# flashlight/wav2letter

Hardware: NVIDIA H100
Metric: frames_per_sec (higher is better)
Workload: dtype f32

## Files before the change

### include/w2l_b200.h

```cpp
#ifndef W2L_B200_H_
#define W2L_B200_H_

#include <stddef.h>
#include <stdint.h>

#ifdef __cplusplus
extern "C" {
#endif

#define W2L_API __attribute__((visibility("default")))

enum {
  W2L_OK = 0,
  W2L_ERR_INVALID_ARGUMENT = 1,
  W2L_ERR_WORKSPACE = 2,
  W2L_ERR_CUDA = 3,
  W2L_ERR_UNSUPPORTED = 4
};

enum {
  W2L_SCALE_NONE = 0,
  W2L_SCALE_INPUT_SZ = 1,
  W2L_SCALE_INPUT_SZ_SQRT = 2,
  W2L_SCALE_TARGET_SZ = 3,
  W2L_SCALE_TARGET_SZ_SQRT = 4
};

enum {
  W2L_TERM_FCC = 1,
  W2L_TERM_FAC = 2,
  W2L_TERM_ASG = 3
};

W2L_API int w2l_version(void);
W2L_API const char* w2l_last_error(void);
W2L_API long long w2l_launch_count(void);
W2L_API void w2l_reset_launch_count(void);
W2L_API void w2l_set_profile_events(void* start_event, void* stop_event);
W2L_API int w2l_set_profile_event_list(int kind, void** start_events, void** stop_events, int n);
W2L_API int w2l_profile_events_used(void);
W2L_API int w2l_trace_begin(void* stream, int capacity);
W2L_API long long w2l_trace_end(char* out, long long out_bytes);
W2L_API long long w2l_trace_list(char* out, long long out_bytes);

W2L_API size_t w2l_asg_workspace_size(int B, int T, int N, int L);
W2L_API int w2l_asg_forward_backward(void* stream, int terms, int B, int T, int N, int L, int scale_mode,
                                     const float* emis, const int32_t* target, const float* trans,
                                     const float* dloss, float* loss, float* d_emis, float* d_trans,
                                     void* workspace, size_t workspace_bytes);

W2L_API size_t w2l_fcc_viterbi_workspace_size(int B, int T, int N);
W2L_API int w2l_fcc_viterbi(void* stream, int B, int T, int N, const float* emis, const float* trans,
                            int32_t* path, void* workspace, size_t workspace_bytes);
W2L_API size_t w2l_fac_viterbi_workspace_size(int B, int T, int N, int L);
W2L_API int w2l_fac_viterbi(void* stream, int B, int T, int N, int L, const float* emis, const int32_t* target,
                            const float* trans, int32_t* path, int32_t* path_idx, void* workspace,
                            size_t workspace_bytes);

W2L_API size_t w2l_ctc_workspace_size(int B, int T, int N, int L);
W2L_API int w2l_ctc_forward_backward(void* stream, int B, int T, int N, int L, int scale_mode, const float* emis,
                                     const int32_t* target, const float* dloss, float* loss, float* d_emis,
                                     void* workspace, size_t workspace_bytes);
W2L_API int w2l_argmax_path(void* stream, int B, int T, int N, const float* emis, int32_t* path);

W2L_API size_t w2l_ctc_viterbi_workspace_size(int B, int T, int N, int L);
W2L_API int w2l_ctc_viterbi_target(void* stream, int B, int T, int N, int L, const float* emis, const int32_t* target,
                                   int32_t* path, int32_t* state, void* workspace, size_t workspace_bytes);

W2L_API int w2l_linseg_target(void* stream, int B, int T, int L, const int32_t* target, int32_t* out);

W2L_API int w2l_gemm_tf32_view(void* stream, int a_mn_major, int b_mn_major, int M, int N, int K, const float* A, int lda,
                               const float* B, int ldb, float* C, int ldc, const float* bias, int act, int accumulate);
enum { W2L_GEMM_TF32 = 0, W2L_GEMM_F32X3 = 1, W2L_GEMM_BF16 = 2 };
enum { W2L_PRECISION_TF32 = 0, W2L_PRECISION_F32 = 1, W2L_PRECISION_BF16 = 2 };
W2L_API int w2l_set_precision(int precision);
W2L_API int w2l_get_precision(void);
W2L_API int w2l_gemm(void* stream, int kind, int a_mn_major, int b_mn_major, int M, int N, int K, const void* A, int lda,
                     const void* B, int ldb, void* C, int ldc, int c_bf16, const float* bias, int act, int accumulate,
                     const void* aux, int ld_aux, int aux_bf16, int aux_mode, float aux_scale, float dropout_p,
                     unsigned long long seed, int allow_overlap);
W2L_API int w2l_cast_bf16(void* stream, long long n, const float* x, void* y);
W2L_API int w2l_cast_bf16_rows(void* stream, long long rows, int cols, int ld_in, int cols_padded, const float* x, void* y);
W2L_API int w2l_gemm_set_tile(int bn);
W2L_API int w2l_gemm_set_variant(int variant);
W2L_API int w2l_gemm_tf32(void* stream, int a_mn_major, int b_mn_major, int M, int N, int K, const float* A, int lda,
                          const float* B, int ldb, float* C, int ldc, const float* bias, int act);

W2L_API int w2l_gemm_tf32_ex(void* stream, int a_mn_major, int b_mn_major, int M, int N, int K, const float* A, int lda,
                             const float* B, int ldb, float* C, int ldc, const float* bias, int act, int accumulate,
                             const float* aux, int ld_aux, int aux_mode, float aux_scale, float dropout_p,
                             unsigned long long seed);

W2L_API size_t w2l_conv_time_workspace_size(int B, int Tout, int Cin, int Cout, int K);
W2L_API int w2l_conv_time_fwd(void* stream, int B, int T, int Tout, int W, int Cin, int Cout, int K, int stride,
                              int pad_left, const float* x, const float* wt, const float* bias, const float* add, float* y,
                              int act, float dropout_p, unsigned long long seed, void* ws, size_t ws_bytes);
W2L_API int w2l_conv_time_dgrad(void* stream, int B, int T, int Tout, int W, int Cin, int Cout, int K, int stride,
                                int pad_left, const float* dy, const float* wt, const float* add, float* dx, void* ws,
                                size_t ws_bytes);
W2L_API int w2l_conv_time_wgrad(void* stream, int B, int T, int Tout, int W, int Cin, int Cout, int K, int stride,
                                int pad_left, const float* x, const float* dy, float* dwt, float* dbias, void* ws,
                                size_t ws_bytes);

W2L_API int w2l_weightnorm_fwd(void* stream, int rows, int len, const float* v, const float* g, float* w, float* inv_norm);
W2L_API int w2l_weightnorm_bwd(void* stream, int rows, int len, const float* v, const float* g, const float* inv_norm,
                               const float* dw, float* dv, float* dg);
W2L_API int w2l_conv1d_arrange(void* stream, int cin, int cout, int kw, int cin_p, int cout_p, int glu_split, const float* w,
                               const float* bias, float* fwd, float* flip, float* bias_p);
W2L_API int w2l_conv1d_arrange_ex(void* stream, int cin, int cout, int kw, int cin_p, int cout_p, int glu_split, const float* w,
                                  const float* bias, void* fwd, void* flip, float* bias_p, int out_bf16);
W2L_API int w2l_conv1d_unarrange_grad(void* stream, int cin, int cout, int kw, int cin_p, int cout_p, int glu_split,
                                      const float* dfwd, float* dw, long long rows, const float* dy, float* dbias);
W2L_API int w2l_glu_fwd(void* stream, long long rows, int half, const float* x, float* y, float dropout_p,
                        unsigned long long seed);
W2L_API int w2l_glu_bwd(void* stream, long long rows, int half, const float* x, const float* dy, float* dx, float dropout_p,
                        unsigned long long seed);

#define W2L_LN_MAX_PARTS 80
#define W2L_LN_SCRATCH_DOUBLES(B) (2 * W2L_LN_MAX_PARTS * (size_t)(B))
W2L_API int w2l_layernorm_fwd(void* stream, int B, long long R, float eps, const float* a, const float* r,
                              const float* gain, const float* bias, float* y, float* mean_rstd, double* scratch);
W2L_API int w2l_layernorm_bwd(void* stream, int B, long long R, const float* a, const float* r, const float* dy,
                              const float* gain, const float* mean_rstd, float* d_branch, float* d_res, int branch_mode,
                              float branch_scale, float* dgain, float* dbias, double* scratch);

W2L_API int w2l_colsum_accumulate(void* stream, int M, int N, const float* X, int ld, float* out);
W2L_API int w2l_sq_norm_accumulate(void* stream, long long n, const float* g, double* out);
W2L_API int w2l_sgd_step(void* stream, long long n, float* params, const float* grads, float* velocity, float lr,
                         float momentum, float weight_decay, float grad_scale, float max_grad_norm, const double* sq_norm);
W2L_API int w2l_sgd_step_ex(void* stream, long long n, float* params, const float* grads, float* velocity, float lr, float momentum,
                            float weight_decay, float grad_scale, float max_grad_norm, const double* sq_norm, int nesterov,
                            const int* guard);
W2L_API int w2l_finite_guard(void* stream, int n_loss, const float* loss, const double* sq_norm, int* guard);
W2L_API int w2l_mask_bands(void* stream, int B, int T, int C, int W, const float* x, float* y, int n_f, const int* f0_host,
                           const int* f1_host, int n_t, const int* t0_host, const int* t1_host, float value);

W2L_API int w2l_transpose_input(void* stream, int B, int F, int T, const float* in, float* out);
W2L_API int w2l_axpy(void* stream, long long n, float a, const float* x, float* y);
W2L_API int w2l_fill(void* stream, long long n, float v, float* y);
W2L_API int w2l_delay(void* stream, int us);
W2L_API int w2l_act_fwd(void* stream, long long n, const float* x, int relu, float dropout_p, unsigned long long seed, float* y);
W2L_API int w2l_mask_mul(void* stream, long long n, const float* g, const float* ref, int mode, float scale, float* out);

W2L_API int w2l_mfsc_num_frames(int n_samples, int sample_rate, int frame_ms, int stride_ms);
W2L_API size_t w2l_mfsc_workspace_size(int B, int max_samples, int sample_rate, int frame_ms, int stride_ms, int n_filters);
W2L_API int w2l_mfsc(void* stream, int B, int max_samples, const float* audio, const int32_t* n_samples_host, int sample_rate,
                     int frame_ms, int stride_ms, int n_filters, int left_ctx, float* features, int T_out, void* ws,
                     size_t ws_bytes);

W2L_API void* w2l_trainer_create(void* stream, const char* arch_text, int n_feat, int n_label, const char* criterion,
                                 int scale_mode, float transdiag, float lr, float lrcrit, float momentum, float maxgradnorm);
W2L_API void w2l_trainer_destroy(void* trainer);
W2L_API int w2l_trainer_step(void* trainer, void* stream, int B, int T, const float* features, int L, const int32_t* target,
                             float* loss_out, int train, float total_batch);
W2L_API int w2l_trainer_forward(void* trainer, void* stream, int B, int T, const float* features, float* emissions_out,
                                long long capacity, int* t_out);
W2L_API int w2l_trainer_align(void* trainer, void* stream, int B, int T, const float* features, int L, const int32_t* target,
                              int32_t* path, int32_t* idx, long long capacity, int* t_out);
W2L_API int w2l_trainer_time_stride(void* trainer);
W2L_API int w2l_trainer_set_grad_stream(void* trainer, int on);
W2L_API int w2l_trainer_set_grad_stream_delay(void* trainer, int us);
W2L_API int w2l_trainer_set_precision(void* trainer, int precision);
W2L_API int w2l_trainer_status(void* trainer, void* stream, long long* skipped_steps);
W2L_API long long w2l_trainer_num_params(void* trainer, int which );
W2L_API int w2l_trainer_param_layout(void* trainer, int which, int max_params, long long* elements, long long* dims4);
W2L_API int w2l_trainer_get_flat(void* trainer, void* stream, int which, int what , float* out);
W2L_API int w2l_trainer_set_flat(void* trainer, void* stream, int which, const float* in);
W2L_API int w2l_trainer_sync_parameters(void* trainer, void* stream);
W2L_API const char* w2l_trainer_describe(void* trainer);
W2L_API int w2l_trainer_save(void* trainer, void* stream, const char* path);
W2L_API void* w2l_trainer_load(void* stream, const char* path);
W2L_API int w2l_trainer_export_streaming(void* trainer, void* stream, const char* outdir, const char* tokens_text);
W2L_API int w2l_nccl_unique_id(void* out128);
W2L_API int w2l_init_distributed(int rank, int world, const void* id128);

W2L_API void* w2l_text_create(const char* tokens_text, const char* lexicon_text, const char* criterion, int replabel,
                              const char* surround, int usewordpiece, const char* wordsep);
W2L_API void w2l_text_destroy(void* text);
W2L_API int w2l_text_num_classes(void* text);
W2L_API long long w2l_text_encode(void* text, const char* transcript, int32_t* out, long long cap);
W2L_API long long w2l_text_prediction2ltr(void* text, const int32_t* path, int n, char* out, long long cap);
W2L_API long long w2l_text_target2ltr(void* text, const int32_t* target, int len, char* out, long long cap);
W2L_API long long w2l_text_ltr2wrd(void* text, const char* letters, char* out, long long cap);
W2L_API long long w2l_text_align_words(void* text, const int32_t* target, int len, const int32_t* idx, int n_frames,
                                       double ms_per_frame, const char* utt_id, char* out, long long cap);
W2L_API int w2l_edit_distance(const char* hyp, const char* ref, long long* out4);

#ifdef __cplusplus
}
#endif
#endif
```

### wav2letter_b200/capi.py

```python
from __future__ import annotations

import ctypes
import os

import torch

_HERE = os.path.dirname(os.path.abspath(__file__))
LIB_PATH = os.path.join(_HERE, "libw2l_b200.so")

SCALE_MODES = {"none": 0, "input_sz": 1, "input_sz_sqrt": 2, "target_sz": 3, "target_sz_sqrt": 4}
TERM_FCC, TERM_FAC, TERM_ASG = 1, 2, 3

EXPORTS = [
    "w2l_version", "w2l_last_error", "w2l_launch_count", "w2l_reset_launch_count", "w2l_set_profile_events", "w2l_set_profile_event_list", "w2l_profile_events_used", "w2l_trace_begin", "w2l_trace_end", "w2l_trace_list",
    "w2l_asg_workspace_size", "w2l_asg_forward_backward",
    "w2l_fcc_viterbi_workspace_size", "w2l_fcc_viterbi",
    "w2l_fac_viterbi_workspace_size", "w2l_fac_viterbi",
    "w2l_ctc_workspace_size", "w2l_ctc_forward_backward", "w2l_argmax_path", "w2l_linseg_target",
    "w2l_ctc_viterbi_workspace_size", "w2l_ctc_viterbi_target",
    "w2l_set_precision", "w2l_get_precision", "w2l_gemm", "w2l_cast_bf16", "w2l_cast_bf16_rows", "w2l_sgd_step_ex", "w2l_finite_guard",
    "w2l_mask_bands", "w2l_trainer_set_precision", "w2l_trainer_set_grad_stream", "w2l_trainer_set_grad_stream_delay", "w2l_delay", "w2l_trainer_status", "w2l_trainer_save", "w2l_trainer_load", "w2l_trainer_export_streaming",
    "w2l_text_create", "w2l_text_destroy", "w2l_text_num_classes", "w2l_text_encode", "w2l_text_prediction2ltr", "w2l_text_target2ltr",
    "w2l_text_ltr2wrd", "w2l_text_align_words", "w2l_edit_distance",
    "w2l_gemm_set_variant", "w2l_gemm_set_tile", "w2l_gemm_tf32", "w2l_gemm_tf32_ex", "w2l_gemm_tf32_view", "w2l_conv_time_workspace_size", "w2l_conv_time_fwd", "w2l_conv_time_dgrad",
    "w2l_conv_time_wgrad", "w2l_layernorm_fwd", "w2l_layernorm_bwd", "w2l_colsum_accumulate", "w2l_sq_norm_accumulate",
    "w2l_sgd_step", "w2l_weightnorm_fwd", "w2l_weightnorm_bwd", "w2l_conv1d_arrange", "w2l_conv1d_arrange_ex", "w2l_conv1d_unarrange_grad",
    "w2l_glu_fwd", "w2l_glu_bwd", "w2l_transpose_input", "w2l_axpy", "w2l_fill", "w2l_act_fwd", "w2l_mask_mul",
    "w2l_trainer_create", "w2l_trainer_destroy", "w2l_trainer_step", "w2l_trainer_forward", "w2l_trainer_num_params",
    "w2l_trainer_param_layout", "w2l_trainer_get_flat", "w2l_trainer_set_flat", "w2l_trainer_sync_parameters",
    "w2l_trainer_describe", "w2l_nccl_unique_id", "w2l_init_distributed", "w2l_trainer_align", "w2l_trainer_time_stride",
    "w2l_mfsc_num_frames", "w2l_mfsc_workspace_size", "w2l_mfsc",
]


class W2LError(RuntimeError):
    def __init__(self, code: int, msg: str):
        super().__init__(f"w2l error {code}: {msg}")
        self.code = code


def _load() -> ctypes.CDLL:
    if not os.path.exists(LIB_PATH):
        raise ImportError(
            f"{LIB_PATH} is missing: build it with `python -c 'import __graft_entry__ as g; g.build()'` "
            "(there is no CPU / PyTorch fallback for the hot path)")
    lib = ctypes.CDLL(LIB_PATH)
    vp, i, sz = ctypes.c_void_p, ctypes.c_int, ctypes.c_size_t
    lib.w2l_last_error.restype = ctypes.c_char_p
    lib.w2l_launch_count.restype = ctypes.c_longlong
    lib.w2l_set_profile_events.argtypes = [vp, vp]
    lib.w2l_set_profile_event_list.argtypes = [i, vp, vp, i]
    lib.w2l_trace_begin.argtypes = [vp, i]
    lib.w2l_trace_end.restype = ctypes.c_longlong
    lib.w2l_trace_end.argtypes = [ctypes.c_char_p, ctypes.c_longlong]
    lib.w2l_trace_list.restype = ctypes.c_longlong
    lib.w2l_trace_list.argtypes = [ctypes.c_char_p, ctypes.c_longlong]
    lib.w2l_asg_workspace_size.restype = sz
    lib.w2l_asg_workspace_size.argtypes = [i, i, i, i]
    lib.w2l_asg_forward_backward.argtypes = [vp, i, i, i, i, i, i, vp, vp, vp, vp, vp, vp, vp, vp, sz]
    lib.w2l_fcc_viterbi_workspace_size.restype = sz
    lib.w2l_fcc_viterbi_workspace_size.argtypes = [i, i, i]
    lib.w2l_fcc_viterbi.argtypes = [vp, i, i, i, vp, vp, vp, vp, sz]
    lib.w2l_fac_viterbi_workspace_size.restype = sz
    lib.w2l_fac_viterbi_workspace_size.argtypes = [i, i, i, i]
    lib.w2l_fac_viterbi.argtypes = [vp, i, i, i, i, vp, vp, vp, vp, vp, vp, sz]
    lib.w2l_ctc_workspace_size.restype = sz
    lib.w2l_ctc_workspace_size.argtypes = [i, i, i, i]
    lib.w2l_ctc_forward_backward.argtypes = [vp, i, i, i, i, i, vp, vp, vp, vp, vp, vp, sz]
    lib.w2l_argmax_path.argtypes = [vp, i, i, i, vp, vp]
    lib.w2l_linseg_target.argtypes = [vp, i, i, i, vp, vp]
    lib.w2l_ctc_viterbi_workspace_size.restype = sz
    lib.w2l_ctc_viterbi_workspace_size.argtypes = [i, i, i, i]
    lib.w2l_ctc_viterbi_target.argtypes = [vp, i, i, i, i, vp, vp, vp, vp, vp, sz]
    lib.w2l_gemm_tf32.argtypes = [vp, i, i, i, i, i, vp, i, vp, i, vp, i, vp, i]
    f32, u64, ll = ctypes.c_float, ctypes.c_ulonglong, ctypes.c_longlong
    ll = ctypes.c_longlong
    lib.w2l_weightnorm_fwd.argtypes = [vp, i, i, vp, vp, vp, vp]
    lib.w2l_weightnorm_bwd.argtypes = [vp, i, i, vp, vp, vp, vp, vp, vp]
    lib.w2l_conv1d_arrange.argtypes = [vp, i, i, i, i, i, i, vp, vp, vp, vp, vp]
    lib.w2l_conv1d_unarrange_grad.argtypes = [vp, i, i, i, i, i, i, vp, vp, ll, vp, vp]
    lib.w2l_glu_fwd.argtypes = [vp, ll, i, vp, vp, f32, u64]
    lib.w2l_glu_bwd.argtypes = [vp, ll, i, vp, vp, vp, f32, u64]
    lib.w2l_act_fwd.argtypes = [vp, ll, vp, i, f32, u64, vp]
    lib.w2l_mask_mul.argtypes = [vp, ll, vp, vp, i, f32, vp]
    lib.w2l_gemm_tf32_view.argtypes = [vp, i, i, i, i, i, vp, i, vp, i, vp, i, vp, i, i]
    lib.w2l_gemm_tf32_ex.argtypes = [vp, i, i, i, i, i, vp, i, vp, i, vp, i, vp, i, i, vp, i, i, f32, f32, u64]
    lib.w2l_conv_time_workspace_size.restype = sz
    lib.w2l_conv_time_workspace_size.argtypes = [i, i, i, i, i]
    lib.w2l_conv_time_fwd.argtypes = [vp, i, i, i, i, i, i, i, i, i, vp, vp, vp, vp, vp, i, f32, u64, vp, sz]
    lib.w2l_conv_time_dgrad.argtypes = [vp, i, i, i, i, i, i, i, i, i, vp, vp, vp, vp, vp, sz]
    lib.w2l_conv_time_wgrad.argtypes = [vp, i, i, i, i, i, i, i, i, i, vp, vp, vp, vp, vp, sz]
    lib.w2l_layernorm_fwd.argtypes = [vp, i, ll, f32, vp, vp, vp, vp, vp, vp, vp]
    lib.w2l_layernorm_bwd.argtypes = [vp, i, ll, vp, vp, vp, vp, vp, vp, vp, i, f32, vp, vp, vp]
    lib.w2l_colsum_accumulate.argtypes = [vp, i, i, vp, i, vp]
    lib.w2l_sq_norm_accumulate.argtypes = [vp, ll, vp, vp]
    lib.w2l_sgd_step.argtypes = [vp, ll, vp, vp, vp, f32, f32, f32, f32, f32, vp]
    lib.w2l_set_precision.argtypes = [i]
    lib.w2l_gemm.argtypes = [vp, i, i, i, i, i, i, vp, i, vp, i, vp, i, i, vp, i, i, vp, i, i, i, f32, f32, u64, i]
    lib.w2l_cast_bf16.argtypes = [vp, ll, vp, vp]
    lib.w2l_cast_bf16_rows.argtypes = [vp, ll, i, i, i, vp, vp]
    lib.w2l_sgd_step_ex.argtypes = [vp, ll, vp, vp, vp, f32, f32, f32, f32, f32, vp, i, vp]
    lib.w2l_finite_guard.argtypes = [vp, i, vp, vp, vp]
    lib.w2l_mask_bands.argtypes = [vp, i, i, i, i, vp, vp, i, vp, vp, i, vp, vp, f32]
    lib.w2l_trainer_set_precision.argtypes = [vp, i]
    lib.w2l_trainer_set_grad_stream.argtypes = [vp, i]
    lib.w2l_trainer_set_grad_stream_delay.argtypes = [vp, i]
    lib.w2l_delay.argtypes = [vp, i]
    lib.w2l_trainer_status.argtypes = [vp, vp, vp]
    cp = ctypes.c_char_p
    lib.w2l_trainer_save.argtypes = [vp, vp, cp]
    lib.w2l_trainer_load.restype = vp
    lib.w2l_trainer_load.argtypes = [vp, cp]
    lib.w2l_trainer_export_streaming.argtypes = [vp, vp, cp, cp]
    lib.w2l_text_create.restype = vp
    lib.w2l_text_create.argtypes = [cp, cp, cp, i, cp, i, cp]
    lib.w2l_text_destroy.argtypes = [vp]
    lib.w2l_text_destroy.restype = None
    lib.w2l_text_num_classes.argtypes = [vp]
    for fn in (lib.w2l_text_encode, lib.w2l_text_prediction2ltr, lib.w2l_text_target2ltr, lib.w2l_text_ltr2wrd):
        fn.restype = ll
    lib.w2l_text_encode.argtypes = [vp, cp, vp, ll]
    lib.w2l_text_prediction2ltr.argtypes = [vp, vp, i, vp, ll]
    lib.w2l_text_target2ltr.argtypes = [vp, vp, i, vp, ll]
    lib.w2l_text_ltr2wrd.argtypes = [vp, cp, vp, ll]
    lib.w2l_text_align_words.restype = ll
    lib.w2l_text_align_words.argtypes = [vp, vp, i, vp, i, ctypes.c_double, cp, vp, ll]
    lib.w2l_edit_distance.argtypes = [cp, cp, vp]
    lib.w2l_trainer_create.restype = vp
    lib.w2l_trainer_create.argtypes = [vp, ctypes.c_char_p, i, i, ctypes.c_char_p, i, f32, f32, f32, f32, f32]
    lib.w2l_trainer_destroy.argtypes = [vp]
    lib.w2l_trainer_destroy.restype = None
    lib.w2l_trainer_step.argtypes = [vp, vp, i, i, vp, i, vp, vp, i, f32]
    lib.w2l_trainer_forward.argtypes = [vp, vp, i, i, vp, vp, ll, vp]
    lib.w2l_trainer_align.argtypes = [vp, vp, i, i, vp, i, vp, vp, vp, ll, vp]
    lib.w2l_trainer_time_stride.argtypes = [vp]
    lib.w2l_trainer_num_params.restype = ll
    lib.w2l_trainer_num_params.argtypes = [vp, i]
    lib.w2l_trainer_param_layout.argtypes = [vp, i, i, vp, vp]
    lib.w2l_trainer_get_flat.argtypes = [vp, vp, i, i, vp]
    lib.w2l_trainer_set_flat.argtypes = [vp, vp, i, vp]
    lib.w2l_trainer_sync_parameters.argtypes = [vp, vp]
    lib.w2l_trainer_describe.restype = ctypes.c_char_p
    lib.w2l_trainer_describe.argtypes = [vp]
    lib.w2l_nccl_unique_id.argtypes = [vp]
    lib.w2l_init_distributed.argtypes = [i, i, vp]
    lib.w2l_mfsc_num_frames.argtypes = [i, i, i, i]
    lib.w2l_mfsc_workspace_size.restype = sz
    lib.w2l_mfsc_workspace_size.argtypes = [i, i, i, i, i, i]
    lib.w2l_mfsc.argtypes = [vp, i, i, vp, vp, i, i, i, i, i, vp, i, vp, sz]
    return lib


lib = _load()


def _check(rc: int) -> None:
    if rc != 0:
        raise W2LError(rc, lib.w2l_last_error().decode())


def _stream() -> int:
    return torch.cuda.current_stream().cuda_stream


def _ptr(t):
    return None if t is None else ctypes.c_void_p(t.data_ptr())


def _req(t, dtype, name):
    if t is None:
        return None
    if not t.is_cuda or t.dtype != dtype or not t.is_contiguous():
        raise TypeError(f"{name}: expected a contiguous CUDA tensor of {dtype}")
    return t


_ws_cache: dict = {}


def workspace(nbytes: int, device) -> torch.Tensor:
    key = (str(device), "ws")
    t = _ws_cache.get(key)
    if t is None or t.numel() < nbytes:
        t = torch.empty(max(nbytes, 256), dtype=torch.uint8, device=device)
        _ws_cache[key] = t
    return t


def _mode(m) -> int:
    return SCALE_MODES[m] if isinstance(m, str) else int(m)


def launch_count() -> int:
    return int(lib.w2l_launch_count())


def reset_launch_count() -> None:
    lib.w2l_reset_launch_count()


def set_profile_events(start=None, stop=None) -> None:
    if start is None:
        lib.w2l_set_profile_events(None, None)
    else:
        start.record()
        stop.record()
        lib.w2l_set_profile_events(ctypes.c_void_p(start.cuda_event), ctypes.c_void_p(stop.cuda_event))


def asg_forward_backward(emis, target, trans, scale_mode="none", dloss=None, terms=TERM_ASG, need_grad=True,
                         out=None, ws=None):
    emis = _req(emis, torch.float32, "emis")
    trans = _req(trans, torch.float32, "trans")
    target = _req(target, torch.int32, "target")
    dloss = _req(dloss, torch.float32, "dloss")
    B, T, N = emis.shape
    L = 0 if target is None else target.shape[1]
    if out is None:
        loss = torch.empty(B, dtype=torch.float32, device=emis.device)
        d_emis = torch.empty_like(emis) if need_grad else None
        d_trans = torch.empty_like(trans) if need_grad else None
    else:
        loss, d_emis, d_trans = out
    need = lib.w2l_asg_workspace_size(B, T, N, L)
    if ws is None:
        ws = workspace(need, emis.device)
    _check(lib.w2l_asg_forward_backward(_stream(), terms, B, T, N, L, _mode(scale_mode), _ptr(emis), _ptr(target),
                                        _ptr(trans), _ptr(dloss), _ptr(loss), _ptr(d_emis), _ptr(d_trans),
                                        _ptr(ws), ws.numel()))
    return loss, d_emis, d_trans


def fcc_viterbi(emis, trans):
    emis = _req(emis, torch.float32, "emis")
    trans = _req(trans, torch.float32, "trans")
    B, T, N = emis.shape
    path = torch.empty((B, T), dtype=torch.int32, device=emis.device)
    ws = workspace(lib.w2l_fcc_viterbi_workspace_size(B, T, N), emis.device)
    _check(lib.w2l_fcc_viterbi(_stream(), B, T, N, _ptr(emis), _ptr(trans), _ptr(path), _ptr(ws), ws.numel()))
    return path


def fac_viterbi(emis, target, trans, return_index=False):
    emis = _req(emis, torch.float32, "emis")
    trans = _req(trans, torch.float32, "trans")
    target = _req(target, torch.int32, "target")
    B, T, N = emis.shape
    L = target.shape[1]
    path = torch.empty((B, T), dtype=torch.int32, device=emis.device)
    idx = torch.empty((B, T), dtype=torch.int32, device=emis.device) if return_index else None
    ws = workspace(lib.w2l_fac_viterbi_workspace_size(B, T, N, L), emis.device)
    _check(lib.w2l_fac_viterbi(_stream(), B, T, N, L, _ptr(emis), _ptr(target), _ptr(trans), _ptr(path), _ptr(idx),
                               _ptr(ws), ws.numel()))
    return (path, idx) if return_index else path


def ctc_forward_backward(emis, target, scale_mode="none", dloss=None, need_grad=True, out=None, ws=None):
    emis = _req(emis, torch.float32, "emis")
    target = _req(target, torch.int32, "target")
    dloss = _req(dloss, torch.float32, "dloss")
    B, T, N = emis.shape
    L = 0 if target is None else target.shape[1]
    if out is None:
        loss = torch.empty(B, dtype=torch.float32, device=emis.device)
        d_emis = torch.empty_like(emis) if need_grad else None
    else:
        loss, d_emis = out
    need = lib.w2l_ctc_workspace_size(B, T, N, L)
    if ws is None:
        ws = workspace(need, emis.device)
    _check(lib.w2l_ctc_forward_backward(_stream(), B, T, N, L, _mode(scale_mode), _ptr(emis), _ptr(target),
                                        _ptr(dloss), _ptr(loss), _ptr(d_emis), _ptr(ws), ws.numel()))
    return loss, d_emis


def argmax_path(emis):
    emis = _req(emis, torch.float32, "emis")
    B, T, N = emis.shape
    path = torch.empty((B, T), dtype=torch.int32, device=emis.device)
    _check(lib.w2l_argmax_path(_stream(), B, T, N, _ptr(emis), _ptr(path)))
    return path


def ctc_viterbi_target(emis, target, return_state=False):
    emis = _req(emis, torch.float32, "emis")
    target = _req(target, torch.int32, "target")
    B, T, N = emis.shape
    L = target.shape[1]
    path = torch.empty((B, T), dtype=torch.int32, device=emis.device)
    state = torch.empty((B, T), dtype=torch.int32, device=emis.device) if return_state else None
    ws = workspace(lib.w2l_ctc_viterbi_workspace_size(B, T, N, L), emis.device)
    _check(lib.w2l_ctc_viterbi_target(_stream(), B, T, N, L, _ptr(emis), _ptr(target), _ptr(path), _ptr(state), _ptr(ws),
                                      ws.numel()))
    return (path, state) if return_state else path


def linseg_target(target, T: int):
    target = _req(target, torch.int32, "target")
    B, L = target.shape
    out = torch.empty((B, int(T)), dtype=torch.int32, device=target.device)
    _check(lib.w2l_linseg_target(_stream(), B, int(T), L, _ptr(target), _ptr(out)))
    return out


class ProfileList:

    def __init__(self, kind: int, n: int):
        self.starts = [torch.cuda.Event(enable_timing=True) for _ in range(n)]
        self.stops = [torch.cuda.Event(enable_timing=True) for _ in range(n)]
        for e in self.starts + self.stops:
            e.record()
        self._a = (ctypes.c_void_p * n)(*[e.cuda_event for e in self.starts])
        self._b = (ctypes.c_void_p * n)(*[e.cuda_event for e in self.stops])
        self.kind, self.n = kind, n

    def arm(self):
        lib.w2l_set_profile_event_list(self.kind, self._a, self._b, self.n)

    def disarm(self) -> int:
        used = int(lib.w2l_profile_events_used())
        lib.w2l_set_profile_event_list(0, None, None, 0)
        return used

    def times_ms(self, used: int):
        return [self.starts[k].elapsed_time(self.stops[k]) for k in range(used)]


def trace_list() -> list:
    buf = ctypes.create_string_buffer(1 << 18)
    lib.w2l_trace_list(buf, len(buf))
    return [(ln.split("\t")[0], float(ln.split("\t")[1])) for ln in buf.value.decode().splitlines()]


PRECISIONS = {"tf32": 0, "f32": 1, "fp32": 1, "bf16": 2}
GEMM_KINDS = {"tf32": 0, "f32x3": 1, "bf16": 2}


def set_precision(p) -> None:
    _check(lib.w2l_set_precision(PRECISIONS[p] if isinstance(p, str) else int(p)))


def get_precision() -> int:
    return int(lib.w2l_get_precision())


def gemm(A, B, kind="tf32", a_mn=False, b_mn=False, bias=None, act=0, out=None, out_bf16=False, accumulate=False, aux=None,
         aux_mode=0, aux_scale=1.0, dropout_p=0.0, seed=0, M=None, N=None, K=None, lda=None, ldb=None, allow_overlap=False):
    if M is None:
        M, K = (A.shape[1], A.shape[0]) if a_mn else A.shape
        N = B.shape[1] if b_mn else B.shape[0]
    lda = A.stride(0) if lda is None else lda
    ldb = B.stride(0) if ldb is None else ldb
    if out is None:
        out = torch.empty((M, N), dtype=torch.bfloat16 if out_bf16 else torch.float32, device=A.device)
    _check(lib.w2l_gemm(_stream(), GEMM_KINDS[kind], int(a_mn), int(b_mn), M, N, K, _ptr(A), lda, _ptr(B), ldb, _ptr(out),
                        out.stride(0), int(out.dtype == torch.bfloat16), _ptr(bias), int(act), int(accumulate), _ptr(aux),
                        0 if aux is None else aux.stride(0), int(aux is not None and aux.dtype == torch.bfloat16),
                        int(aux_mode), float(aux_scale), float(dropout_p), int(seed), int(allow_overlap)))
    return out


def cast_bf16(x):
    x = _req(x, torch.float32, "x")
    y = torch.empty(x.shape, dtype=torch.bfloat16, device=x.device)
    _check(lib.w2l_cast_bf16(_stream(), x.numel(), _ptr(x), _ptr(y)))
    return y


def gemm_set_variant(v: int = 1):
    _check(lib.w2l_gemm_set_variant(int(v)))


def gemm_set_tile(bn: int = 0):
    _check(lib.w2l_gemm_set_tile(int(bn)))


def trace(fn, capacity: int = 4096) -> dict:
    _check(lib.w2l_trace_begin(_stream(), capacity))
    try:
        fn()
    finally:
        buf = ctypes.create_string_buffer(1 << 16)
        lib.w2l_trace_end(buf, len(buf))
    out = {}
    for line in buf.value.decode().splitlines():
        name, n, ms = line.split("\t")
        out[name] = (int(n), float(ms))
    return out


def gemm_tf32(A, B, bias=None, act=0, a_mn=False, b_mn=False, out=None):
    A = _req(A, torch.float32, "A")
    B = _req(B, torch.float32, "B")
    bias = _req(bias, torch.float32, "bias")
    M, K = (A.shape[1], A.shape[0]) if a_mn else A.shape
    N = B.shape[1] if b_mn else B.shape[0]
    if out is None:
        out = torch.empty((M, N), dtype=torch.float32, device=A.device)
    _check(lib.w2l_gemm_tf32(_stream(), int(a_mn), int(b_mn), M, N, K, _ptr(A), A.stride(0), _ptr(B), B.stride(0),
                             _ptr(out), out.stride(0), _ptr(bias), int(act)))
    return out


def gemm_tf32_ex(A, B, out, bias=None, act=0, a_mn=False, b_mn=False, accumulate=False, aux=None, aux_mode=0,
                 aux_scale=1.0, dropout_p=0.0, seed=0):
    M, K = (A.shape[1], A.shape[0]) if a_mn else A.shape
    N = B.shape[1] if b_mn else B.shape[0]
    _check(lib.w2l_gemm_tf32_ex(_stream(), int(a_mn), int(b_mn), M, N, K, _ptr(A), A.stride(0), _ptr(B), B.stride(0),
                                _ptr(out), out.stride(0), _ptr(bias), int(act), int(accumulate), _ptr(aux),
                                0 if aux is None else aux.stride(0), int(aux_mode), float(aux_scale), float(dropout_p),
                                int(seed)))
    return out


def gemm_tf32_view(A, lda, B, ldb, out, M, N, K, a_mn=False, b_mn=False, bias=None, act=0, accumulate=False):
    _check(lib.w2l_gemm_tf32_view(_stream(), int(a_mn), int(b_mn), M, N, K, _ptr(A), lda, _ptr(B), ldb, _ptr(out), out.stride(0),
                                  _ptr(bias), int(act), int(accumulate)))
    return out


def conv_time_ws(B, Tout, Cin, Cout, K, device):
    return workspace(lib.w2l_conv_time_workspace_size(B, Tout, Cin, Cout, K), device)


def conv_time_fwd(x, wt, bias, Tout, stride, pad_left, act=0, dropout_p=0.0, seed=0, add=None):
    B, T, Cin, W = x.shape
    Cout, _, K = wt.shape
    y = torch.empty((B, Tout, Cout, W), dtype=torch.float32, device=x.device)
    ws = conv_time_ws(B, Tout, Cin, Cout, K, x.device)
    _check(lib.w2l_conv_time_fwd(_stream(), B, T, Tout, W, Cin, Cout, K, stride, pad_left, _ptr(x), _ptr(wt), _ptr(bias),
                                 _ptr(add), _ptr(y), act, float(dropout_p), int(seed), _ptr(ws), ws.numel()))
    return y


def conv_time_dgrad(dy, wt, T, stride, pad_left, add=None, out=None):
    B, Tout, Cout, W = dy.shape
    _, Cin, K = wt.shape
    dx = out if out is not None else torch.empty((B, T, Cin, W), dtype=torch.float32, device=dy.device)
    ws = conv_time_ws(B, Tout, Cin, Cout, K, dy.device)
    _check(lib.w2l_conv_time_dgrad(_stream(), B, T, Tout, W, Cin, Cout, K, stride, pad_left, _ptr(dy), _ptr(wt), _ptr(add),
                                   _ptr(dx), _ptr(ws), ws.numel()))
    return dx


def conv_time_wgrad(x, dy, K, stride, pad_left, dwt=None, dbias=None):
    B, T, Cin, W = x.shape
    _, Tout, Cout, _ = dy.shape
    if dwt is None:
        dwt = torch.zeros((Cout, Cin, K), dtype=torch.float32, device=x.device)
        dbias = torch.zeros(Cout, dtype=torch.float32, device=x.device)
    ws = conv_time_ws(B, Tout, Cin, Cout, K, x.device)
    _check(lib.w2l_conv_time_wgrad(_stream(), B, T, Tout, W, Cin, Cout, K, stride, pad_left, _ptr(x), _ptr(dy), _ptr(dwt),
                                   _ptr(dbias), _ptr(ws), ws.numel()))
    return dwt, dbias


def layernorm_fwd(a, r, gain, bias, eps=1e-5):
    B = a.shape[0]
    R = a[0].numel()
    y = torch.empty_like(a)
    mr = torch.empty((B, 2), dtype=torch.float32, device=a.device)
    scratch = torch.empty(160 * B, dtype=torch.float64, device=a.device)
    _check(lib.w2l_layernorm_fwd(_stream(), B, R, float(eps), _ptr(a), _ptr(r), _ptr(gain), _ptr(bias), _ptr(y), _ptr(mr),
                                 _ptr(scratch)))
    return y, mr


def layernorm_bwd(a, r, dy, gain, mr, branch_mode=0, branch_scale=1.0):
    B = a.shape[0]
    R = a[0].numel()
    d_branch = torch.empty_like(a)
    d_res = torch.empty_like(a)
    dgain = torch.zeros(1, dtype=torch.float32, device=a.device)
    dbias = torch.zeros(1, dtype=torch.float32, device=a.device)
    scratch = torch.empty(160 * B, dtype=torch.float64, device=a.device)
    _check(lib.w2l_layernorm_bwd(_stream(), B, R, _ptr(a), _ptr(r), _ptr(dy), _ptr(gain), _ptr(mr), _ptr(d_branch),
                                 _ptr(d_res), int(branch_mode), float(branch_scale), _ptr(dgain), _ptr(dbias),
                                 _ptr(scratch)))
    return d_branch, d_res, dgain, dbias
```

### wav2letter_b200/csrc/gemm_wgmma.cu

```cuda
#include <cuda.h>
#include <cuda_bf16.h>
#include <cuda_runtime.h>

#include <algorithm>
#include <cmath>
#include <cstdlib>
#include <mutex>

#include "common.cuh"
#include "tma_ptx.cuh"
#include "wgmma_ptx.cuh"

namespace w2l {
namespace {
using namespace tma;

constexpr int BM = 128;
constexpr int kRowBytes = 128;
constexpr int kTileBytes = BM * kRowBytes;
constexpr int kGemmThreads = 384;
constexpr int kConvThreads = 96;
constexpr int kConsumerThreads = 256;
enum { kTf32 = W2L_GEMM_TF32, kF32x3 = W2L_GEMM_F32X3, kBf16 = W2L_GEMM_BF16 };

__host__ __device__ constexpr bool converts(int mode, bool a_mn, bool b_mn) { return mode == kF32x3 || (mode == kTf32 && (a_mn || b_mn)); }
__host__ __device__ constexpr size_t raw_bytes(int bn) { return (size_t)kTileBytes + (size_t)bn * kRowBytes; }
__host__ __device__ constexpr size_t cvt_bytes(int mode, int bn) { return (size_t)bn * kRowBytes * (mode == kF32x3 ? 2 : 1); }
constexpr size_t kSmemTail = 1024 + 256;
constexpr size_t kSmemBudget = 227 * 1024 - kSmemTail;
constexpr int kConvRawStages = 4;
constexpr int kIdSlots = 4;
__host__ __device__ constexpr int raw_stages(int mode, bool a_mn, bool b_mn, int bn) {
  return converts(mode, a_mn, b_mn) ? kConvRawStages : (kSmemBudget / raw_bytes(bn) > 6 ? 6 : (int)(kSmemBudget / raw_bytes(bn)));
}
__host__ __device__ constexpr int cvt_stages(int mode, bool a_mn, bool b_mn, int bn) {
  return !converts(mode, a_mn, b_mn) ? 0
         : (kSmemBudget - kConvRawStages * raw_bytes(bn)) / cvt_bytes(mode, bn) > 4 ? 4
                                                                                     : (int)((kSmemBudget - kConvRawStages * raw_bytes(bn)) / cvt_bytes(mode, bn));
}
__host__ __device__ constexpr size_t smem_for(int mode, bool a_mn, bool b_mn, int bn) {
  return raw_stages(mode, a_mn, b_mn, bn) * raw_bytes(bn) + cvt_stages(mode, a_mn, b_mn, bn) * cvt_bytes(mode, bn) + kSmemTail;
}

struct GemmParams {
  int M, N, K, ldc, act;
  void* C;
  const float* bias;
  int accumulate, aux_mode, ld_aux;
  const void* aux;
  float aux_scale, drop_p;
  unsigned long long seed;
  int k_splits;
  int c_bf16, aux_bf16;
  float* ws;
};

__device__ __forceinline__ uint32_t rn_tf32(uint32_t x) { return (x + 0x1000u) & 0xffffe000u; }

template <bool kMn, bool kLo, int ROWS>
__device__ __forceinline__ void convert_tile(const unsigned char* raw, unsigned char* hi, unsigned char* lo, int ct) {
#pragma unroll 4
  for (int i = ct; i < ROWS * 8; i += kConvThreads) {
    const int r = i % ROWS, c = i / ROWS;
    const uint32_t off = (uint32_t)r * 128u + ((uint32_t)(c ^ (r & 7)) << 4);
    uint4 v;
    if (kMn) {
      const uint32_t* src = reinterpret_cast<const uint32_t*>(raw) + 4 * c * ROWS + r;
      v = make_uint4(src[0], src[ROWS], src[2 * ROWS], src[3 * ROWS]);
    } else {
      v = *reinterpret_cast<const uint4*>(raw + off);
    }
    const uint4 h = make_uint4(rn_tf32(v.x), rn_tf32(v.y), rn_tf32(v.z), rn_tf32(v.w));
    *reinterpret_cast<uint4*>(hi + off) = h;
    if (kLo) {
      const uint4 l = make_uint4(rn_tf32(__float_as_uint(__uint_as_float(v.x) - __uint_as_float(h.x))),
                                 rn_tf32(__float_as_uint(__uint_as_float(v.y) - __uint_as_float(h.y))),
                                 rn_tf32(__float_as_uint(__uint_as_float(v.z) - __uint_as_float(h.z))),
                                 rn_tf32(__float_as_uint(__uint_as_float(v.w) - __uint_as_float(h.w))));
      *reinterpret_cast<uint4*>(lo + off) = l;
    }
  }
}

__device__ __forceinline__ void epilogue_pair(const GemmParams& p, int z, int row, int col, float x0, float x1, float b0, float b1, bool vec_c) {
  const bool two = col + 1 < p.N;
  x0 += b0;
  x1 += b1;
  if (p.act == 1) {
    x0 = fmaxf(x0, 0.f);
    x1 = fmaxf(x1, 0.f);
  }
  if (p.drop_p > 0.f) {
    const uint32_t thresh = (uint32_t)(p.drop_p * 65536.0f);
    const float inv_keep = 1.0f / (1.0f - p.drop_p);
    const unsigned long long idx = ((unsigned long long)row * (unsigned long long)p.N + (unsigned long long)col) >> 1;
    uint32_t h = ((uint32_t)idx ^ (uint32_t)p.seed) * 0x9E3779B1u + ((uint32_t)(idx >> 32) ^ (uint32_t)(p.seed >> 32));
    h ^= h >> 15;
    h *= 0x85EBCA77u;
    h ^= h >> 13;
    h *= 0xC2B2AE3Du;
    h ^= h >> 16;
    x0 *= (h & 0xffffu) >= thresh ? inv_keep : 0.f;
    x1 *= (h >> 16) >= thresh ? inv_keep : 0.f;
  }
  if (p.aux_mode != 0) {
    float m0, m1 = 0.f;
    const size_t ai = (size_t)row * p.ld_aux + col;
    if (p.aux_bf16) {
      const __nv_bfloat16* a = static_cast<const __nv_bfloat16*>(p.aux) + ai;
      m0 = __bfloat162float(a[0]);
      if (two) m1 = __bfloat162float(a[1]);
    } else {
      const float* a = static_cast<const float*>(p.aux) + ai;
      m0 = a[0];
      if (two) m1 = a[1];
    }
    if (p.aux_mode == 1) {
      x0 *= m0 > 0.f ? p.aux_scale : 0.f;
      x1 *= m1 > 0.f ? p.aux_scale : 0.f;
    } else {
      x0 *= m0 != 0.f ? p.aux_scale : 0.f;
      x1 *= m1 != 0.f ? p.aux_scale : 0.f;
    }
  }
  const size_t ci = (size_t)row * p.ldc + col;
  if (p.c_bf16) {
    __nv_bfloat16* dst = static_cast<__nv_bfloat16*>(p.C) + ci;
    if (two && vec_c) {
      *reinterpret_cast<__nv_bfloat162*>(dst) = __floats2bfloat162_rn(x0, x1);
    } else {
      dst[0] = __float2bfloat16_rn(x0);
      if (two) dst[1] = __float2bfloat16_rn(x1);
    }
    return;
  }
  if (p.k_splits > 1) {
    float* part = p.ws + ((size_t)z * p.M + row) * p.N + col;
    part[0] = x0;
    if (two) part[1] = x1;
    return;
  }
  float* dst = static_cast<float*>(p.C) + ci;
  if (two && vec_c) {
    if (p.accumulate) {
      const float2 c = *reinterpret_cast<const float2*>(dst);
      x0 += c.x;
      x1 += c.y;
    }
    *reinterpret_cast<float2*>(dst) = make_float2(x0, x1);
  } else {
    if (p.accumulate) x0 += dst[0];
    dst[0] = x0;
    if (two) {
      if (p.accumulate) x1 += dst[1];
      dst[1] = x1;
    }
  }
}

template <int kMode, bool kAMn, bool kBMn, int BN>
__global__ void __launch_bounds__(kGemmThreads, 1)
gemm_wgmma_kernel(const __grid_constant__ CUtensorMap map_a, const __grid_constant__ CUtensorMap map_b, GemmParams p, int tiles_m, int tiles_n,
                  unsigned int* sched) {
  extern __shared__ __align__(1024) unsigned char smem_raw[];
  unsigned char* smem = reinterpret_cast<unsigned char*>((reinterpret_cast<uintptr_t>(smem_raw) + 1023) & ~(uintptr_t)1023);
  constexpr bool kIsBf16 = kMode == kBf16, kSplit = kMode == kF32x3, kConv = converts(kMode, kAMn, kBMn);
  constexpr int BKE = kRowBytes / (kIsBf16 ? 2 : 4);
  constexpr int kStages = raw_stages(kMode, kAMn, kBMn, BN), kCvtStages = cvt_stages(kMode, kAMn, kBMn, BN);
  constexpr size_t kRaw = raw_bytes(BN), kCvt = cvt_bytes(kMode, BN);
  constexpr uint32_t kOperandBytes = (uint32_t)kRaw;
  static_assert(kStages >= 2 && (!kConv || kCvtStages >= 2), "gemm: at least two stages per ring");
  static_assert(!kConv || BN == 128, "gemm: the converted kinds take A from registers at BN = 128");
  static_assert(!kIsBf16 || !kBMn || BN % 64 == 0, "gemm: MN-major bf16 B is staged in boxes of 64 columns");
  unsigned char* cvt_ring = smem + kStages * kRaw;
  uint64_t* bars = reinterpret_cast<uint64_t*>(cvt_ring + kCvtStages * kCvt);
  uint64_t* full = bars;
  uint64_t* empty = bars + kStages;
  uint64_t* ready = bars + 2 * kStages;
  uint64_t* cvt_empty = ready + kCvtStages;
  uint64_t* id_full = cvt_empty + kCvtStages;
  uint64_t* id_empty = id_full + kIdSlots;
  int* id_ring = reinterpret_cast<int*>(id_empty + kIdSlots);
  static_assert((2 * (kStages + kCvtStages + kIdSlots)) * 8 + kIdSlots * 4 <= kSmemTail - 1024, "gemm: barrier space");
  constexpr uint32_t kIdReaders = kConsumerThreads + (kConv ? kConvThreads : 0);

  const int tid = threadIdx.x, warp = tid >> 5, lane = tid & 31, wg = warp >> 2;
  const int total_kb = (p.K + BKE - 1) / BKE;
  const int kb_per = (total_kb + p.k_splits - 1) / p.k_splits;
  const int tiles_mn = tiles_m * tiles_n, total_tiles = tiles_mn * p.k_splits;

  if (tid == 0) {
    for (int s = 0; s < kStages; ++s) {
      mbar_init(&full[s], 1);
      mbar_init(&empty[s], kConsumerThreads + (kConv ? kConvThreads : 0));
    }
    for (int s = 0; s < kCvtStages; ++s) {
      mbar_init(&ready[s], kConvThreads);
      mbar_init(&cvt_empty[s], kConsumerThreads);
    }
    for (int s = 0; s < kIdSlots; ++s) {
      mbar_init(&id_full[s], 1);
      mbar_init(&id_empty[s], kIdReaders);
    }
    asm volatile("fence.mbarrier_init.release.cluster;" ::: "memory");
  }
  __syncthreads();

  uint32_t id_it = 0;
  auto next_item = [&]() {
    const int s = id_it % kIdSlots;
    mbar_wait(&id_full[s], (id_it / kIdSlots) & 1);
    const int t = id_ring[s];
    mbar_arrive(&id_empty[s]);
    ++id_it;
    return t;
  };
  auto tile_coords = [&](int t, int& m0, int& n0, int& kb_begin, int& num_kb) {
    const int z = t / tiles_mn, r = t - z * tiles_mn;
    m0 = (r / tiles_n) * BM;
    n0 = (r % tiles_n) * BN;
    kb_begin = z * kb_per;
    num_kb = max(0, min(total_kb, kb_begin + kb_per) - kb_begin);
  };

  if (wg == 0) {
    if (warp == 0) {
      if (lane == 0) {
        asm volatile("prefetch.tensormap [%0];" ::"l"(&map_a) : "memory");
        asm volatile("prefetch.tensormap [%0];" ::"l"(&map_b) : "memory");
        uint32_t it = 0;
        for (int t = blockIdx.x; t < total_tiles;) {
          int m0, n0, kb_begin, num_kb;
          tile_coords(t, m0, n0, kb_begin, num_kb);
          for (int kb = 0; kb < num_kb; ++kb, ++it) {
            const int s = it % kStages;
            mbar_wait(&empty[s], ((it / kStages) & 1) ^ 1);
            mbar_expect_tx(&full[s], kOperandBytes);
            unsigned char* sa = smem + s * kRaw;
            unsigned char* sb = sa + kTileBytes;
            const int k0 = (kb_begin + kb) * BKE;
            if (!kAMn) {
              tma_load_2d(&map_a, &full[s], sa, k0, m0);
            } else if (kIsBf16) {
#pragma unroll
              for (int j = 0; j < BM / 64; ++j) tma_load_2d(&map_a, &full[s], sa + j * 8192, m0 + 64 * j, k0);
            } else {
#pragma unroll
              for (int j = 0; j < BM / 8; ++j) tma_load_2d(&map_a, &full[s], sa + j * 1024, m0 + 8 * j, k0);
            }
            if (!kBMn) {
              tma_load_2d(&map_b, &full[s], sb, k0, n0);
            } else if (kIsBf16) {
#pragma unroll
              for (int j = 0; j < BN / 64; ++j) tma_load_2d(&map_b, &full[s], sb + j * 8192, n0 + 64 * j, k0);
            } else {
              tma_load_2d(&map_b, &full[s], sb, n0, k0);
            }
          }
          t = sched ? (int)gridDim.x + (int)atomicAdd(sched, 1u) : t + (int)gridDim.x;
          const int s = id_it % kIdSlots;
          mbar_wait(&id_empty[s], ((id_it / kIdSlots) & 1) ^ 1);
          id_ring[s] = t;
          mbar_arrive(&id_full[s]);
          ++id_it;
        }
        if (sched) {
          __threadfence();
          if (atomicAdd(sched + 1, 1u) == gridDim.x - 1) {
            atomicExch(sched, 0u);
            atomicExch(sched + 1, 0u);
          }
        }
      }
    } else if constexpr (kConv) {
      const int ct = tid - 32;
      uint32_t it = 0;
      for (int t = blockIdx.x; t < total_tiles; t = next_item()) {
        int m0, n0, kb_begin, num_kb;
        tile_coords(t, m0, n0, kb_begin, num_kb);
        for (int kb = 0; kb < num_kb; ++kb, ++it) {
          const int s = it % kStages, c = it % kCvtStages;
          mbar_wait(&cvt_empty[c], ((it / kCvtStages) & 1) ^ 1);
          mbar_wait(&full[s], (it / kStages) & 1);
          unsigned char* dst = cvt_ring + c * kCvt;
          convert_tile<kBMn, kSplit, BN>(smem + s * kRaw + kTileBytes, dst, dst + BN * kRowBytes, ct);
          mbar_arrive(&empty[s]);
          asm volatile("fence.proxy.async.shared::cta;" ::: "memory");
          mbar_arrive(&ready[c]);
        }
      }
    }
  } else {
    const int cw = wg - 1;
    const bool vec_c = (p.ldc % 2) == 0 && (reinterpret_cast<uintptr_t>(p.C) & (p.c_bf16 ? 3 : 7)) == 0;
    const int fr = 64 * cw + 16 * (warp & 3) + (lane >> 2), fq = lane & 3;
    uint32_t it = 0;
    for (int t = blockIdx.x; t < total_tiles; t = next_item()) {
      int m0, n0, kb_begin, num_kb;
      tile_coords(t, m0, n0, kb_begin, num_kb);
      float acc[BN / 2];
#pragma unroll
      for (int i = 0; i < BN / 2; ++i) acc[i] = 0.f;
      if constexpr (kConv) {
        struct AFrag {
          uint32_t hi[4][4], lo[4][4];
        };
        auto fence_frag = [&](AFrag& f) {
          wg::fence_operands(f.hi);
          if constexpr (kSplit) wg::fence_operands(f.lo);
        };
        auto step = [&](AFrag& cur, AFrag& prev, int kb) {
          const int s = it % kStages, c = it % kCvtStages;
          mbar_wait(&full[s], (it / kStages) & 1);
          const uint32_t sa = smem_u32(smem + s * kRaw);
#pragma unroll
          for (int kk = 0; kk < 4; ++kk) {
#pragma unroll
            for (int i = 0; i < 4; ++i) {
              const int r = fr + 8 * (i & 1), k = 8 * kk + 4 * (i >> 1) + fq;
              const int off = kAMn ? (r >> 3) * 1024 + k * 32 + (r & 7) * 4 : r * 128 + (((k >> 2) ^ (r & 7)) << 4) + (k & 3) * 4;
              uint32_t x;
              asm volatile("ld.shared.b32 %0, [%1];" : "=r"(x) : "r"(sa + off) : "memory");
              cur.hi[kk][i] = rn_tf32(x);
              if constexpr (kSplit) cur.lo[kk][i] = rn_tf32(__float_as_uint(__uint_as_float(x) - __uint_as_float(cur.hi[kk][i])));
            }
          }
          mbar_arrive(&empty[s]);
          mbar_wait(&ready[c], (it / kCvtStages) & 1);
          const uint32_t b_base = smem_u32(cvt_ring + c * kCvt);
          fence_frag(cur);
          wg::fence_operands(acc);
          wg::fence();
#pragma unroll
          for (int kk = 0; kk < 4; ++kk) {
            const int sc = (kb | kk) != 0;
            const uint64_t db = make_desc_sw128(b_base + kk * 32, 16, 1024);
            if constexpr (kSplit) {
              wg::mma_tf32_rs<BN>(acc, cur.lo[kk], db, sc);
              wg::mma_tf32_rs<BN>(acc, cur.hi[kk], make_desc_sw128(b_base + BN * kRowBytes + kk * 32, 16, 1024), 1);
              wg::mma_tf32_rs<BN>(acc, cur.hi[kk], db, 1);
            } else {
              wg::mma_tf32_rs<BN>(acc, cur.hi[kk], db, sc);
            }
          }
          wg::commit();
          wg::fence_operands(acc);
          if constexpr (kSplit) wg::wait<1>(); else wg::wait<0>();
          fence_frag(prev);
          if (kb > 0) mbar_arrive(&cvt_empty[(it - 1) % kCvtStages]);
          ++it;
        };
        AFrag fa, fb;
        for (int kb = 0; kb < num_kb; kb += 2) {
          step(fa, fb, kb);
          if (kb + 1 < num_kb) step(fb, fa, kb + 1);
        }
        wg::wait<0>();
        wg::fence_operands(acc);
        fence_frag(fa);
        fence_frag(fb);
        if (num_kb > 0) mbar_arrive(&cvt_empty[(it - 1) % kCvtStages]);
      } else {
        for (int kb = 0; kb < num_kb; ++kb, ++it) {
          const int s = it % kStages;
          mbar_wait(&full[s], (it / kStages) & 1);
          const uint32_t a_base = smem_u32(smem + s * kRaw) + (uint32_t)(cw * 8192), b_base = smem_u32(smem + s * kRaw) + kTileBytes;
          wg::fence_operands(acc);
          wg::fence();
#pragma unroll
          for (int k = 0; k < 4; ++k) {
            const int sc = (kb | k) != 0;
            if constexpr (kIsBf16) {
              const uint64_t da = kAMn ? make_desc_sw128(a_base + k * 2048, 8192, 1024) : make_desc_sw128(a_base + k * 32, 16, 1024);
              const uint64_t db = kBMn ? make_desc_sw128(b_base + k * 2048, 8192, 1024) : make_desc_sw128(b_base + k * 32, 16, 1024);
              wg::mma_bf16<BN, kAMn ? 1 : 0, kBMn ? 1 : 0>(acc, da, db, sc);
            } else {
              wg::mma_tf32<BN>(acc, make_desc_sw128(a_base + k * 32, 16, 1024), make_desc_sw128(b_base + k * 32, 16, 1024), sc);
            }
          }
          wg::commit();
          wg::fence_operands(acc);
          wg::wait<1>();
          if (kb > 0) mbar_arrive(&empty[(it - 1) % kStages]);
        }
        wg::wait<0>();
        wg::fence_operands(acc);
        if (num_kb > 0) mbar_arrive(&empty[(it - 1) % kStages]);
      }
      const int z = t / tiles_mn;
      const int row0 = m0 + 64 * cw + 16 * (warp & 3) + (lane >> 2);
      const int col0 = n0 + 2 * (lane & 3);
#pragma unroll
      for (int j = 0; j < BN / 8; ++j) {
        const int col = col0 + 8 * j;
        if (col < p.N) {
          const float b0 = p.bias != nullptr ? __ldg(p.bias + col) : 0.f;
          const float b1 = (p.bias != nullptr && col + 1 < p.N) ? __ldg(p.bias + col + 1) : 0.f;
          if (row0 < p.M) epilogue_pair(p, z, row0, col, acc[4 * j], acc[4 * j + 1], b0, b1, vec_c);
          if (row0 + 8 < p.M) epilogue_pair(p, z, row0 + 8, col, acc[4 * j + 2], acc[4 * j + 3], b0, b1, vec_c);
        }
      }
    }
  }
}

__global__ void __launch_bounds__(256) splitk_reduce_kernel(int M, int N, int splits, const float* __restrict__ ws, float* __restrict__ C, int ldc,
                                                            int accumulate) {
  const long long mn = (long long)M * N;
  for (long long i = (long long)blockIdx.x * blockDim.x + threadIdx.x; i < mn; i += (long long)gridDim.x * blockDim.x) {
    const long long r = i / N, c = i - r * N;
    float* dst = C + r * ldc + c;
    float s = accumulate ? *dst : 0.f;
    for (int z = 0; z < splits; ++z) s += ws[z * mn + i];
    *dst = s;
  }
}

int make_map(CUtensorMap* map, int mode, bool conv, const void* ptr, long long rows, long long cols, long long ld, int box_cols, int box_rows,
             bool swizzle) {
  EncodeTiledFn fn = encode_fn();
  if (!fn) return fail(W2L_ERR_CUDA, "gemm: cuTensorMapEncodeTiled entry point not found");
  const int es = mode == kBf16 ? 2 : 4;
  cuuint64_t dims[2] = {(cuuint64_t)cols, (cuuint64_t)rows};
  cuuint64_t strides[1] = {(cuuint64_t)ld * es};
  cuuint32_t box[2] = {(cuuint32_t)box_cols, (cuuint32_t)box_rows};
  cuuint32_t estr[2] = {1, 1};
  const CUtensorMapDataType dt = mode == kBf16 ? CU_TENSOR_MAP_DATA_TYPE_BFLOAT16 : (conv ? CU_TENSOR_MAP_DATA_TYPE_FLOAT32 : CU_TENSOR_MAP_DATA_TYPE_TFLOAT32);
  CUresult r = fn(map, dt, 2, const_cast<void*>(ptr), dims, strides, box, estr, CU_TENSOR_MAP_INTERLEAVE_NONE,
                  swizzle ? CU_TENSOR_MAP_SWIZZLE_128B : CU_TENSOR_MAP_SWIZZLE_NONE, CU_TENSOR_MAP_L2_PROMOTION_L2_256B,
                  CU_TENSOR_MAP_FLOAT_OOB_FILL_NONE);
  if (r != CUDA_SUCCESS) return fail(W2L_ERR_CUDA, "gemm: cuTensorMapEncodeTiled failed with code " + std::to_string((int)r));
  return W2L_OK;
}

const char* kernel_name(int mode) { return mode == kBf16 ? "gemm_wgmma_kernel<bf16>" : (mode == kF32x3 ? "gemm_wgmma_kernel<f32x3>" : "gemm_wgmma_kernel<tf32>"); }

thread_local int g_variant = 1;

constexpr int kSchedSlots = 64;
__device__ unsigned int g_sched[kSchedSlots][2];
unsigned int* sched_slot(cudaStream_t stream) {
  static std::mutex mu;
  static cudaStream_t owner[kSchedSlots];
  static int used = 0;
  int slot = -1;
  {
    std::lock_guard<std::mutex> lock(mu);
    for (int i = 0; i < used && slot < 0; ++i)
      if (owner[i] == stream) slot = i;
    if (slot < 0 && used < kSchedSlots) {
      owner[used] = stream;
      slot = used++;
    }
  }
  void* base = nullptr;
  if (slot < 0 || cudaGetSymbolAddress(&base, g_sched) != cudaSuccess) return nullptr;
  return static_cast<unsigned int*>(base) + 2 * slot;
}

template <int kMode, bool kAMn, bool kBMn, int BN>
int launch_bn(cudaStream_t stream, const CUtensorMap& ma, const CUtensorMap& mb, const GemmParams& p) {
  constexpr size_t smem = smem_for(kMode, kAMn, kBMn, BN);
  static_assert(smem <= 227 * 1024, "gemm: shared-memory budget");
  static bool configured = false;
  if (!configured) {
    W2L_CUDA_CHECK(cudaFuncSetAttribute(gemm_wgmma_kernel<kMode, kAMn, kBMn, BN>, cudaFuncAttributeMaxDynamicSharedMemorySize, (int)smem));
    configured = true;
  }
  const int tiles_m = (p.M + BM - 1) / BM, tiles_n = (p.N + BN - 1) / BN;
  const int total = tiles_m * tiles_n * p.k_splits;
  const int grid = g_variant == 1 ? std::min(total, sm_count()) : total;
  unsigned int* sched = g_variant == 1 && grid < total ? sched_slot(stream) : nullptr;
  profile_kind(1);
  profile_start(stream);
  gemm_wgmma_kernel<kMode, kAMn, kBMn, BN><<<grid, kGemmThreads, smem, stream>>>(ma, mb, p, tiles_m, tiles_n, sched);
  profile_stop(stream);
  W2L_LAUNCH_CHECK(kernel_name(kMode));
  return W2L_OK;
}
template <int kMode, bool kAMn, bool kBMn>
int launch_mode(cudaStream_t stream, int bn, const CUtensorMap& ma, const CUtensorMap& mb, const GemmParams& p) {
  if constexpr (converts(kMode, kAMn, kBMn)) {
    return launch_bn<kMode, kAMn, kBMn, 128>(stream, ma, mb, p);
  } else if constexpr (kMode == kBf16) {
    return bn <= 128 ? launch_bn<kMode, kAMn, kBMn, 128>(stream, ma, mb, p) : launch_bn<kMode, kAMn, kBMn, 256>(stream, ma, mb, p);
  } else {
    switch (bn) {
      case 128: return launch_bn<kMode, kAMn, kBMn, 128>(stream, ma, mb, p);
      case 160: return launch_bn<kMode, kAMn, kBMn, 160>(stream, ma, mb, p);
      case 224: return launch_bn<kMode, kAMn, kBMn, 224>(stream, ma, mb, p);
      default: return launch_bn<kMode, kAMn, kBMn, 256>(stream, ma, mb, p);
    }
  }
}
template <int kMode>
int launch(cudaStream_t stream, bool a_mn, bool b_mn, int bn, const CUtensorMap& ma, const CUtensorMap& mb, const GemmParams& p) {
  if (!a_mn && !b_mn) return launch_mode<kMode, false, false>(stream, bn, ma, mb, p);
  if (!a_mn && b_mn) return launch_mode<kMode, false, true>(stream, bn, ma, mb, p);
  if (a_mn && b_mn) return launch_mode<kMode, true, true>(stream, bn, ma, mb, p);
  return launch_mode<kMode, true, false>(stream, bn, ma, mb, p);
}

int splits_for(int tiles, int total_kb, bool plain) {
  const int sms = sm_count();
  if (!plain || tiles >= sms || total_kb < 16) return 1;
  return std::max(1, std::min(std::min(sms / tiles, total_kb / 4), 32));
}
thread_local int g_force_bn = 0;
int choose_bn(int mode, bool a_mn, bool b_mn, int M, int N, int total_kb, bool plain, int* splits_out) {
  auto allowed = [&](int bn) {
    if (converts(mode, a_mn, b_mn)) return bn == 128;
    if (mode == kBf16) return bn == 128 || bn == 256;
    return true;
  };
  if (g_force_bn && allowed(g_force_bn)) {
    const int tiles = ((N + g_force_bn - 1) / g_force_bn) * ((M + BM - 1) / BM);
    *splits_out = splits_for(tiles, total_kb, plain);
    return g_force_bn;
  }
  const int cands[4] = {128, 160, 224, 256};
  const double sms = sm_count();
  double best = 1e300;
  int best_bn = 128;
  *splits_out = 1;
  for (int bn : cands) {
    if (!allowed(bn)) continue;
    const int tiles = ((N + bn - 1) / bn) * ((M + BM - 1) / BM);
    const int splits = splits_for(tiles, total_kb, plain);
    const int kb_local = (total_kb + splits - 1) / splits;
    const double waves = std::ceil((double)tiles * splits / sms);
    const double cost = waves * ((double)(128 + bn) * kb_local + 2.0 * bn);
    if (cost < best - 1e-9) {
      best = cost;
      best_bn = bn;
      *splits_out = splits;
    }
  }
  return best_bn;
}

int gemm_impl(void* stream_, int mode, int a_mn_major, int b_mn_major, int M, int N, int K, const void* A, int lda, const void* B, int ldb,
              void* C, int ldc, int c_bf16, const float* bias, int act, int accumulate, const void* aux, int ld_aux, int aux_bf16,
              int aux_mode, float aux_scale, float dropout_p, unsigned long long seed, bool allow_overlap) {
  cudaStream_t stream = static_cast<cudaStream_t>(stream_);
  if (mode != kTf32 && mode != kF32x3 && mode != kBf16) return fail(W2L_ERR_INVALID_ARGUMENT, "gemm: unknown operand kind");
  if (M <= 0 || N <= 0 || K <= 0) return fail(W2L_ERR_INVALID_ARGUMENT, "gemm: M, N, K must be positive");
  if (!A || !B || !C) return fail(W2L_ERR_INVALID_ARGUMENT, "gemm: null pointer");
  if (act < 0 || act > 1) return fail(W2L_ERR_INVALID_ARGUMENT, "gemm: act must be 0 (none) or 1 (relu)");
  if (aux_mode < 0 || aux_mode > 2 || (aux_mode != 0 && (!aux || ld_aux < N)))
    return fail(W2L_ERR_INVALID_ARGUMENT, "gemm: bad aux mask arguments");
  if (dropout_p < 0.f || dropout_p >= 1.f) return fail(W2L_ERR_INVALID_ARGUMENT, "gemm: dropout_p must be in [0, 1)");
  if (dropout_p > 0.f && N % 4 != 0) return fail(W2L_ERR_INVALID_ARGUMENT, "gemm: dropout needs N % 4 == 0");
  const int row_align = mode == kBf16 ? 8 : 4;
  if ((lda % row_align) || (ldb % row_align) || (reinterpret_cast<uintptr_t>(A) & 15) || (reinterpret_cast<uintptr_t>(B) & 15))
    return fail(W2L_ERR_INVALID_ARGUMENT, "gemm: operand rows must be 16-byte aligned (ld % 4 == 0 for fp32, ld % 8 == 0 for bf16)");
  if (ldc < N || (!allow_overlap && (lda < (a_mn_major ? M : K) || ldb < (b_mn_major ? N : K))))
    return fail(W2L_ERR_INVALID_ARGUMENT, "gemm: leading dimension smaller than the row length");
  if (lda <= 0 || ldb <= 0) return fail(W2L_ERR_INVALID_ARGUMENT, "gemm: non-positive leading dimension");
  if (c_bf16 && accumulate) return fail(W2L_ERR_INVALID_ARGUMENT, "gemm: accumulation needs an fp32 C");
  const int bke = kRowBytes / (mode == kBf16 ? 2 : 4);
  const int total_kb = (K + bke - 1) / bke;
  const bool plain = act == 0 && aux_mode == 0 && dropout_p == 0.f && bias == nullptr && !c_bf16;
  int splits = 1;
  const int BN = choose_bn(mode, a_mn_major != 0, b_mn_major != 0, M, N, total_kb, plain, &splits);
  const bool conv = converts(mode, a_mn_major != 0, b_mn_major != 0);
  const bool bf16 = mode == kBf16;
  CUtensorMap ma, mb;
  int rc;
  if (!a_mn_major)
    rc = make_map(&ma, mode, conv, A, M, K, lda, bke, BM, true);
  else
    rc = make_map(&ma, mode, conv, A, K, M, lda, bf16 ? 64 : 8, bke, bf16);
  if (rc) return rc;
  if (!b_mn_major)
    rc = make_map(&mb, mode, conv, B, N, K, ldb, bke, BN, true);
  else
    rc = make_map(&mb, mode, conv, B, K, N, ldb, bf16 ? 64 : BN, bke, bf16);
  if (rc) return rc;
  GemmParams p{M, N, K, ldc, act, C, bias, accumulate, aux_mode, ld_aux, aux, aux_scale, dropout_p, seed, splits, c_bf16, aux_bf16, nullptr};
  if (splits > 1) W2L_CUDA_CHECK(cudaMallocAsync(reinterpret_cast<void**>(&p.ws), sizeof(float) * (size_t)splits * M * N, stream));
  rc = mode == kBf16 ? launch<kBf16>(stream, a_mn_major, b_mn_major, BN, ma, mb, p)
                     : (mode == kF32x3 ? launch<kF32x3>(stream, a_mn_major, b_mn_major, BN, ma, mb, p) : launch<kTf32>(stream, a_mn_major, b_mn_major, BN, ma, mb, p));
  if (splits > 1) {
    if (rc == W2L_OK) {
      const long long mn = (long long)M * N;
      splitk_reduce_kernel<<<(unsigned)std::min<long long>((mn + 255) / 256, (long long)sm_count() * 8), 256, 0, stream>>>(M, N, splits, p.ws,
                                                                                                                        static_cast<float*>(C), ldc, accumulate);
      cudaError_t e = cudaGetLastError();
      if (e != cudaSuccess) rc = fail(W2L_ERR_CUDA, std::string("launch splitk_reduce_kernel: ") + cudaGetErrorString(e));
      else {
        count_launch();
        trace_launch("splitk_reduce_kernel");
      }
    }
    cudaFreeAsync(p.ws, stream);
  }
  return rc;
}

int f32_kind() { return current_precision() == W2L_PRECISION_F32 ? kF32x3 : kTf32; }

__global__ void __launch_bounds__(256) cast_bf16_kernel(long long n4, const float4* __restrict__ x, uint2* __restrict__ y, long long n,
                                                        const float* __restrict__ xs, __nv_bfloat16* __restrict__ ys) {
  const long long i = (long long)blockIdx.x * blockDim.x + threadIdx.x;
  if (i < n4) {
    const float4 v = x[i];
    const __nv_bfloat162 a = __floats2bfloat162_rn(v.x, v.y), b = __floats2bfloat162_rn(v.z, v.w);
    y[i] = make_uint2(*reinterpret_cast<const uint32_t*>(&a), *reinterpret_cast<const uint32_t*>(&b));
  }
  if (i < n - 4 * n4) ys[4 * n4 + i] = __float2bfloat16_rn(xs[4 * n4 + i]);
}
__global__ void __launch_bounds__(256) cast_bf16_rows_kernel(long long rows, int cols, int ld_in, int cols_p, const float* __restrict__ x,
                                                             __nv_bfloat16* __restrict__ y) {
  const long long total = rows * cols_p;
  for (long long i = (long long)blockIdx.x * blockDim.x + threadIdx.x; i < total; i += (long long)gridDim.x * blockDim.x) {
    const long long r = i / cols_p;
    const int c = (int)(i % cols_p);
    y[i] = c < cols ? __float2bfloat16_rn(x[r * ld_in + c]) : __float2bfloat16_rn(0.f);
  }
}

}
}

using namespace w2l;

extern "C" int w2l_gemm_set_variant(int variant) {
  if (variant < 0 || variant > 1) return fail(W2L_ERR_INVALID_ARGUMENT, "gemm: variant must be 0 (one tile per CTA) or 1 (one CTA per SM)");
  g_variant = variant;
  return W2L_OK;
}

extern "C" int w2l_gemm_set_tile(int bn) {
  if (bn != 0 && bn != 128 && bn != 160 && bn != 224 && bn != 256) return fail(W2L_ERR_INVALID_ARGUMENT, "gemm: tile width must be 0 (auto), 128, 160, 224 or 256");
  g_force_bn = bn;
  return W2L_OK;
}

extern "C" int w2l_gemm(void* stream, int kind, int a_mn_major, int b_mn_major, int M, int N, int K, const void* A, int lda, const void* B,
                        int ldb, void* C, int ldc, int c_bf16, const float* bias, int act, int accumulate, const void* aux, int ld_aux,
                        int aux_bf16, int aux_mode, float aux_scale, float dropout_p, unsigned long long seed, int allow_overlap) {
  return gemm_impl(stream, kind, a_mn_major, b_mn_major, M, N, K, A, lda, B, ldb, C, ldc, c_bf16, bias, act, accumulate, aux, ld_aux, aux_bf16,
                   aux_mode, aux_scale, dropout_p, seed, allow_overlap != 0);
}

extern "C" int w2l_gemm_tf32_ex(void* stream_, int a_mn_major, int b_mn_major, int M, int N, int K, const float* A, int lda,
                                const float* B, int ldb, float* C, int ldc, const float* bias, int act, int accumulate,
                                const float* aux, int ld_aux, int aux_mode, float aux_scale, float dropout_p,
                                unsigned long long seed) {
  return gemm_impl(stream_, f32_kind(), a_mn_major, b_mn_major, M, N, K, A, lda, B, ldb, C, ldc, 0, bias, act, accumulate, aux, ld_aux, 0, aux_mode,
                   aux_scale, dropout_p, seed, false);
}

extern "C" int w2l_gemm_tf32(void* stream_, int a_mn_major, int b_mn_major, int M, int N, int K, const float* A, int lda,
                             const float* B, int ldb, float* C, int ldc, const float* bias, int act) {
  return w2l_gemm_tf32_ex(stream_, a_mn_major, b_mn_major, M, N, K, A, lda, B, ldb, C, ldc, bias, act, 0, nullptr, 0, 0, 1.f, 0.f, 0ull);
}

extern "C" int w2l_gemm_tf32_view(void* stream_, int a_mn_major, int b_mn_major, int M, int N, int K, const float* A, int lda,
                                  const float* B, int ldb, float* C, int ldc, const float* bias, int act, int accumulate) {
  return gemm_impl(stream_, f32_kind(), a_mn_major, b_mn_major, M, N, K, A, lda, B, ldb, C, ldc, 0, bias, act, accumulate, nullptr, 0, 0, 0, 1.f, 0.f,
                   0ull, true);
}

extern "C" int w2l_cast_bf16(void* stream_, long long n, const float* x, void* y) {
  if (n <= 0) return W2L_OK;
  if (!x || !y) return fail(W2L_ERR_INVALID_ARGUMENT, "cast_bf16: null pointer");
  cudaStream_t stream = static_cast<cudaStream_t>(stream_);
  const bool vec = ((reinterpret_cast<uintptr_t>(x) & 15) == 0) && ((reinterpret_cast<uintptr_t>(y) & 7) == 0);
  const long long n4 = vec ? n / 4 : 0;
  const long long threads = std::max<long long>(n4, n - 4 * n4);
  cast_bf16_kernel<<<(unsigned)((threads + 255) / 256), 256, 0, stream>>>(n4, reinterpret_cast<const float4*>(x), static_cast<uint2*>(y), n, x,
                                                                         static_cast<__nv_bfloat16*>(y));
  W2L_LAUNCH_CHECK("cast_bf16_kernel");
  return W2L_OK;
}
extern "C" int w2l_cast_bf16_rows(void* stream_, long long rows, int cols, int ld_in, int cols_padded, const float* x, void* y) {
  if (rows <= 0 || cols <= 0) return W2L_OK;
  if (!x || !y || cols_padded < cols || ld_in < cols) return fail(W2L_ERR_INVALID_ARGUMENT, "cast_bf16_rows: bad arguments");
  cudaStream_t stream = static_cast<cudaStream_t>(stream_);
  const long long total = rows * cols_padded;
  const unsigned grid = (unsigned)std::min<long long>((total + 255) / 256, (long long)sm_count() * 16);
  cast_bf16_rows_kernel<<<grid, 256, 0, stream>>>(rows, cols, ld_in, cols_padded, x, static_cast<__nv_bfloat16*>(y));
  W2L_LAUNCH_CHECK("cast_bf16_rows_kernel");
  return W2L_OK;
}
```

### wav2letter_b200/csrc/tma_ptx.cuh

```cuda
#pragma once
#include <cuda.h>
#include <cuda_runtime.h>
#include <stdint.h>

namespace w2l {
namespace tma {

__device__ __forceinline__ uint32_t smem_u32(const void* p) { return (uint32_t)__cvta_generic_to_shared(p); }

__device__ __forceinline__ void mbar_init(uint64_t* bar, uint32_t count) {
  asm volatile("mbarrier.init.shared::cta.b64 [%0], %1;" ::"r"(smem_u32(bar)), "r"(count));
}
__device__ __forceinline__ void mbar_expect_tx(uint64_t* bar, uint32_t bytes) {
  asm volatile("mbarrier.arrive.expect_tx.shared::cta.b64 _, [%0], %1;" ::"r"(smem_u32(bar)), "r"(bytes) : "memory");
}
__device__ __forceinline__ void mbar_arrive(uint64_t* bar) {
  asm volatile("mbarrier.arrive.shared::cta.b64 _, [%0];" ::"r"(smem_u32(bar)) : "memory");
}
__device__ __forceinline__ void mbar_wait(uint64_t* bar, uint32_t parity) {
  asm volatile(
      "{\n"
      ".reg .pred P1;\n"
      "WAIT_LOOP:\n"
      "mbarrier.try_wait.parity.shared::cta.b64 P1, [%0], %1;\n"
      "@P1 bra DONE;\n"
      "bra WAIT_LOOP;\n"
      "DONE:\n"
      "}\n" ::"r"(smem_u32(bar)),
      "r"(parity)
      : "memory");
}
__device__ __forceinline__ void tma_load_2d(const CUtensorMap* map, uint64_t* bar, void* smem_dst, int c0, int c1) {
  asm volatile(
      "cp.async.bulk.tensor.2d.shared::cluster.global.mbarrier::complete_tx::bytes [%0], [%1, {%3, %4}], [%2];" ::"r"(
          smem_u32(smem_dst)),
      "l"(map), "r"(smem_u32(bar)), "r"(c0), "r"(c1)
      : "memory");
}
__device__ __forceinline__ uint64_t make_desc_sw128(uint32_t saddr, uint32_t lbo_bytes, uint32_t sbo_bytes) {
  uint64_t d = 0;
  d |= (uint64_t)((saddr >> 4) & 0x3FFF);
  d |= (uint64_t)((lbo_bytes >> 4) & 0x3FFF) << 16;
  d |= (uint64_t)((sbo_bytes >> 4) & 0x3FFF) << 32;
  d |= (uint64_t)1 << 62;
  return d;
}

typedef CUresult (*EncodeTiledFn)(CUtensorMap*, CUtensorMapDataType, cuuint32_t, void*, const cuuint64_t*, const cuuint64_t*,
                                  const cuuint32_t*, const cuuint32_t*, CUtensorMapInterleave, CUtensorMapSwizzle,
                                  CUtensorMapL2promotion, CUtensorMapFloatOOBfill);
inline EncodeTiledFn encode_fn() {
  static EncodeTiledFn fn = nullptr;
  if (fn == nullptr) {
    void* ptr = nullptr;
    cudaDriverEntryPointQueryResult qres;
    if (cudaGetDriverEntryPoint("cuTensorMapEncodeTiled", &ptr, cudaEnableDefault, &qres) != cudaSuccess ||
        qres != cudaDriverEntryPointSuccess)
      return nullptr;
    fn = reinterpret_cast<EncodeTiledFn>(ptr);
  }
  return fn;
}

}
}
```

### wav2letter_b200/host/fl_compat.cpp

```cpp
#include "fl_compat/fl_compat.h"

#include <dlfcn.h>

#include <cuda_runtime.h>
#include <nccl.h>

#include <algorithm>
#include <atomic>
#include <chrono>
#include <cstdio>
#include <thread>
#include <cmath>
#include <cstring>
#include <fstream>
#include <random>
#include <sstream>
#include <stdexcept>
#include <unordered_set>

#include "w2l_b200.h"

namespace w2l {

namespace {
thread_local cudaStream_t g_stream = nullptr;
void cudaCheck(cudaError_t e, const char* what) {
  if (e != cudaSuccess) throw std::runtime_error(std::string(what) + ": " + cudaGetErrorString(e));
}
}

void check(int rc) {
  if (rc == W2L_OK) return;
  const std::string msg = w2l_last_error();
  if (rc == W2L_ERR_CUDA) throw std::runtime_error(msg);
  throw std::invalid_argument(msg);
}

void* currentStream() { return g_stream; }
void copyRows(void* dst, size_t dstPitch, const void* src, size_t srcPitch, size_t width, size_t height) {
  cudaCheck(cudaMemcpy2DAsync(dst, dstPitch, src, srcPitch, width, height, cudaMemcpyDeviceToDevice, g_stream), "copyRows");
}
void setCurrentStream(void* s) { g_stream = static_cast<cudaStream_t>(s); }
void sync() { cudaCheck(cudaStreamSynchronize(g_stream), "af::sync"); }

namespace {
thread_local cudaStream_t g_grad_stream = nullptr;
thread_local int g_grad_delay_us = 0;
cudaError_t handOver(cudaStream_t from, cudaStream_t to) {
  static thread_local cudaEvent_t ev = nullptr;
  cudaError_t e = ev ? cudaSuccess : cudaEventCreateWithFlags(&ev, cudaEventDisableTiming);
  if (e == cudaSuccess) e = cudaEventRecord(ev, from);
  if (e == cudaSuccess) e = cudaStreamWaitEvent(to, ev, 0);
  return e;
}
}
void setGradStream(void* s, int delayUs) {
  g_grad_stream = static_cast<cudaStream_t>(s);
  g_grad_delay_us = s ? delayUs : 0;
}
void* gradStream() { return g_grad_stream; }
void forkGradStream() {
  cudaCheck(handOver(g_stream, g_grad_stream), "gradient stream fork");
  if (g_grad_delay_us) check(w2l_delay(g_grad_stream, g_grad_delay_us));
}
void joinGradStream() { cudaCheck(handOver(g_grad_stream, g_stream), "gradient stream join"); }

size_t dtypeSize(DType t) {
  switch (t) {
    case DType::f32:
    case DType::i32:
      return 4;
    case DType::f64:
      return 8;
    case DType::bf16:
      return 2;
    default:
      return 1;
  }
}

std::string Dims::str() const {
  std::ostringstream o;
  o << "[" << d[0] << " " << d[1] << " " << d[2] << " " << d[3] << "]";
  return o.str();
}

struct Storage {
  void* ptr = nullptr;
  size_t bytes = 0;
  cudaStream_t stream = nullptr;
  bool owner = true;
  bool gradRead = false;
  ~Storage() {
    if (!ptr || !owner) return;
    cudaStream_t s = g_stream ? g_stream : stream;
    if (gradRead && g_grad_stream && g_grad_stream != s) {
      handOver(s, g_grad_stream);
      s = g_grad_stream;
    }
    cudaFreeAsync(ptr, s);
  }
};
void readOnGradStream(const Tensor& t) {
  if (!t.isEmpty()) t.st_->gradRead = true;
}

namespace {
void configurePoolOnce() {
  static bool done = false;
  if (done) return;
  int dev = 0;
  cudaGetDevice(&dev);
  cudaMemPool_t pool;
  if (cudaDeviceGetDefaultMemPool(&pool, dev) == cudaSuccess) {
    unsigned long long threshold = ~0ull;
    cudaMemPoolSetAttribute(pool, cudaMemPoolAttrReleaseThreshold, &threshold);
  }
  done = true;
}
}

Tensor Tensor::empty(const Dims& dims, DType t) {
  configurePoolOnce();
  Tensor r;
  r.dims_ = dims;
  r.type_ = t;
  r.st_ = std::make_shared<Storage>();
  r.st_->bytes = std::max<size_t>(r.bytes(), 16);
  r.st_->stream = g_stream;
  cudaCheck(cudaMallocAsync(&r.st_->ptr, r.st_->bytes, g_stream), "cudaMallocAsync");
  return r;
}
Tensor Tensor::zeros(const Dims& dims, DType t) {
  Tensor r = empty(dims, t);
  r.zero();
  return r;
}
Tensor Tensor::fromHost(const void* host, const Dims& dims, DType t) {
  Tensor r = empty(dims, t);
  cudaCheck(cudaMemcpyAsync(r.ptr(), host, r.bytes(), cudaMemcpyHostToDevice, g_stream), "cudaMemcpyAsync H2D");
  return r;
}
Tensor Tensor::view(const Tensor& base, size_t byte_offset, const Dims& dims, DType t) {
  Tensor r;
  r.st_ = base.st_;
  r.off_ = base.off_ + byte_offset;
  r.dims_ = dims;
  r.type_ = t;
  if (r.off_ + r.bytes() > base.st_->bytes) throw std::invalid_argument("Tensor::view: window outside the storage");
  return r;
}
Tensor Tensor::wrap(void* device_ptr, const Dims& dims, DType t) {
  Tensor r;
  r.dims_ = dims;
  r.type_ = t;
  r.st_ = std::make_shared<Storage>();
  r.st_->ptr = device_ptr;
  r.st_->bytes = r.bytes();
  r.st_->owner = false;
  return r;
}
void* Tensor::ptr() const { return st_ ? static_cast<char*>(st_->ptr) + off_ : nullptr; }
Tensor Tensor::reshaped(const Dims& dims) const {
  if (dims.elements() != elements()) throw std::invalid_argument("moddims: element count mismatch " + dims_.str() + " -> " + dims.str());
  Tensor r = *this;
  r.dims_ = dims;
  return r;
}
void Tensor::copyToHost(void* host) const {
  cudaCheck(cudaMemcpyAsync(host, ptr(), bytes(), cudaMemcpyDeviceToHost, g_stream), "cudaMemcpyAsync D2H");
  sync();
}
void Tensor::zero() const { cudaCheck(cudaMemsetAsync(ptr(), 0, bytes(), g_stream), "cudaMemsetAsync"); }
void Tensor::fill(float v) const {
  if (type_ != DType::f32) throw std::invalid_argument("fill: f32 only");
  check(w2l_fill(g_stream, elements(), v, f32()));
}
void Tensor::copyFrom(const Tensor& src) const {
  if (src.bytes() != bytes()) throw std::invalid_argument("copyFrom: size mismatch");
  cudaCheck(cudaMemcpyAsync(ptr(), src.ptr(), bytes(), cudaMemcpyDeviceToDevice, g_stream), "cudaMemcpyAsync D2D");
}

}

namespace fl {

using w2l::check;
using w2l::currentStream;
using w2l::DType;
using w2l::forkGradStream;
using w2l::gradStream;
using w2l::readOnGradStream;

thread_local OverlappedArenaReducer* g_active_reducer = nullptr;

struct Variable::Impl {
  af::array data;
  bool calcGrad = false;
  std::vector<Variable> inputs;
  GradFunc gradFunc;
  std::shared_ptr<Variable> grad;
  af::array boundGrad;
  bool gradLive = false;
  bool onesSeed = false;
  bool gradOwned = false;
  long long validFrames = -1;
};

Variable::Variable(const af::array& data, bool calcGrad) : impl_(std::make_shared<Impl>()) {
  impl_->data = data;
  impl_->calcGrad = calcGrad;
}
Variable::Variable(const af::array& data, std::vector<Variable> inputs, GradFunc gradFunc) : impl_(std::make_shared<Impl>()) {
  impl_->data = data;
  bool any = false;
  for (auto& in : inputs) any = any || in.isCalcGrad();
  impl_->calcGrad = any;
  if (any) {
    impl_->inputs = std::move(inputs);
    impl_->gradFunc = std::move(gradFunc);
  }
}
af::array& Variable::array() const {
  if (!impl_) throw std::logic_error("Variable: empty");
  return impl_->data;
}
bool Variable::isCalcGrad() const { return impl_ && impl_->calcGrad; }
bool Variable::isGradAvailable() const { return impl_ && impl_->calcGrad && (impl_->grad != nullptr); }
Variable& Variable::grad() const {
  if (!isGradAvailable()) throw std::logic_error("Variable::grad: gradient not available");
  return *impl_->grad;
}
bool Variable::isOnesSeed() const { return impl_ && impl_->onesSeed; }
void Variable::setGradStorage(const af::array& buf) {
  if (buf.elements() != array().elements()) throw std::invalid_argument("setGradStorage: size mismatch");
  impl_->boundGrad = buf.reshaped(array().dims());
  impl_->gradLive = false;
  impl_->grad.reset();
}
af::array Variable::gradStorage() const { return impl_ ? impl_->boundGrad : af::array(); }
long long Variable::validFrames() const { return impl_ ? impl_->validFrames : -1; }
void Variable::setValidFrames(long long n) {
  if (impl_) impl_->validFrames = n;
}
af::array Variable::accumulableGrad() const {
  if (impl_ && impl_->calcGrad && impl_->boundGrad.isEmpty() && impl_->grad && impl_->gradOwned) return impl_->grad->array();
  return af::array();
}
void Variable::addGrad(const Variable& g, bool fresh) {
  if (!impl_ || !impl_->calcGrad) return;
  if (g.elements() != elements()) throw std::invalid_argument("addGrad: size mismatch");
  if (!impl_->boundGrad.isEmpty()) {
    if (g.array().ptr() != impl_->boundGrad.ptr())
      check(w2l_axpy(currentStream(), elements(), 1.0f, g.array().f32(), impl_->boundGrad.f32()));
    if (!impl_->grad) impl_->grad = std::make_shared<Variable>(impl_->boundGrad, false);
    if (g_active_reducer) g_active_reducer->onGradReady(impl_.get());
    return;
  }
  if (!impl_->grad) {
    impl_->grad = std::make_shared<Variable>(g.array(), false);
    impl_->grad->impl_->onesSeed = g.isOnesSeed();
    impl_->gradOwned = fresh;
  } else if (impl_->gradOwned) {
    if (g.array().ptr() != impl_->grad->array().ptr())
      check(w2l_axpy(currentStream(), elements(), 1.0f, g.array().f32(), impl_->grad->array().f32()));
  } else {
    af::array sum = af::array::empty(array().dims());
    sum.copyFrom(impl_->grad->array());
    check(w2l_axpy(currentStream(), elements(), 1.0f, g.array().f32(), sum.f32()));
    impl_->grad = std::make_shared<Variable>(sum, false);
    impl_->gradOwned = true;
  }
}
void Variable::zeroGrad(bool zeroStorage) {
  if (!impl_) return;
  impl_->grad.reset();
  impl_->gradLive = false;
  impl_->gradOwned = false;
  if (zeroStorage && !impl_->boundGrad.isEmpty()) impl_->boundGrad.zero();
}
void Variable::backward(bool retainGraph) {
  af::array ones = af::array::empty(array().dims());
  ones.fill(1.0f);
  Variable seed(ones, false);
  seed.impl_->onesSeed = true;
  backward(seed, retainGraph);
}
void Variable::backward(const Variable& g, bool retainGraph) {
  addGrad(g);
  std::vector<Variable> order;
  std::unordered_set<const void*> seen;
  std::function<void(const Variable&)> dfs = [&](const Variable& v) {
    if (!v.impl_ || seen.count(v.id())) return;
    seen.insert(v.id());
    for (auto& in : v.impl_->inputs) dfs(in);
    order.push_back(v);
  };
  dfs(*this);
  if (g_active_reducer)
    for (const Variable& v : order)
      if (v.impl_->gradFunc)
        for (const Variable& in : v.impl_->inputs)
          if (in.impl_ && !in.impl_->boundGrad.isEmpty()) g_active_reducer->expectContribution(in.impl_.get());
  for (auto it = order.rbegin(); it != order.rend(); ++it) {
    Variable& v = *it;
    if (v.impl_->gradFunc && v.isGradAvailable()) v.impl_->gradFunc(v.impl_->inputs, v.grad());
    if (!retainGraph && v.impl_->gradFunc) {
      v.impl_->gradFunc = nullptr;
      v.impl_->inputs.clear();
      v.impl_->grad.reset();
    }
  }
}
Variable constant(double v, const af::dim4& dims, DType t, bool calcGrad) {
  af::array a = af::array::empty(dims, t);
  if (t == DType::f32)
    a.fill((float)v);
  else
    a.zero();
  return Variable(a, calcGrad);
}

Variable Module::param(int i) const {
  auto p = params();
  if (i < 0 || i >= (int)p.size()) throw std::out_of_range("Module::param: index out of range");
  return p[i];
}
void Module::setParams(const Variable& v, int i) {
  if (i < 0 || i >= (int)params_.size()) throw std::out_of_range("Module::setParams: index out of range");
  params_[i] = v;
}
void Module::zeroGrad() {
  for (auto& p : params()) p.zeroGrad();
}
std::vector<Variable> UnaryModule::forward(const std::vector<Variable>& inputs) {
  if (inputs.empty()) throw std::invalid_argument("UnaryModule: expects at least one input");
  return {forward(inputs[0])};
}
void Sequential::add(std::shared_ptr<Module> m) { modules_.push_back(std::move(m)); }
std::vector<Variable> Sequential::forward(const std::vector<Variable>& inputs) {
  std::vector<Variable> cur = inputs;
  for (auto& m : modules_) cur = m->forward(cur);
  return cur;
}
std::vector<Variable> Sequential::params() const {
  std::vector<Variable> all;
  for (auto& m : modules_) {
    auto p = m->params();
    all.insert(all.end(), p.begin(), p.end());
  }
  return all;
}
void Sequential::setParams(const Variable& v, int i) {
  for (auto& m : modules_) {
    const int n = (int)m->params().size();
    if (i < n) {
      m->setParams(v, i);
      return;
    }
    i -= n;
  }
  throw std::out_of_range("Sequential::setParams: index out of range");
}
void Sequential::train() {
  train_ = true;
  for (auto& m : modules_) m->train();
}
void Sequential::eval() {
  train_ = false;
  for (auto& m : modules_) m->eval();
}
std::string Sequential::prettyString() const {
  std::ostringstream o;
  o << "Sequential [input";
  for (size_t i = 0; i < modules_.size(); ++i) o << " -> (" << i << ")";
  o << " -> output]";
  for (size_t i = 0; i < modules_.size(); ++i) o << "\n\t(" << i << "): " << modules_[i]->prettyString();
  return o.str();
}

namespace {
std::atomic<unsigned long long> g_seed_counter{0x5eed0000ull};
unsigned long long nextSeed() { return g_seed_counter.fetch_add(0x9E3779B97F4A7C15ull); }

af::array uniformInit(const af::dim4& dims, double bound, unsigned long long seed) {
  std::mt19937_64 gen(seed);
  std::uniform_real_distribution<float> dist((float)-bound, (float)bound);
  std::vector<float> h((size_t)dims.elements());
  for (auto& v : h) v = dist(gen);
  return af::array::fromHost(h.data(), dims);
}

void requireInternal(const Variable& v, const char* who) {
  if (v.type() != DType::f32) throw std::invalid_argument(std::string(who) + ": expects f32 activations");
}
af::array workspaceFor(af::array& cache, size_t bytes) {
  if (cache.isEmpty() || cache.bytes() < bytes) cache = af::array::empty(af::dim4((long long)std::max<size_t>(bytes, 256)), DType::u8);
  return cache;
}
thread_local af::array g_conv_ws;
thread_local af::array g_conv_grad_ws;

bool bf16Mode() { return w2l_get_precision() == W2L_PRECISION_BF16; }
int gemmKind() { return bf16Mode() ? W2L_GEMM_BF16 : (w2l_get_precision() == W2L_PRECISION_F32 ? W2L_GEMM_F32X3 : W2L_GEMM_TF32); }
int chanPad() { return bf16Mode() ? 8 : 4; }
long long padUp(long long n, long long a) { return (n + a - 1) / a * a; }
af::array padRowsF32(const float* x, long long rows, int cols, int ld, int colsP) {
  af::array out = af::array::zeros(af::dim4(colsP, rows));
  w2l::copyRows(out.f32(), sizeof(float) * (size_t)colsP, x, sizeof(float) * (size_t)ld, sizeof(float) * (size_t)cols, (size_t)rows);
  return out;
}
af::array castRowsBf16(const float* x, long long rows, int cols, int ld, int colsP) {
  af::array out = af::array::empty(af::dim4(colsP, rows), DType::bf16);
  if (cols == colsP && ld == cols)
    check(w2l_cast_bf16(currentStream(), rows * cols, x, out.ptr()));
  else
    check(w2l_cast_bf16_rows(currentStream(), rows, cols, ld, colsP, x, out.ptr()));
  return out;
}
struct GemmOperand {
  af::array a;
  int ld = 0;
};
GemmOperand gemmOperand(const af::array& x, long long rows, int cols, int ld) {
  GemmOperand op;
  if (bf16Mode()) {
    op.ld = (int)padUp(cols, 8);
    op.a = castRowsBf16(x.f32(), rows, cols, ld, op.ld);
  } else if (ld % 4 == 0 && (reinterpret_cast<uintptr_t>(x.ptr()) & 15) == 0) {
    op.a = x;
    op.ld = ld;
  } else {
    op.ld = (int)padUp(cols, 4);
    op.a = padRowsF32(x.f32(), rows, cols, ld, op.ld);
  }
  return op;
}
int gemmP(int a_mn, int b_mn, int M, int N, int K, const GemmOperand& A, const GemmOperand& B, float* C, int ldc, const float* bias, int act,
          int accumulate, const float* aux = nullptr, int ld_aux = 0, int aux_mode = 0, float aux_scale = 1.f, float dropP = 0.f,
          unsigned long long seed = 0, int allowOverlap = 0) {
  return w2l_gemm(currentStream(), gemmKind(), a_mn, b_mn, M, N, K, A.a.ptr(), A.ld, B.a.ptr(), B.ld, C, ldc, 0, bias, act, accumulate, aux, ld_aux, 0,
                  aux_mode, aux_scale, dropP, seed, allowOverlap);
}
}

Variable View::forward(const Variable& in) {
  if (dims_[2] == 1 && dims_[0] == -1 && in.dims(2) == 1 && in.dims(1) == dims_[1]) {
    const long long T = in.dims(0), F = in.dims(1), B = in.dims(3);
    af::array out = af::array::empty(af::dim4(F, 1, T, B));
    check(w2l_transpose_input(currentStream(), (int)B, (int)F, (int)T, in.array().f32(), out.f32()));
    return Variable(out, in.isCalcGrad());
  }
  if (dims_[1] == 1 && dims_[0] == -1 && dims_[2] > 1 && in.dims(2) == 1 && in.dims(1) == dims_[2]) {
    const long long T = in.dims(0), F = in.dims(1), B = in.dims(3);
    if (F % chanPad()) throw std::invalid_argument("View: the channel-major head needs a feature count that is a multiple of 4 (8 in bf16 mode)");
    af::array out = af::array::empty(af::dim4(1, F, T, B));
    check(w2l_transpose_input(currentStream(), (int)B, (int)F, (int)T, in.array().f32(), out.f32()));
    return Variable(out, in.isCalcGrad());
  }
  if (dims_[2] > 1 && dims_[1] > 0 && (dims_[0] == 0 || dims_[0] == -1 || dims_[0] == in.dims(2)) && (dims_[3] == 0 || dims_[3] == in.dims(3)) &&
      dims_[1] * dims_[2] == in.dims(0) * in.dims(1) && (dims_[1] != in.dims(0) || dims_[2] != in.dims(1))) {
    af::array y = in.array().reshaped(af::dim4(dims_[1], dims_[2], in.dims(2), in.dims(3)));
    Variable out(y, {in}, [](std::vector<Variable>& ins, const Variable& g) { ins[0].addGrad(Variable(g.array().reshaped(ins[0].dims()), false)); });
    out.setValidFrames(in.validFrames());
    return out;
  }
  return in;
}
std::string View::prettyString() const { return "View (" + dims_.str() + ")"; }
std::string Reorder::prettyString() const {
  std::ostringstream o;
  o << "Reorder (" << perm_[0] << "," << perm_[1] << "," << perm_[2] << "," << perm_[3] << ")";
  return o.str();
}

Conv2D::Conv2D(int nIn_, int nOut_, int wx, int wy, int sx, int sy, int px, int py, int dx, int dy, bool bias, int groups)
    : nIn(nIn_), nOut(nOut_), kw(wx), stride(sx), pad(px), hasBias_(bias) {
  if (wy != 1 || sy != 1 || dx != 1 || dy != 1 || groups != 1 || (py != 0 && py != -1))
    throw std::invalid_argument("Conv2D: only kw x 1 kernels over time (wy = sy = 1, no dilation/groups) are covered");
  if (nIn <= 0 || nOut <= 0 || kw <= 0 || sx <= 0) throw std::invalid_argument("Conv2D: non-positive size");
  const double bound = std::sqrt(3.0 / (double)(nIn * kw));
  params_.push_back(Variable(uniformInit(af::dim4(kw, 1, nIn, nOut), bound, nextSeed()), true));
  if (bias) params_.push_back(Variable(uniformInit(af::dim4(1, 1, nOut, 1), bound, nextSeed()), true));
}
std::string Conv2D::prettyString() const {
  std::ostringstream o;
  o << "Conv2D (" << nIn << "->" << nOut << ", " << kw << "x1, " << stride << ",1, " << (pad == -1 ? std::string("SAME") : std::to_string(pad))
    << ",0, 1, 1)" << (hasBias_ ? " (with bias)" : " (without bias)") << (relu_ ? " +ReLU" : "") << (dropP_ > 0 ? " +Dropout" : "");
  return o.str();
}
Variable Conv2D::forwardMasked(const Variable& in, bool maskByConsumer) {
  return forwardWith(in, params_[0], hasBias_ ? params_[1] : Variable(), maskByConsumer);
}
Variable Conv2D::forwardWith(const Variable& in, const Variable& weight, const Variable& biasVar, bool maskByConsumer) {
  requireInternal(in, "Conv2D");
  const int W = (int)in.dims(0), Cin = (int)in.dims(1), T = (int)in.dims(2), B = (int)in.dims(3);
  if (W == 1 && (Cin == padUp(nIn, 4) || Cin == padUp(nIn, 8))) return forwardGemm(in, weight, biasVar);
  if (Cin != nIn) throw std::invalid_argument("Conv2D: input has " + std::to_string(Cin) + " channels, expected " + std::to_string(nIn));
  int pl, pr;
  if (explicitPad_) {
    pl = padL_;
    pr = padR_;
  } else if (pad == (int)PaddingMode::SAME) {
    const int rem = T % stride;
    int tot = (kw - 1) - (rem == 0 ? stride : rem) + 1;
    pl = pr = std::max((tot + 1) / 2, 0);
  } else {
    pl = pr = pad;
  }
  const int Tout = (T + pl + pr - kw) / stride + 1;
  if (Tout <= 0) throw std::invalid_argument("Conv2D: input shorter than the kernel");
  af::array y = af::array::empty(af::dim4(W, nOut, Tout, B));
  const size_t wsb = w2l_conv_time_workspace_size(B, Tout, nIn, nOut, kw);
  af::array ws = workspaceFor(g_conv_ws, wsb);
  const float dp = (train_ && dropP_ > 0) ? dropP_ : 0.f;
  const unsigned long long seed = nextSeed();
  Variable wv = weight;
  Variable bv = hasBias_ ? biasVar : Variable();
  check(w2l_conv_time_fwd(currentStream(), B, T, Tout, W, nIn, nOut, kw, stride, pl, in.array().f32(), wv.array().f32(),
                          hasBias_ ? bv.array().f32() : nullptr, nullptr, y.f32(), relu_ ? 1 : 0, dp, seed, ws.ptr(), ws.bytes()));
  const bool relu = relu_;
  const int k = kw, s = stride, cin = nIn, cout = nOut;
  const bool hasBias = hasBias_;
  std::vector<Variable> inputs{in, wv};
  if (hasBias) inputs.push_back(bv);
  return Variable(y, inputs, [=](std::vector<Variable>& ins, const Variable& gout) {
    af::array dy = gout.array();
    if (!maskByConsumer && (relu || dp > 0.f)) {
      af::array m = af::array::empty(y.dims());
      check(w2l_mask_mul(currentStream(), y.elements(), dy.f32(), y.f32(), relu ? 1 : 2, dp > 0.f ? 1.0f / (1.0f - dp) : 1.0f, m.f32()));
      dy = m;
    }
    const size_t wsb2 = w2l_conv_time_workspace_size(B, Tout, cin, cout, k);
    af::array ws2 = workspaceFor(g_conv_ws, wsb2);
    if (ins[0].isCalcGrad()) {
      af::array acc = ins[0].accumulableGrad();
      af::array dx = acc.isEmpty() ? af::array::empty(ins[0].dims()) : acc;
      check(w2l_conv_time_dgrad(currentStream(), B, T, Tout, W, cin, cout, k, s, pl, dy.f32(), ins[1].array().f32(),
                                acc.isEmpty() ? nullptr : acc.f32(), dx.f32(), ws2.ptr(), ws2.bytes()));
      if (acc.isEmpty()) ins[0].addGrad(Variable(dx, false), true);
    }
    if (ins[1].isCalcGrad()) {
      af::array dw = ins[1].gradStorage();
      af::array db = hasBias ? ins[2].gradStorage() : af::array();
      void* wstream = currentStream();
      af::array wws = ws2;
      if (gradStream() && !dw.isEmpty() && (!hasBias || !db.isEmpty())) {
        wstream = gradStream();
        wws = workspaceFor(g_conv_grad_ws, wsb2);
        readOnGradStream(wws);
        readOnGradStream(dy);
        readOnGradStream(ins[0].array());
        forkGradStream();
      }
      if (dw.isEmpty()) dw = af::array::zeros(ins[1].dims());
      if (hasBias && db.isEmpty()) db = af::array::zeros(ins[2].dims());
      check(w2l_conv_time_wgrad(wstream, B, T, Tout, W, cin, cout, k, s, pl, ins[0].array().f32(), dy.f32(), dw.f32(),
                                hasBias ? db.f32() : nullptr, wws.ptr(), wws.bytes()));
      ins[1].addGrad(Variable(dw, false));
      if (hasBias) ins[2].addGrad(Variable(db, false));
    }
  });
}

namespace {
void copyFrames(const af::array& src, long long srcFrames, long long srcOff, af::array& dst, long long dstFrames, long long dstOff,
                long long frames, long long C, long long B) {
  w2l::copyRows(dst.f32() + dstOff * C, sizeof(float) * dstFrames * C, src.f32() + srcOff * C, sizeof(float) * srcFrames * C,
                sizeof(float) * frames * C, (size_t)B);
}
}
Variable Conv2D::forwardGemm(const Variable& in, const Variable& weight, const Variable& biasVar) {
  if (stride != 1) throw std::invalid_argument("Conv2D: the large-channel path covers stride 1 only");
  const int Cp = (int)in.dims(1), TsIn = (int)in.dims(2), B = (int)in.dims(3);
  const int align = chanPad();
  if (Cp % align) throw std::invalid_argument("Conv2D: the activation's channel padding does not match the precision mode (bf16 rows are multiples of 8 channels)");
  const int TvIn = in.validFrames() >= 0 ? (int)in.validFrames() : TsIn;
  int pl, pr;
  if (explicitPad_) {
    pl = padL_;
    pr = padR_;
  } else if (pad == (int)PaddingMode::SAME) {
    pl = pr = kw / 2;
  } else {
    pl = pr = pad;
  }
  const bool padded = pl || pr;
  const int Ts = padded ? TvIn + pl + pr : TsIn;
  const int Tv = padded ? Ts : TvIn;
  const int Tout = Tv - kw + 1;
  if (Tout <= 0) throw std::invalid_argument("Conv2D: input shorter than the kernel");
  const bool glu = gluSplit_;
  if (glu && (nOut % 2)) throw std::invalid_argument("Conv2D: a GLU needs an even channel count");
  const int CoutP = glu ? 2 * (int)padUp(nOut / 2, align) : (int)padUp(nOut, align);
  const int cin = nIn, cout = nOut, k = kw;
  const bool hasBias = hasBias_, relu = relu_;
  const DType wtype = bf16Mode() ? DType::bf16 : DType::f32;
  GemmOperand fwdOp, flipOp;
  fwdOp.a = af::array::empty(af::dim4((long long)k * Cp, CoutP), wtype);
  fwdOp.ld = k * Cp;
  flipOp.a = af::array::empty(af::dim4((long long)k * CoutP, Cp), wtype);
  flipOp.ld = k * CoutP;
  af::array biasP = af::array::empty(af::dim4(CoutP));
  check(w2l_conv1d_arrange_ex(currentStream(), cin, cout, k, Cp, CoutP, glu ? 1 : 0, weight.array().f32(),
                              hasBias ? biasVar.array().f32() : nullptr, fwdOp.a.ptr(), flipOp.a.ptr(), biasP.f32(), bf16Mode() ? 1 : 0));
  af::array xp = in.array();
  if (padded) {
    xp = af::array::zeros(af::dim4(1, Cp, Ts, B));
    copyFrames(in.array(), TsIn, 0, xp, Ts, pl, TvIn, Cp, B);
  }
  const long long rowsAll = (long long)B * Ts, M = rowsAll - k + 1;
  if (rowsAll > 0x7fffffffLL / 2) throw std::invalid_argument("Conv2D: batch too long for one GEMM");
  const GemmOperand xop = gemmOperand(xp, rowsAll, Cp, Cp);
  af::array y = af::array::empty(af::dim4(1, CoutP, Ts, B));
  cudaMemsetAsync(y.f32() + (size_t)M * CoutP, 0, sizeof(float) * (size_t)(k - 1) * CoutP, static_cast<cudaStream_t>(currentStream()));
  check(gemmP(0, 0, (int)M, CoutP, k * Cp, xop, fwdOp, y.f32(), CoutP, biasP.f32(), relu ? 1 : 0, 0, nullptr, 0, 0, 1.f, 0.f, 0ull, 1));
  std::vector<Variable> inputs{in, weight};
  if (hasBias) inputs.push_back(biasVar);
  Variable out(y, inputs, [=](std::vector<Variable>& ins, const Variable& gout) {
    af::array dy = gout.array();
    if (relu) {
      af::array m = af::array::empty(y.dims());
      check(w2l_mask_mul(currentStream(), y.elements(), dy.f32(), y.f32(), 1, 1.0f, m.f32()));
      dy = m;
    }
    if (ins[1].isCalcGrad()) {
      af::array dWarr = af::array::empty(af::dim4((long long)k * Cp, CoutP));
      const GemmOperand dyop = gemmOperand(dy, rowsAll, CoutP, CoutP);
      check(gemmP(1, 1, CoutP, k * Cp, (int)M, dyop, xop, dWarr.f32(), k * Cp, nullptr, 0, 0, nullptr, 0, 0, 1.f, 0.f, 0ull, 1));
      af::array dw = ins[1].gradStorage();
      if (dw.isEmpty()) dw = af::array::zeros(ins[1].dims());
      af::array db;
      if (hasBias) {
        db = ins[2].gradStorage();
        if (db.isEmpty()) db = af::array::zeros(ins[2].dims());
      }
      check(w2l_conv1d_unarrange_grad(currentStream(), cin, cout, k, Cp, CoutP, glu ? 1 : 0, dWarr.f32(), dw.f32(), rowsAll, dy.f32(),
                                      hasBias ? db.f32() : nullptr));
      ins[1].addGrad(Variable(dw, false));
      if (hasBias) ins[2].addGrad(Variable(db, false));
    }
    if (ins[0].isCalcGrad()) {
      GemmOperand dypOp;
      dypOp.ld = CoutP;
      if (bf16Mode()) {
        dypOp.a = af::array::empty(af::dim4(CoutP, rowsAll + k - 1), DType::bf16);
        cudaMemsetAsync(dypOp.a.ptr(), 0, 2 * (size_t)(k - 1) * CoutP, static_cast<cudaStream_t>(currentStream()));
        check(w2l_cast_bf16(currentStream(), rowsAll * CoutP, dy.f32(), static_cast<char*>(dypOp.a.ptr()) + 2 * (size_t)(k - 1) * CoutP));
      } else {
        dypOp.a = af::array::empty(af::dim4(CoutP, rowsAll + k - 1));
        cudaMemsetAsync(dypOp.a.ptr(), 0, sizeof(float) * (size_t)(k - 1) * CoutP, static_cast<cudaStream_t>(currentStream()));
        w2l::copyRows(dypOp.a.f32() + (size_t)(k - 1) * CoutP, sizeof(float) * (size_t)rowsAll * CoutP, dy.f32(), sizeof(float) * (size_t)rowsAll * CoutP,
                      sizeof(float) * (size_t)rowsAll * CoutP, 1);
      }
      af::array dxp = af::array::empty(af::dim4(1, Cp, Ts, B));
      check(gemmP(0, 0, (int)rowsAll, Cp, k * CoutP, dypOp, flipOp, dxp.f32(), Cp, nullptr, 0, 0, nullptr, 0, 0, 1.f, 0.f, 0ull, 1));
      if (Tv < Ts)
        cudaMemset2DAsync(dxp.f32() + (size_t)Tv * Cp, sizeof(float) * (size_t)Ts * Cp, 0, sizeof(float) * (size_t)(Ts - Tv) * Cp, (size_t)B,
                          static_cast<cudaStream_t>(currentStream()));
      af::array dx = dxp;
      if (padded) {
        dx = af::array::zeros(af::dim4(1, Cp, TsIn, B));
        copyFrames(dxp, Ts, pl, dx, TsIn, 0, TvIn, Cp, B);
      }
      ins[0].addGrad(Variable(dx, false), true);
    }
  });
  out.setValidFrames(Tout);
  return out;
}

Variable Reorder::forward(const Variable& in) {
  const long long Tv = in.validFrames(), Ts = in.dims(2);
  if (Tv < 0 || Tv == Ts) return in;
  const long long C = in.dims(0) * in.dims(1), B = in.dims(3);
  af::array y = af::array::empty(af::dim4(in.dims(0), in.dims(1), Tv, B));
  w2l::copyRows(y.f32(), sizeof(float) * Tv * C, in.array().f32(), sizeof(float) * Ts * C, sizeof(float) * Tv * C, (size_t)B);
  return Variable(y, {in}, [=](std::vector<Variable>& ins, const Variable& g) {
    af::array dx = af::array::zeros(ins[0].dims());
    w2l::copyRows(dx.f32(), sizeof(float) * Ts * C, g.array().f32(), sizeof(float) * Tv * C, sizeof(float) * Tv * C, (size_t)B);
    ins[0].addGrad(Variable(dx, false), true);
  });
}

std::string GatedLinearUnit::prettyString() const {
  return "GatedLinearUnit (" + std::to_string(dim_) + ")" + (dropP_ > 0 ? " +Dropout" : "");
}
Variable GatedLinearUnit::forward(const Variable& in) {
  requireInternal(in, "GatedLinearUnit");
  const bool lead = in.dims(0) > 1;
  const long long C = lead ? in.dims(0) : in.dims(1);
  if (C % 2) throw std::invalid_argument("GatedLinearUnit: odd channel count " + std::to_string(C));
  const long long rows = in.elements() / C, H = C / 2;
  af::dim4 od = in.dims();
  od[lead ? 0 : 1] = H;
  af::array y = af::array::empty(od);
  const float dp = (train_ && dropP_ > 0) ? dropP_ : 0.f;
  const unsigned long long seed = nextSeed();
  check(w2l_glu_fwd(currentStream(), rows, (int)H, in.array().f32(), y.f32(), dp, seed));
  Variable out(y, {in}, [=](std::vector<Variable>& ins, const Variable& g) {
    af::array dx = af::array::empty(ins[0].dims());
    check(w2l_glu_bwd(currentStream(), rows, (int)H, ins[0].array().f32(), g.array().f32(), dx.f32(), dp, seed));
    ins[0].addGrad(Variable(dx, false), true);
  });
  out.setValidFrames(in.validFrames());
  return out;
}

WeightNorm::WeightNorm(std::shared_ptr<Module> module, int dim) : module_(std::move(module)), dim_(dim) {
  Variable v, b;
  bool hasBias = false;
  if (auto conv = std::dynamic_pointer_cast<Conv2D>(module_)) {
    if (dim != 3) throw std::invalid_argument("WeightNorm: a Conv2D is normalised along dim 3 (output channels)");
    rows_ = conv->nOut;
    len_ = conv->nIn * conv->kw;
    hasBias = conv->hasBias();
  } else if (auto lin = std::dynamic_pointer_cast<Linear>(module_)) {
    if (dim != 0) throw std::invalid_argument("WeightNorm: a Linear is normalised along dim 0 (output units)");
    rows_ = lin->nOut;
    len_ = lin->nIn;
    hasBias = lin->hasBias();
  } else {
    throw std::invalid_argument("WeightNorm: only Conv2D and Linear are covered");
  }
  v = module_->param(0);
  af::array g = af::array::empty(af::dim4(rows_));
  af::array tmpw = af::array::empty(v.dims()), ones = af::array::empty(af::dim4(rows_));
  ones.fill(1.0f);
  check(w2l_weightnorm_fwd(currentStream(), rows_, len_, v.array().f32(), ones.f32(), tmpw.f32(), g.f32()));
  std::vector<float> h = g.host<float>();
  for (auto& x : h) x = 1.0f / x;
  g = af::array::fromHost(h.data(), af::dim4(rows_));
  params_.push_back(v);
  params_.push_back(Variable(g, true));
  if (hasBias) params_.push_back(module_->param(1));
}
void WeightNorm::train() {
  train_ = true;
  module_->train();
}
void WeightNorm::eval() {
  train_ = false;
  module_->eval();
}
std::string WeightNorm::prettyString() const { return "WeightNorm (" + std::to_string(dim_) + ") of " + module_->prettyString(); }
Variable WeightNorm::forward(const Variable& in) {
  Variable v = params_[0], g = params_[1];
  Variable b = params_.size() > 2 ? params_[2] : Variable();
  af::array w = af::array::empty(v.dims());
  af::array inv = af::array::empty(af::dim4(rows_));
  const int rows = rows_, len = len_;
  check(w2l_weightnorm_fwd(currentStream(), rows, len, v.array().f32(), g.array().f32(), w.f32(), inv.f32()));
  Variable wv(w, {v, g}, [=](std::vector<Variable>& ins, const Variable& gw) {
    af::array dv = ins[0].gradStorage(), dg = ins[1].gradStorage();
    if (dv.isEmpty()) dv = af::array::zeros(ins[0].dims());
    if (dg.isEmpty()) dg = af::array::zeros(ins[1].dims());
    check(w2l_weightnorm_bwd(currentStream(), rows, len, ins[0].array().f32(), ins[1].array().f32(), inv.f32(), gw.array().f32(), dv.f32(),
                             dg.f32()));
    ins[0].addGrad(Variable(dv, false));
    ins[1].addGrad(Variable(dg, false));
  });
  if (auto conv = std::dynamic_pointer_cast<Conv2D>(module_)) return conv->forwardWith(in, wv, b, false);
  return std::static_pointer_cast<Linear>(module_)->forwardWith(in, wv, b);
}

Variable ReLU::forward(const Variable& in) {
  af::array y = af::array::empty(in.dims());
  check(w2l_act_fwd(currentStream(), in.elements(), in.array().f32(), 1, 0.f, 0ull, y.f32()));
  return Variable(y, {in}, [y](std::vector<Variable>& ins, const Variable& g) {
    af::array d = af::array::empty(y.dims());
    check(w2l_mask_mul(currentStream(), y.elements(), g.array().f32(), y.f32(), 1, 1.0f, d.f32()));
    ins[0].addGrad(Variable(d, false));
  });
}
Variable Dropout::forward(const Variable& in) {
  if (!train_ || p_ <= 0) return in;
  af::array y = af::array::empty(in.dims());
  const float p = (float)p_;
  check(w2l_act_fwd(currentStream(), in.elements(), in.array().f32(), 0, p, nextSeed(), y.f32()));
  return Variable(y, {in}, [y, p](std::vector<Variable>& ins, const Variable& g) {
    af::array d = af::array::empty(y.dims());
    check(w2l_mask_mul(currentStream(), y.elements(), g.array().f32(), y.f32(), 2, 1.0f / (1.0f - p), d.f32()));
    ins[0].addGrad(Variable(d, false));
  });
}
std::string Dropout::prettyString() const { return "Dropout (" + std::to_string(p_) + ")"; }

SpecAugment::SpecAugment(int tWarpW, int fMaskF, int nFMask, int tMaskT, double tMaskP, int nTMask)
    : tWarpW_(tWarpW), fMaskF_(fMaskF), nFMask_(nFMask), tMaskT_(tMaskT), nTMask_(nTMask), tMaskP_(tMaskP), rng_(nextSeed()) {
  if (nFMask > 0 && fMaskF <= 0) throw std::invalid_argument("invalid arguments for frequency masking.");
  if (nTMask > 0 && tMaskT <= 0) throw std::invalid_argument("invalid arguments for time masking.");
  if (nTMask > 0 && (tMaskP <= 0 || tMaskP > 1.0)) throw std::invalid_argument("invalid arguments for time masking.");
  if (nFMask > 8 || nTMask > 8) throw std::invalid_argument("SpecAugment: at most 8 masks per axis are covered");
}
std::string SpecAugment::prettyString() const {
  std::ostringstream o;
  o << "SpecAugment ( W: " << tWarpW_ << ", F: " << fMaskF_ << ", mF: " << nFMask_ << ", T: " << tMaskT_ << ", p: " << tMaskP_ << ", mT: " << nTMask_ << " )";
  return o.str();
}
Variable SpecAugment::forward(const Variable& in) {
  if (!train_) return in;
  requireInternal(in, "SpecAugment");
  const int W = (int)in.dims(0), C = (int)in.dims(1), T = (int)in.dims(2), B = (int)in.dims(3);
  if (W < fMaskF_) throw std::runtime_error("Invalid input frequency channels");
  auto randInt = [&](int low, int high) {
    return high - 1 <= low ? low : std::uniform_int_distribution<int>(low, high - 1)(rng_);
  };
  int f0[8], f1[8], t0[8], t1[8], nt = 0;
  for (int i = 0; i < nFMask_; ++i) {
    const int f = randInt(0, fMaskF_);
    f0[i] = randInt(0, W - f);
    f1[i] = std::min(W, f0[i] + f + 1);
  }
  const int Tm = std::min(tMaskT_, (int)(T * tMaskP_));
  if (Tm > 0)
    for (; nt < nTMask_; ++nt) {
      const int t = randInt(0, Tm);
      t0[nt] = randInt(0, T - t);
      t1[nt] = std::min(T, t0[nt] + t + 1);
    }
  af::array y = af::array::empty(in.dims());
  check(w2l_mask_bands(currentStream(), B, T, C, W, in.array().f32(), y.f32(), nFMask_, f0, f1, nt, t0, t1, 0.0f));
  return Variable(y, false);
}

LayerNorm::LayerNorm(const std::vector<int>& axes, double eps, bool affine) : axes_(axes), eps_(eps) {
  std::vector<int> s = axes;
  std::sort(s.begin(), s.end());
  const bool whole = (s == std::vector<int>{0, 1, 2}) || (s == std::vector<int>{3});
  perFrame_ = (s == std::vector<int>{1, 2});
  if (!whole && !perFrame_) throw std::invalid_argument("LayerNorm: axes must be {0,1,2} (whole sample) or {1,2} (per frame)");
  if (affine) {
    params_.push_back(Variable(af::array::zeros(af::dim4(1)), true));
    params_[0].array().fill(1.0f);
    params_.push_back(Variable(af::array::zeros(af::dim4(1)), true));
  }
}
std::string LayerNorm::prettyString() const {
  return perFrame_ ? "LayerNorm ( axis : { 1 2 } , size : -1)" : "LayerNorm ( axis : { 0 1 2 } , size : -1)";
}
Variable LayerNorm::forward(const Variable& in) { return forwardResidual(in, Variable(), 0, 1.0f); }
Variable LayerNorm::forwardResidual(const Variable& a, const Variable& r, int branchMode, float keepScale) {
  requireInternal(a, "LayerNorm");
  const long long groups = perFrame_ ? a.dims(2) * a.dims(3) : a.dims(3);
  if (groups > 0x7fffffffLL) throw std::invalid_argument("LayerNorm: too many groups");
  const int B = (int)groups;
  const long long R = a.elements() / B;
  const bool hasRes = !r.isEmpty();
  if (hasRes && r.elements() != a.elements()) throw std::invalid_argument("LayerNorm: residual size mismatch");
  af::array y = af::array::empty(a.dims());
  af::array mr = af::array::empty(af::dim4(2, B));
  af::array scratch = af::array::empty(af::dim4((long long)W2L_LN_SCRATCH_DOUBLES(B)), DType::f64);
  const bool affine = !params_.empty();
  check(w2l_layernorm_fwd(currentStream(), B, R, (float)eps_, a.array().f32(), hasRes ? r.array().f32() : nullptr,
                          affine ? params_[0].array().f32() : nullptr, affine ? params_[1].array().f32() : nullptr, y.f32(), mr.f32(),
                          scratch.f64()));
  std::vector<Variable> inputs{a};
  if (hasRes) inputs.push_back(r);
  if (affine) {
    inputs.push_back(params_[0]);
    inputs.push_back(params_[1]);
  }
  return Variable(y, inputs, [=](std::vector<Variable>& ins, const Variable& g) {
    const int gi = hasRes ? 2 : 1;
    af::array d_branch = af::array::empty(ins[0].dims());
    af::array d_res = hasRes ? af::array::empty(ins[0].dims()) : af::array();
    af::array dg, db;
    if (affine) {
      dg = ins[gi].gradStorage();
      if (dg.isEmpty()) dg = af::array::zeros(af::dim4(1));
      db = ins[gi + 1].gradStorage();
      if (db.isEmpty()) db = af::array::zeros(af::dim4(1));
    }
    af::array sc = af::array::empty(af::dim4((long long)W2L_LN_SCRATCH_DOUBLES(B)), DType::f64);
    check(w2l_layernorm_bwd(currentStream(), B, R, ins[0].array().f32(), hasRes ? ins[1].array().f32() : nullptr, g.array().f32(),
                            affine ? ins[gi].array().f32() : nullptr, mr.f32(), d_branch.f32(), hasRes ? d_res.f32() : nullptr,
                            branchMode, keepScale, affine ? dg.f32() : nullptr, affine ? db.f32() : nullptr, sc.f64()));
    ins[0].addGrad(Variable(d_branch, false), true);
    if (hasRes) ins[1].addGrad(Variable(d_res, false), true);
    if (affine) {
      ins[gi].addGrad(Variable(dg, false));
      ins[gi + 1].addGrad(Variable(db, false));
    }
  });
}

Linear::Linear(int nIn_, int nOut_, bool bias) : nIn(nIn_), nOut(nOut_), hasBias_(bias) {
  if (nIn <= 0 || nOut <= 0) throw std::invalid_argument("Linear: non-positive size");
  const double bound = std::sqrt(1.0 / (double)nIn);
  params_.push_back(Variable(uniformInit(af::dim4(nIn, nOut), bound, nextSeed()), true));
  if (bias) params_.push_back(Variable(uniformInit(af::dim4(nOut), bound, nextSeed()), true));
}
std::string Linear::prettyString() const {
  return "Linear (" + std::to_string(nIn) + "->" + std::to_string(nOut) + ")" + (hasBias_ ? " (with bias)" : " (without bias)");
}
Variable Linear::forward(const Variable& in) { return forwardFused(in, false, 0.f); }
Variable Linear::forwardFused(const Variable& in, bool relu, float dropP, bool maskByConsumer, int inMaskMode, float inMaskScale) {
  return forwardWith(in, params_[0], hasBias_ ? params_[1] : Variable(), relu, dropP, maskByConsumer, inMaskMode, inMaskScale);
}
Variable Linear::forwardWith(const Variable& in, const Variable& weight, const Variable& bias, bool relu, float dropP, bool maskByConsumer,
                             int inMaskMode, float inMaskScale) {
  requireInternal(in, "Linear");
  if (in.validFrames() >= 0 && in.validFrames() != in.dims(2))
    throw std::invalid_argument("Linear: the input carries slack frames (large-channel convolutions); a Reorder must come first");
  auto isPadded = [&](long long c) { return c == nIn || (c > nIn && (c == padUp(nIn, 4) || c == padUp(nIn, 8))); };
  long long T, B;
  int inCols;
  if (in.dims(0) == 1 && isPadded(in.dims(1))) {
    inCols = (int)in.dims(1);
    T = in.dims(2);
    B = in.dims(3);
  } else if (isPadded(in.dims(0))) {
    inCols = (int)in.dims(0);
    T = in.dims(1);
    B = in.dims(2) * in.dims(3);
  } else if (in.dims(0) * in.dims(1) == nIn) {
    inCols = nIn;
    T = in.dims(2);
    B = in.dims(3);
  } else {
    throw std::invalid_argument("Linear: input " + in.dims().str() + " does not have " + std::to_string(nIn) + " features");
  }
  const int M = (int)(T * B);
  af::array y = af::array::empty(af::dim4(nOut, T, B));
  Variable wv = weight;
  Variable bv = hasBias_ ? bias : Variable();
  const float dp = (train_ && dropP > 0) ? dropP : 0.f;
  const GemmOperand xop = gemmOperand(in.array(), M, inCols, inCols);
  const int Kp = xop.ld;
  GemmOperand wop;
  if (bf16Mode()) {
    wop.ld = Kp;
    wop.a = castRowsBf16(wv.array().f32(), nOut, nIn, nIn, Kp);
  } else if (Kp == nIn) {
    wop.a = wv.array();
    wop.ld = nIn;
  } else {
    wop.ld = Kp;
    wop.a = padRowsF32(wv.array().f32(), nOut, nIn, nIn, Kp);
  }
  check(gemmP(0, 0, M, nOut, Kp, xop, wop, y.f32(), nOut, hasBias_ ? bv.array().f32() : nullptr, relu ? 1 : 0, 0, nullptr, 0, 0, 1.f, dp, nextSeed()));
  const int nin = nIn, nout = nOut;
  const bool hasBias = hasBias_;
  std::vector<Variable> inputs{in, wv};
  if (hasBias) inputs.push_back(bv);
  return Variable(y, inputs, [=](std::vector<Variable>& ins, const Variable& gout) {
    af::array dy = gout.array();
    if (!maskByConsumer && (relu || dp > 0.f)) {
      af::array m = af::array::empty(y.dims());
      check(w2l_mask_mul(currentStream(), y.elements(), dy.f32(), y.f32(), relu ? 1 : 2, dp > 0.f ? 1.0f / (1.0f - dp) : 1.0f, m.f32()));
      dy = m;
    }
    const GemmOperand dyop = gemmOperand(dy, M, nout, nout);
    if (ins[1].isCalcGrad()) {
      void* wstream = currentStream();
      if (gradStream() && Kp == nin && !ins[1].gradStorage().isEmpty() && (!hasBias || !ins[2].gradStorage().isEmpty())) {
        wstream = gradStream();
        forkGradStream();
        readOnGradStream(dy);
        readOnGradStream(dyop.a);
        readOnGradStream(xop.a);
      }
      if (Kp == nin) {
        af::array dw = ins[1].gradStorage();
        const int accumulate = dw.isEmpty() ? 0 : 1;
        if (!accumulate) dw = af::array::empty(ins[1].dims());
        check(w2l_gemm(wstream, gemmKind(), 1, 1, nout, nin, M, dyop.a.ptr(), dyop.ld, xop.a.ptr(), xop.ld, dw.f32(), nin, 0, nullptr, 0, accumulate,
                       nullptr, 0, 0, 0, 1.f, 0.f, 0ull, 0));
        ins[1].addGrad(Variable(dw, false));
      } else {
        af::array dwp = af::array::empty(af::dim4(Kp, nout));
        check(gemmP(1, 1, nout, Kp, M, dyop, xop, dwp.f32(), Kp, nullptr, 0, 0));
        af::array dw = af::array::empty(ins[1].dims());
        w2l::copyRows(dw.f32(), sizeof(float) * (size_t)nin, dwp.f32(), sizeof(float) * (size_t)Kp, sizeof(float) * (size_t)nin, (size_t)nout);
        ins[1].addGrad(Variable(dw, false));
      }
      if (hasBias) {
        af::array db = ins[2].gradStorage();
        if (db.isEmpty()) db = af::array::zeros(ins[2].dims());
        check(w2l_colsum_accumulate(wstream, M, nout, dy.f32(), nout, db.f32()));
        ins[2].addGrad(Variable(db, false));
      }
    }
    if (ins[0].isCalcGrad()) {
      if (Kp == inCols) {
        af::array acc = ins[0].accumulableGrad();
        af::array dx = acc.isEmpty() ? af::array::empty(ins[0].dims()) : acc;
        check(gemmP(0, 1, M, Kp, nout, dyop, wop, dx.f32(), Kp, nullptr, 0, acc.isEmpty() ? 0 : 1, inMaskMode ? ins[0].array().f32() : nullptr, Kp,
                    inMaskMode, inMaskScale));
        if (acc.isEmpty()) ins[0].addGrad(Variable(dx, false), true);
      } else {
        af::array dxp = af::array::empty(af::dim4(Kp, M));
        check(gemmP(0, 1, M, Kp, nout, dyop, wop, dxp.f32(), Kp, nullptr, 0, 0));
        af::array dx = af::array::empty(ins[0].dims());
        w2l::copyRows(dx.f32(), sizeof(float) * (size_t)inCols, dxp.f32(), sizeof(float) * (size_t)Kp, sizeof(float) * (size_t)inCols, (size_t)M);
        if (inMaskMode) {
          af::array m = af::array::empty(dx.dims());
          check(w2l_mask_mul(currentStream(), dx.elements(), dx.f32(), ins[0].array().f32(), inMaskMode, inMaskScale, m.f32()));
          dx = m;
        }
        ins[0].addGrad(Variable(dx, false), true);
      }
    }
  });
}

TDSBlock::TDSBlock(int channels, int kernelSize, int width, double dropout, int innerLinearDim, int rightPadding, bool lNormIncludeTime)
    : c_(channels), k_(kernelSize), w_(width), inner_(innerLinearDim > 0 ? innerLinearDim : channels * width), dropout_(dropout) {
  conv_ = std::make_shared<Conv2D>(c_, c_, k_, 1, 1, 1, (int)PaddingMode::SAME, 0);
  if (rightPadding >= 0) {
    if (rightPadding > k_ - 1) throw std::invalid_argument("TDSBlock: rightPadding exceeds kernel - 1");
    conv_->setAsymmetricPad(k_ - 1 - rightPadding, rightPadding);
  }
  conv_->fuseRelu();
  conv_->fuseDropout((float)dropout);
  const std::vector<int> lnAxes = lNormIncludeTime ? std::vector<int>{0, 1, 2} : std::vector<int>{1, 2};
  ln1_ = std::make_shared<LayerNorm>(lnAxes);
  ln2_ = std::make_shared<LayerNorm>(lnAxes);
  lin1_ = std::make_shared<Linear>(c_ * w_, inner_);
  lin2_ = std::make_shared<Linear>(inner_, c_ * w_);
}
std::vector<Variable> TDSBlock::params() const {
  std::vector<Variable> p;
  for (const Module* m : {(const Module*)conv_.get(), (const Module*)ln1_.get(), (const Module*)lin1_.get(), (const Module*)lin2_.get(),
                          (const Module*)ln2_.get()}) {
    auto q = m->params();
    p.insert(p.end(), q.begin(), q.end());
  }
  return p;
}
void TDSBlock::setParams(const Variable& v, int i) {
  Module* mods[5] = {conv_.get(), ln1_.get(), lin1_.get(), lin2_.get(), ln2_.get()};
  for (Module* m : mods) {
    const int n = (int)m->params().size();
    if (i < n) {
      m->setParams(v, i);
      return;
    }
    i -= n;
  }
  throw std::out_of_range("TDSBlock::setParams: index out of range");
}
void TDSBlock::train() {
  train_ = true;
  for (Module* m : {(Module*)conv_.get(), (Module*)ln1_.get(), (Module*)lin1_.get(), (Module*)lin2_.get(), (Module*)ln2_.get()}) m->train();
}
void TDSBlock::eval() {
  train_ = false;
  for (Module* m : {(Module*)conv_.get(), (Module*)ln1_.get(), (Module*)lin1_.get(), (Module*)lin2_.get(), (Module*)ln2_.get()}) m->eval();
}
std::string TDSBlock::prettyString() const {
  std::ostringstream o;
  o << "TDSBlock (c=" << c_ << ", k=" << k_ << ", w=" << w_ << ", dropout=" << dropout_ << ", inner=" << inner_ << ")\n\t\t" << conv_->prettyString()
    << "\n\t\t" << lin1_->prettyString() << "\n\t\t" << lin2_->prettyString();
  return o.str();
}
Variable TDSBlock::forward(const Variable& in) {
  if (in.dims(0) != w_ || in.dims(1) != c_) throw std::invalid_argument("TDSBlock: expects [W=" + std::to_string(w_) + ", C=" + std::to_string(c_) + ", T, B] input, got " + in.dims().str());
  const float dp = train_ ? (float)dropout_ : 0.f;
  const float keep = dp > 0 ? 1.0f / (1.0f - dp) : 1.0f;
  Variable y1 = conv_->forwardMasked(in, true);
  Variable z = ln1_->forwardResidual(y1, in, 1, keep);
  Variable h = lin1_->forwardFused(z, true, dp, true);
  Variable u = lin2_->forwardFused(h, false, dp, true, 1, keep);
  Variable ur(u.array().reshaped(z.dims()), {u}, [](std::vector<Variable>& ins, const Variable& g) {
    ins[0].addGrad(Variable(g.array().reshaped(ins[0].dims()), false));
  });
  return ln2_->forwardResidual(ur, z, dp > 0.f ? 2 : 0, keep);
}

void FirstOrderOptimizer::zeroGrad() {
  for (auto& p : parameters_) p.zeroGrad();
}
SGDOptimizer::SGDOptimizer(const std::vector<Variable>& params, double lr, double momentum, double weightDecay, bool useNesterov)
    : FirstOrderOptimizer(params, lr), mu_(momentum), wd_(weightDecay), nesterov_(useNesterov) {
  if (useNesterov && momentum <= 0) throw std::invalid_argument("SGDOptimizer: Nesterov momentum needs momentum > 0");
  if (mu_ != 0)
    for (auto& p : parameters_) velocities_.push_back(af::array::zeros(p.dims()));
}
void SGDOptimizer::step() {
  for (size_t i = 0; i < parameters_.size(); ++i) {
    auto& p = parameters_[i];
    if (!p.isGradAvailable()) continue;
    check(w2l_sgd_step_ex(currentStream(), p.elements(), p.array().f32(), p.grad().array().f32(), mu_ != 0 ? velocities_[i].f32() : nullptr,
                          (float)lr_, (float)mu_, (float)wd_, 1.0f, 0.f, nullptr, nesterov_ ? 1 : 0, nullptr));
  }
}
std::string SGDOptimizer::prettyString() const {
  std::ostringstream o;
  o << "SGD" << (mu_ != 0 ? std::string(nesterov_ ? " (Nesterov momentum=" : " (momentum=") + std::to_string(mu_) + ")" : "") << (wd_ != 0 ? " (weight decay=" + std::to_string(wd_) + ")" : "");
  return o.str();
}
double clipGradNorm(const std::vector<Variable>& params, double maxNorm) {
  af::array sq = af::array::zeros(af::dim4(1), DType::f64);
  for (auto& p : params)
    if (p.isGradAvailable()) check(w2l_sq_norm_accumulate(currentStream(), p.elements(), p.grad().array().f32(), sq.f64()));
  const double norm = std::sqrt(sq.scalar<double>());
  const double scale = maxNorm / (norm + 1e-6);
  if (scale < 1.0)
    for (auto& p : params)
      if (p.isGradAvailable()) {
        af::array g = p.grad().array();
        af::array tmp = af::array::zeros(g.dims());
        check(w2l_axpy(currentStream(), g.elements(), (float)scale, g.f32(), tmp.f32()));
        g.copyFrom(tmp);
      }
  return norm;
}
ParameterArena flattenParameters(const std::vector<std::shared_ptr<Module>>& modules) {
  ParameterArena a;
  std::vector<std::pair<Module*, int>> slots;
  long long total = 0;
  for (auto& m : modules) {
    auto ps = m->params();
    for (int i = 0; i < (int)ps.size(); ++i) {
      slots.emplace_back(m.get(), i);
      total += (ps[i].elements() + 3) / 4 * 4;
    }
  }
  a.elements = total;
  a.values = af::array::zeros(af::dim4(total));
  a.grads = af::array::zeros(af::dim4(total));
  a.velocity = af::array::zeros(af::dim4(total));
  long long off = 0;
  for (auto& s : slots) {
    Variable p = s.first->param(s.second);
    af::array slot = af::array::view(a.values, (size_t)off * 4, p.dims(), DType::f32);
    slot.copyFrom(p.array());
    Variable np(slot, true);
    np.setGradStorage(af::array::view(a.grads, (size_t)off * 4, p.dims(), DType::f32));
    s.first->setParams(np, s.second);
    off += (p.elements() + 3) / 4 * 4;
  }
  return a;
}

namespace {
ncclComm_t g_comm = nullptr;
int g_rank = 0, g_world = 1;
void ncclCheck(ncclResult_t r, const char* what) {
  if (r != ncclSuccess) throw std::runtime_error(std::string(what) + ": " + ncclGetErrorString(r));
}
}
int getWorldRank() { return g_rank; }
int getWorldSize() { return g_world; }
bool isDistributedInit() { return g_comm != nullptr; }
void allReduce(af::array& arr, double scale) {
  if (g_comm) {
    const ncclDataType_t t = arr.type() == DType::f64 ? ncclDouble : (arr.type() == DType::i32 ? ncclInt32 : ncclFloat32);
    ncclCheck(ncclAllReduce(arr.ptr(), arr.ptr(), (size_t)arr.elements(), t, ncclSum, g_comm, static_cast<cudaStream_t>(currentStream())),
              "ncclAllReduce");
  }
  if (scale != 1.0 && arr.type() == DType::f32) {
    af::array tmp = af::array::zeros(arr.dims());
    check(w2l_axpy(currentStream(), arr.elements(), (float)scale, arr.f32(), tmp.f32()));
    arr.copyFrom(tmp);
  }
}
void allReduceParameters(const std::shared_ptr<const Module>& module) {
  if (!g_comm) return;
  for (auto& p : module->params()) allReduce(p.array(), 1.0 / g_world);
}
CoalescingReducer::CoalescingReducer(double scale, bool, bool) : scale_(scale) {}
void CoalescingReducer::add(Variable& var) { pending_.push_back(var.array()); }
void CoalescingReducer::finalize() {
  size_t i = 0;
  while (i < pending_.size()) {
    char* begin = static_cast<char*>(pending_[i].ptr());
    char* end = begin + pending_[i].bytes();
    size_t j = i + 1;
    while (j < pending_.size() && static_cast<char*>(pending_[j].ptr()) >= end &&
           static_cast<char*>(pending_[j].ptr()) - end < 16 && pending_[j].type() == DType::f32) {
      end = static_cast<char*>(pending_[j].ptr()) + pending_[j].bytes();
      ++j;
    }
    if (g_comm)
      ncclCheck(ncclAllReduce(begin, begin, (size_t)(end - begin) / 4, ncclFloat32, ncclSum, g_comm, static_cast<cudaStream_t>(currentStream())),
                "ncclAllReduce");
    i = j;
  }
  if (scale_ != 1.0)
    for (auto& a : pending_) {
      af::array tmp = af::array::zeros(a.dims());
      check(w2l_axpy(currentStream(), a.elements(), (float)scale_, a.f32(), tmp.f32()));
      a.copyFrom(tmp);
    }
  pending_.clear();
}
OverlappedArenaReducer::OverlappedArenaReducer(const std::vector<Variable>& params, const af::array& arenaGrads, size_t bucketBytes)
    : grads_(arenaGrads) {
  const char* base = static_cast<const char*>(arenaGrads.ptr());
  const size_t total = arenaGrads.bytes();
  Bucket cur;
  bool open = false;
  for (const auto& p : params) {
    af::array g = p.gradStorage();
    if (g.isEmpty()) throw std::invalid_argument("OverlappedArenaReducer: a parameter is not bound to the gradient arena");
    const size_t off = (size_t)(static_cast<const char*>(g.ptr()) - base);
    if (off >= total) throw std::invalid_argument("OverlappedArenaReducer: parameter outside the arena");
    if (!open) {
      cur = Bucket();
      cur.offset = off / 4;
      open = true;
    }
    cur.count = (off + g.bytes()) / 4 - cur.offset;
    cur.params += 1;
    owner_.emplace_back(p.id(), (int)bucket_.size());
    const size_t k = bucket_.size();
    const size_t limit = k == 0 ? bucketBytes / 8 : (k == 1 ? bucketBytes / 4 : (k == 2 ? bucketBytes / 2 : bucketBytes));
    if (cur.count * 4 >= limit) {
      bucket_.push_back(cur);
      open = false;
    }
  }
  if (open) bucket_.push_back(cur);
  std::sort(owner_.begin(), owner_.end());
  seen_.assign(owner_.size(), 0);
  expected_.assign(owner_.size(), 0);
  cudaStream_t cs;
  int lo = 0, hi = 0;
  cudaDeviceGetStreamPriorityRange(&lo, &hi);
  if (cudaStreamCreateWithPriority(&cs, cudaStreamNonBlocking, hi) != cudaSuccess) throw std::runtime_error("OverlappedArenaReducer: stream");
  comm_stream_ = cs;
  for (auto& b : bucket_) {
    cudaEvent_t e;
    if (cudaEventCreateWithFlags(&e, cudaEventDisableTiming) != cudaSuccess) throw std::runtime_error("OverlappedArenaReducer: event");
    b.event = e;
  }
  cudaEvent_t d;
  if (cudaEventCreateWithFlags(&d, cudaEventDisableTiming) != cudaSuccess) throw std::runtime_error("OverlappedArenaReducer: event");
  done_ = d;
}
OverlappedArenaReducer::~OverlappedArenaReducer() {
  if (g_active_reducer == this) g_active_reducer = nullptr;
  for (auto& b : bucket_)
    if (b.event) cudaEventDestroy(static_cast<cudaEvent_t>(b.event));
  if (done_) cudaEventDestroy(static_cast<cudaEvent_t>(done_));
  if (comm_stream_) cudaStreamDestroy(static_cast<cudaStream_t>(comm_stream_));
}
void OverlappedArenaReducer::arm() {
  for (auto& b : bucket_) {
    b.remaining = b.params;
    b.launched = false;
  }
  std::fill(seen_.begin(), seen_.end(), 0);
  std::fill(expected_.begin(), expected_.end(), 0);
  armed_ = true;
  g_active_reducer = this;
}
void OverlappedArenaReducer::launch(Bucket& b) {
  b.launched = true;
  if (!g_comm) return;
  cudaStream_t compute = static_cast<cudaStream_t>(currentStream()), comm = static_cast<cudaStream_t>(comm_stream_);
  cudaEvent_t e = static_cast<cudaEvent_t>(b.event);
  if (cudaEventRecord(e, compute) != cudaSuccess || cudaStreamWaitEvent(comm, e, 0) != cudaSuccess)
    throw std::runtime_error("OverlappedArenaReducer: event record/wait failed");
  if (gradStream() && (cudaEventRecord(e, static_cast<cudaStream_t>(gradStream())) != cudaSuccess || cudaStreamWaitEvent(comm, e, 0) != cudaSuccess))
    throw std::runtime_error("OverlappedArenaReducer: event record/wait failed");
  float* ptr = grads_.f32() + b.offset;
  ncclCheck(ncclAllReduce(ptr, ptr, b.count, ncclFloat32, ncclSum, g_comm, comm), "ncclAllReduce (bucket)");
  if (norm_acc_) check(w2l_sq_norm_accumulate(comm, (long long)b.count, ptr, norm_acc_));
}
void OverlappedArenaReducer::expectContribution(const void* id) {
  if (!armed_) return;
  auto it = std::lower_bound(owner_.begin(), owner_.end(), std::make_pair(id, -1));
  if (it == owner_.end() || it->first != id) return;
  ++expected_[(size_t)(it - owner_.begin())];
}
void OverlappedArenaReducer::onGradReady(const void* id) {
  if (!armed_) return;
  auto it = std::lower_bound(owner_.begin(), owner_.end(), std::make_pair(id, -1));
  if (it == owner_.end() || it->first != id) return;
  const size_t k = (size_t)(it - owner_.begin());
  Bucket& b = bucket_[(size_t)it->second];
  if (b.launched)
    throw std::logic_error("OverlappedArenaReducer: a gradient arrived after its bucket was reduced");
  ++seen_[k];
  if (seen_[k] != std::max(1, expected_[k])) return;
  if (--b.remaining == 0) launch(b);
}
void OverlappedArenaReducer::finalize() {
  if (!armed_) return;
  armed_ = false;
  g_active_reducer = nullptr;
  for (size_t i = bucket_.size(); i-- > 0;)
    if (!bucket_[i].launched) launch(bucket_[i]);
  if (!g_comm) return;
  cudaStream_t compute = static_cast<cudaStream_t>(currentStream()), comm = static_cast<cudaStream_t>(comm_stream_);
  if (cudaEventRecord(static_cast<cudaEvent_t>(done_), comm) != cudaSuccess ||
      cudaStreamWaitEvent(compute, static_cast<cudaEvent_t>(done_), 0) != cudaSuccess)
    throw std::runtime_error("OverlappedArenaReducer: final wait failed");
}

namespace pkg {
namespace runtime {
void createUniqueId(void* id128) {
  ncclUniqueId id;
  ncclCheck(ncclGetUniqueId(&id), "ncclGetUniqueId");
  static_assert(sizeof(ncclUniqueId) == 128, "ncclUniqueId is 128 bytes");
  std::memcpy(id128, &id, 128);
}
void initDistributed(int worldRank, int worldSize, const void* id128) {
  if (g_comm) return;
  ncclUniqueId id;
  std::memcpy(&id, id128, 128);
  ncclConfig_t config = NCCL_CONFIG_INITIALIZER;
  int maxCtas = 8;
  if (const char* e = std::getenv("W2L_NCCL_MAX_CTAS")) maxCtas = std::atoi(e);
  if (maxCtas > 0) config.maxCTAs = maxCtas;
  ncclCheck(ncclCommInitRankConfig(&g_comm, worldSize, id, worldRank, &config), "ncclCommInitRankConfig");
  g_rank = worldRank;
  g_world = worldSize;
}

void initDistributed(int worldRank, int worldSize, int maxDevicesPerNode, const std::string& rndvFilepath) {
  if (g_comm) return;
  if (worldSize < 1 || worldRank < 0 || worldRank >= worldSize) throw std::invalid_argument("initDistributed: bad rank / size");
  if (maxDevicesPerNode > 0) {
    int ndev = 0;
    if (cudaGetDeviceCount(&ndev) == cudaSuccess && ndev > 0) cudaSetDevice(worldRank % std::min(maxDevicesPerNode, ndev));
  }
  if (worldSize == 1) {
    unsigned char id[128];
    createUniqueId(id);
    initDistributed(0, 1, id);
    return;
  }
  if (rndvFilepath.empty()) throw std::invalid_argument("initDistributed: a rendezvous path is needed for more than one process");
  const std::string path = rndvFilepath + "/w2l_b200_nccl_id." + std::to_string(worldSize);
  unsigned char id[128];
  if (worldRank == 0) {
    createUniqueId(id);
    const std::string tmp = path + ".tmp";
    {
      std::ofstream f(tmp, std::ios::binary | std::ios::trunc);
      if (!f) throw std::runtime_error("initDistributed: cannot write " + tmp);
      f.write(reinterpret_cast<const char*>(id), 128);
    }
    if (std::rename(tmp.c_str(), path.c_str()) != 0) throw std::runtime_error("initDistributed: cannot publish " + path);
  } else {
    bool ok = false;
    for (int tries = 0; tries < 6000 && !ok; ++tries) {
      std::ifstream f(path, std::ios::binary);
      if (f && f.read(reinterpret_cast<char*>(id), 128) && f.gcount() == 128) ok = true;
      else std::this_thread::sleep_for(std::chrono::milliseconds(100));
    }
    if (!ok) throw std::runtime_error("initDistributed: rendezvous file " + path + " did not appear");
  }
  initDistributed(worldRank, worldSize, id);
  if (worldRank == 0) {
    std::remove(path.c_str());
  }
}

namespace {
std::vector<std::string> splitWs(const std::string& line) {
  std::istringstream is(line);
  std::vector<std::string> out;
  std::string tok;
  while (is >> tok) out.push_back(tok);
  return out;
}
std::string replaceAll(std::string s, const std::string& from, const std::string& to) {
  size_t pos = 0;
  while ((pos = s.find(from, pos)) != std::string::npos) {
    s.replace(pos, from.size(), to);
    pos += to.size();
  }
  return s;
}
}

std::shared_ptr<Sequential> buildSequentialModule(const std::string& archText, int64_t nFeatures, int64_t nClasses) {
  auto net = std::make_shared<Sequential>();
  std::istringstream in(archText);
  std::string line;
  std::shared_ptr<Conv2D> lastConv;
  std::shared_ptr<Conv2D> lastBigConv;
  std::shared_ptr<GatedLinearUnit> lastGlu;
  int pendingPadL = -1, pendingPadR = -1;
  int lineNo = 0;
  while (std::getline(in, line)) {
    ++lineNo;
    const auto hash = line.find('#');
    if (hash != std::string::npos) line = line.substr(0, hash);
    line = replaceAll(line, "NFEAT", std::to_string(nFeatures));
    line = replaceAll(line, "NLABEL", std::to_string(nClasses));
    auto p = splitWs(line);
    if (p.empty()) continue;
    auto bad = [&](const std::string& why) { return std::invalid_argument("arch line " + std::to_string(lineNo) + " '" + line + "': " + why); };
    auto num = [&](size_t i) -> int {
      if (i >= p.size()) throw bad("missing argument");
      return std::stoi(p[i]);
    };
    const std::string& op = p[0];
    if (pendingPadL >= 0 && op != "C2") throw bad("PD must be followed by the C2 convolution it pads");
    std::shared_ptr<Conv2D> conv0 = std::move(lastConv), big0 = std::move(lastBigConv);
    std::shared_ptr<GatedLinearUnit> glu0 = std::move(lastGlu);
    lastConv.reset();
    lastBigConv.reset();
    lastGlu.reset();
    if (op == "V") {
      if (p.size() != 5) throw bad("V expects 4 dims");
      net->add(std::make_shared<View>(af::dim4(num(1), num(2), num(3), num(4))));
    } else if (op == "RO") {
      if (p.size() != 5) throw bad("RO expects 4 dims");
      net->add(std::make_shared<Reorder>(num(1), num(2), num(3), num(4)));
    } else if (op == "PD") {
      if (p.size() < 4 || std::stod(p[1]) != 0.0) throw bad("only zero padding of the time axis is covered");
      for (size_t i = 4; i < p.size(); ++i)
        if (num(i) != 0) throw bad("only the time axis may be padded");
      pendingPadL = num(2);
      pendingPadR = num(3);
      if (pendingPadL < 0 || pendingPadR < 0) throw bad("negative padding");
    } else if (op == "C2") {
      if (p.size() < 7) throw bad("C2 expects cin cout kw kh sx sy [px py dx dy]");
      const int px = p.size() > 7 ? num(7) : 0, py = p.size() > 8 ? num(8) : 0;
      auto conv = std::make_shared<Conv2D>(num(1), num(2), num(3), num(4), num(5), num(6), px, py, p.size() > 9 ? num(9) : 1,
                                           p.size() > 10 ? num(10) : 1);
      if (pendingPadL >= 0) {
        if (px != 0) throw bad("PD followed by a padded convolution");
        conv->setAsymmetricPad(pendingPadL, pendingPadR);
        pendingPadL = pendingPadR = -1;
      }
      net->add(conv);
      lastConv = conv;
    } else if (op == "C" || op == "C1" || op == "WN") {
      size_t o = 0;
      int wnDim = -1;
      if (op == "WN") {
        if (p.size() < 4) throw bad("WN expects dim and a layer");
        wnDim = num(1);
        o = 2;
      }
      std::shared_ptr<Module> layer;
      std::shared_ptr<Conv2D> conv;
      if (p[o] == "C" || p[o] == "C1") {
        if (p.size() < o + 5) throw bad("C expects cin cout kw stride [pad dil bias groups]");
        const int px = p.size() > o + 5 ? num(o + 5) : 0, dil = p.size() > o + 6 ? num(o + 6) : 1;
        const bool cb = p.size() > o + 7 ? num(o + 7) != 0 : true;
        const int groups = p.size() > o + 8 ? num(o + 8) : 1;
        conv = std::make_shared<Conv2D>(num(o + 1), num(o + 2), num(o + 3), 1, num(o + 4), 1, px, 0, dil, 1, cb, groups);
        layer = conv;
      } else if (p[o] == "L") {
        if (p.size() < o + 3) throw bad("L expects in out [bias]");
        layer = std::make_shared<Linear>(num(o + 1), num(o + 2), p.size() > o + 3 ? num(o + 3) != 0 : true);
      } else {
        throw bad("WN wraps C or L only");
      }
      if (wnDim >= 0) layer = std::make_shared<WeightNorm>(layer, wnDim);
      net->add(layer);
      lastBigConv = conv;
    } else if (op == "GLU") {
      if (p.size() != 2) throw bad("GLU expects the axis");
      auto glu = std::make_shared<GatedLinearUnit>(num(1));
      if (big0) big0->setGluSplit(true);
      net->add(glu);
      lastGlu = glu;
    } else if (op == "R") {
      if (conv0) {
        conv0->fuseRelu();
        lastConv = conv0;
      } else {
        net->add(std::make_shared<ReLU>());
      }
    } else if (op == "DO") {
      if (p.size() != 2) throw bad("DO expects a probability");
      if (glu0)
        glu0->fuseDropout((float)std::stod(p[1]));
      else if (conv0)
        conv0->fuseDropout(std::stof(p[1]));
      else
        net->add(std::make_shared<Dropout>(std::stod(p[1])));
    } else if (op == "LN") {
      std::vector<int> axes;
      for (size_t i = 1; i < p.size(); ++i) axes.push_back(num(i));
      if (axes.empty()) throw bad("LN expects axes");
      net->add(std::make_shared<LayerNorm>(axes));
    } else if (op == "TDS") {
      if (p.size() < 4) throw bad("TDS expects c kw w [dropout] [inner] [rPad] [lnIncludeTime]");
      net->add(std::make_shared<TDSBlock>(num(1), num(2), num(3), p.size() > 4 ? std::stod(p[4]) : 0.0, p.size() > 5 ? num(5) : 0,
                                          p.size() > 6 ? num(6) : -1, p.size() > 7 ? num(7) != 0 : true));
    } else if (op == "L") {
      if (p.size() < 3) throw bad("L expects in out [bias]");
      net->add(std::make_shared<Linear>(num(1), num(2), p.size() > 3 ? num(3) != 0 : true));
    } else if (op == "SAUG") {
      if (p.size() != 7) throw bad("SAUG expects tWarpW fMaskF nFMask tMaskT tMaskP nTMask");
      net->add(std::make_shared<SpecAugment>(num(1), num(2), num(3), num(4), std::stod(p[5]), num(6)));
    } else {
      throw bad("opcode '" + op + "' is outside the hot-path subset (V RO PD C C2 WN GLU R DO LN TDS L SAUG)");
    }
  }
  if (pendingPadL >= 0) throw std::invalid_argument("arch: trailing PD without a convolution");
  return net;
}
ModulePlugin::ModulePlugin(const std::string& path) : path_(path) {
  handle_ = dlopen(path.c_str(), RTLD_NOW | RTLD_GLOBAL);
  if (!handle_) {
    const char* e = dlerror();
    throw std::runtime_error("ModulePlugin: cannot load " + path + ": " + (e ? e : "unknown error"));
  }
  create_ = dlsym(handle_, "createModule");
  if (!create_) throw std::runtime_error("ModulePlugin: " + path + " does not export createModule(int64_t, int64_t)");
}
std::shared_ptr<Module> ModulePlugin::arch(int64_t nFeatures, int64_t nClasses) {
  using Fn = Module* (*)(int64_t, int64_t);
  Module* m = reinterpret_cast<Fn>(create_)(nFeatures, nClasses);
  if (!m) throw std::runtime_error("ModulePlugin: createModule returned null (" + path_ + ")");
  return std::shared_ptr<Module>(m);
}
std::shared_ptr<Sequential> buildSequentialModuleFromFile(const std::string& path, int64_t nFeatures, int64_t nClasses) {
  std::ifstream f(path);
  if (!f) throw std::invalid_argument("arch file not found: " + path);
  std::stringstream ss;
  ss << f.rdbuf();
  return buildSequentialModule(ss.str(), nFeatures, nClasses);
}
}

namespace speech {
CriterionScaleMode getCriterionScaleMode(const std::string& onorm, bool sqnorm) {
  if (onorm == "none") return CriterionScaleMode::NONE;
  if (onorm == "input") return sqnorm ? CriterionScaleMode::INPUT_SZ_SQRT : CriterionScaleMode::INPUT_SZ;
  if (onorm == "target") return sqnorm ? CriterionScaleMode::TARGET_SZ_SQRT : CriterionScaleMode::TARGET_SZ;
  throw std::invalid_argument("invalid onorm option: " + onorm);
}
namespace {
void checkCriterionInputs(const std::vector<Variable>& inputs, const char* who) {
  if (inputs.size() != 2) throw std::invalid_argument(std::string(who) + ": expects {emissions, target}");
  if (inputs[0].type() != DType::f32) throw std::invalid_argument(std::string(who) + ": emissions must be f32");
  if (inputs[1].type() != DType::i32) throw std::invalid_argument(std::string(who) + ": target must be s32");
  if (inputs[0].dims(2) != inputs[1].dims(1)) throw std::invalid_argument(std::string(who) + ": batch size mismatch between emissions and target");
}
}

AutoSegmentationCriterion::AutoSegmentationCriterion(int N, CriterionScaleMode scalemode, double transdiag) : N_(N), scaleMode_(scalemode) {
  if (N <= 0) throw std::invalid_argument("ASG: N must be positive");
  std::vector<float> tr((size_t)N * N, 0.f);
  for (int i = 0; i < N; ++i) tr[(size_t)i * N + i] = (float)transdiag;
  params_.push_back(Variable(af::array::fromHost(tr.data(), af::dim4(N, N)), true));
}
std::string AutoSegmentationCriterion::prettyString() const { return "AutoSegmentationCriterion"; }

namespace {
std::vector<Variable> asgForward(int terms, int N, CriterionScaleMode mode, bool train, Variable trans, af::array& wsCache,
                                 const Variable& emis, const af::array& target) {
  const int T = (int)emis.dims(1), B = (int)emis.dims(2), L = (int)target.dims(0);
  if (emis.dims(0) != N) throw std::invalid_argument("ASG: emissions have " + std::to_string(emis.dims(0)) + " classes, expected " + std::to_string(N));
  const size_t wsb = w2l_asg_workspace_size(B, T, N, L);
  af::array ws = workspaceFor(wsCache, wsb);
  af::array loss = af::array::empty(af::dim4(B));
  const bool needGrad = train && (emis.isCalcGrad() || trans.isCalcGrad());
  if (!needGrad) {
    check(w2l_asg_forward_backward(currentStream(), terms, B, T, N, L, (int)mode, emis.array().f32(), target.i32(), trans.array().f32(), nullptr,
                                   loss.f32(), nullptr, nullptr, ws.ptr(), ws.bytes()));
    return {Variable(loss, false)};
  }
  af::array dEmis = af::array::empty(emis.dims());
  af::array dTrans = af::array::empty(trans.dims());
  check(w2l_asg_forward_backward(currentStream(), terms, B, T, N, L, (int)mode, emis.array().f32(), target.i32(), trans.array().f32(), nullptr,
                                 loss.f32(), dEmis.f32(), dTrans.f32(), ws.ptr(), ws.bytes()));
  return {Variable(loss, {emis, trans}, [=](std::vector<Variable>& ins, const Variable& g) mutable {
    af::array de = dEmis, dt = dTrans;
    if (!g.isOnesSeed()) {
      af::array ws2 = af::array::empty(af::dim4((long long)wsb), DType::u8);
      af::array l2 = af::array::empty(af::dim4(B));
      de = af::array::empty(ins[0].dims());
      dt = af::array::empty(ins[1].dims());
      check(w2l_asg_forward_backward(currentStream(), terms, B, T, N, L, (int)mode, ins[0].array().f32(), target.i32(), ins[1].array().f32(),
                                     g.array().f32(), l2.f32(), de.f32(), dt.f32(), ws2.ptr(), ws2.bytes()));
    }
    ins[0].addGrad(Variable(de, false));
    ins[1].addGrad(Variable(dt, false));
  })};
}
}

std::vector<Variable> AutoSegmentationCriterion::forward(const std::vector<Variable>& inputs) {
  checkCriterionInputs(inputs, "AutoSegmentationCriterion");
  return asgForward(W2L_TERM_ASG, N_, scaleMode_, train_, params_[0], ws_, inputs[0], inputs[1].array());
}
af::array AutoSegmentationCriterion::viterbiPath(const af::array& input, const af::array&) {
  const int N = (int)input.dims(0), T = (int)input.dims(1), B = (int)input.dims(2);
  if (N != N_) throw std::invalid_argument("ASG viterbiPath: class count mismatch");
  af::array path = af::array::empty(af::dim4(T, B), DType::i32);
  af::array ws = af::array::empty(af::dim4((long long)std::max<size_t>(w2l_fcc_viterbi_workspace_size(B, T, N), 256)), DType::u8);
  check(w2l_fcc_viterbi(currentStream(), B, T, N, input.f32(), params_[0].array().f32(), path.i32(), ws.ptr(), ws.bytes()));
  return path;
}

af::array SequenceCriterion::viterbiPathWithTarget(const af::array&, const af::array&, af::array*) {
  throw std::logic_error(prettyString() + ": viterbiPathWithTarget is not implemented");
}

namespace {
af::array facAlign(int N, const Variable& trans, const af::array& input, const af::array& target, af::array* index) {
  const int T = (int)input.dims(1), B = (int)input.dims(2), L = (int)target.dims(0);
  if (input.dims(0) != N) throw std::invalid_argument("viterbiPathWithTarget: class count mismatch");
  if (target.type() != DType::i32 || target.dims(1) != B) throw std::invalid_argument("viterbiPathWithTarget: target must be s32 [L,B]");
  af::array path = af::array::empty(af::dim4(T, B), DType::i32);
  af::array idx = index ? af::array::empty(af::dim4(T, B), DType::i32) : af::array();
  af::array ws = af::array::empty(af::dim4((long long)std::max<size_t>(w2l_fac_viterbi_workspace_size(B, T, N, L), 256)), DType::u8);
  check(w2l_fac_viterbi(currentStream(), B, T, N, L, input.f32(), target.i32(), trans.array().f32(), path.i32(), index ? idx.i32() : nullptr,
                        ws.ptr(), ws.bytes()));
  if (index) *index = idx;
  return path;
}
}

af::array AutoSegmentationCriterion::viterbiPathWithTarget(const af::array& input, const af::array& target, af::array* index) {
  return facAlign(N_, params_[0], input, target, index);
}

ConnectionistTemporalClassificationCriterion::ConnectionistTemporalClassificationCriterion(CriterionScaleMode scalemode) : scaleMode_(scalemode) {}
std::string ConnectionistTemporalClassificationCriterion::prettyString() const { return "ConnectionistTemporalClassificationCriterion"; }
std::vector<Variable> ConnectionistTemporalClassificationCriterion::forward(const std::vector<Variable>& inputs) {
  checkCriterionInputs(inputs, "ConnectionistTemporalClassificationCriterion");
  const Variable& emis = inputs[0];
  const af::array target = inputs[1].array();
  const int N = (int)emis.dims(0), T = (int)emis.dims(1), B = (int)emis.dims(2), L = (int)target.dims(0);
  const size_t wsb = w2l_ctc_workspace_size(B, T, N, L);
  af::array ws = workspaceFor(ws_, wsb);
  af::array loss = af::array::empty(af::dim4(B));
  const CriterionScaleMode mode = scaleMode_;
  if (!(train_ && emis.isCalcGrad())) {
    check(w2l_ctc_forward_backward(currentStream(), B, T, N, L, (int)mode, emis.array().f32(), target.i32(), nullptr, loss.f32(), nullptr, ws.ptr(),
                                   ws.bytes()));
    return {Variable(loss, false)};
  }
  af::array dEmis = af::array::empty(emis.dims());
  check(w2l_ctc_forward_backward(currentStream(), B, T, N, L, (int)mode, emis.array().f32(), target.i32(), nullptr, loss.f32(), dEmis.f32(), ws.ptr(),
                                 ws.bytes()));
  return {Variable(loss, {emis}, [=](std::vector<Variable>& ins, const Variable& g) mutable {
    af::array de = dEmis;
    if (!g.isOnesSeed()) {
      af::array ws2 = af::array::empty(af::dim4((long long)wsb), DType::u8);
      af::array l2 = af::array::empty(af::dim4(B));
      de = af::array::empty(ins[0].dims());
      check(w2l_ctc_forward_backward(currentStream(), B, T, N, L, (int)mode, ins[0].array().f32(), target.i32(), g.array().f32(), l2.f32(), de.f32(),
                                     ws2.ptr(), ws2.bytes()));
    }
    ins[0].addGrad(Variable(de, false));
  })};
}
af::array ConnectionistTemporalClassificationCriterion::viterbiPath(const af::array& input, const af::array&) {
  const int N = (int)input.dims(0), T = (int)input.dims(1), B = (int)input.dims(2);
  af::array path = af::array::empty(af::dim4(T, B), DType::i32);
  check(w2l_argmax_path(currentStream(), B, T, N, input.f32(), path.i32()));
  return path;
}

af::array ConnectionistTemporalClassificationCriterion::viterbiPathWithTarget(const af::array& input, const af::array& target,
                                                                             af::array* index) {
  const int N = (int)input.dims(0), T = (int)input.dims(1), B = (int)input.dims(2), L = (int)target.dims(0);
  if (target.type() != DType::i32 || target.dims(1) != B) throw std::invalid_argument("viterbiPathWithTarget: target must be s32 [L,B]");
  af::array path = af::array::empty(af::dim4(T, B), DType::i32);
  af::array state = index ? af::array::empty(af::dim4(T, B), DType::i32) : af::array();
  af::array ws = workspaceFor(ws_, w2l_ctc_viterbi_workspace_size(B, T, N, L));
  check(w2l_ctc_viterbi_target(currentStream(), B, T, N, L, input.f32(), target.i32(), path.i32(), index ? state.i32() : nullptr, ws.ptr(),
                               ws.bytes()));
  if (index) *index = state;
  return path;
}

LinearSegmentationCriterion::LinearSegmentationCriterion(int N, CriterionScaleMode scalemode) : N_(N), scaleMode_(scalemode) {
  params_.push_back(Variable(af::array::zeros(af::dim4(N, N)), true));
}
std::string LinearSegmentationCriterion::prettyString() const { return "LinearSegmentationCriterion"; }
std::vector<Variable> LinearSegmentationCriterion::forward(const std::vector<Variable>& inputs) {
  checkCriterionInputs(inputs, "LinearSegmentationCriterion");
  const int T = (int)inputs[0].dims(1), B = (int)inputs[0].dims(2), L = (int)inputs[1].dims(0);
  af::array stretched = af::array::empty(af::dim4(T, B), DType::i32);
  check(w2l_linseg_target(currentStream(), B, T, L, inputs[1].array().i32(), stretched.i32()));
  return asgForward(W2L_TERM_ASG, N_, scaleMode_, train_, params_[0], ws_, inputs[0], stretched);
}
af::array LinearSegmentationCriterion::viterbiPath(const af::array& input, const af::array&) {
  const int N = (int)input.dims(0), T = (int)input.dims(1), B = (int)input.dims(2);
  af::array path = af::array::empty(af::dim4(T, B), DType::i32);
  af::array ws = af::array::empty(af::dim4((long long)std::max<size_t>(w2l_fcc_viterbi_workspace_size(B, T, N), 256)), DType::u8);
  check(w2l_fcc_viterbi(currentStream(), B, T, N, input.f32(), params_[0].array().f32(), path.i32(), ws.ptr(), ws.bytes()));
  return path;
}

af::array LinearSegmentationCriterion::viterbiPathWithTarget(const af::array& input, const af::array& target, af::array* index) {
  return facAlign(N_, params_[0], input, target, index);
}

}
}
}
```

Before: 932,800.

## Pre-split linear weights into TF32 hi/lo planes for F32x3 GEMMs

Adds a kernel that splits a float32 weight matrix, optionally transposed, into TF32 high and low planes. It also adds a GEMM mode that loads both planes by 3-D TMA straight into the operand ring, which skips the in-kernel B conversion stage and its separate converted-buffer ring. Linear forward and data-grad GEMMs use this path when the precision is F32x3. The cost is an extra split kernel launch and twice the B memory traffic and shared-memory space per stage. The path only runs when F32X3 precision is selected.

```diff
diff --git a/include/w2l_b200.h b/include/w2l_b200.h
--- a/include/w2l_b200.h
+++ b/include/w2l_b200.h
@@ -71,7 +71,7 @@
 
 W2L_API int w2l_gemm_tf32_view(void* stream, int a_mn_major, int b_mn_major, int M, int N, int K, const float* A, int lda,
                                const float* B, int ldb, float* C, int ldc, const float* bias, int act, int accumulate);
-enum { W2L_GEMM_TF32 = 0, W2L_GEMM_F32X3 = 1, W2L_GEMM_BF16 = 2 };
+enum { W2L_GEMM_TF32 = 0, W2L_GEMM_F32X3 = 1, W2L_GEMM_BF16 = 2, W2L_GEMM_F32X3_SPLIT_B = 3 };
 enum { W2L_PRECISION_TF32 = 0, W2L_PRECISION_F32 = 1, W2L_PRECISION_BF16 = 2 };
 W2L_API int w2l_set_precision(int precision);
 W2L_API int w2l_get_precision(void);
@@ -81,6 +81,7 @@
                      unsigned long long seed, int allow_overlap);
 W2L_API int w2l_cast_bf16(void* stream, long long n, const float* x, void* y);
 W2L_API int w2l_cast_bf16_rows(void* stream, long long rows, int cols, int ld_in, int cols_padded, const float* x, void* y);
+W2L_API int w2l_split_tf32(void* stream, int transpose, int rows, int cols, int ld, int cols_padded, const float* x, float* planes);
 W2L_API int w2l_gemm_set_tile(int bn);
 W2L_API int w2l_gemm_set_variant(int variant);
 W2L_API int w2l_gemm_tf32(void* stream, int a_mn_major, int b_mn_major, int M, int N, int K, const float* A, int lda,
diff --git a/wav2letter_b200/capi.py b/wav2letter_b200/capi.py
--- a/wav2letter_b200/capi.py
+++ b/wav2letter_b200/capi.py
@@ -18,7 +18,7 @@
     "w2l_fac_viterbi_workspace_size", "w2l_fac_viterbi",
     "w2l_ctc_workspace_size", "w2l_ctc_forward_backward", "w2l_argmax_path", "w2l_linseg_target",
     "w2l_ctc_viterbi_workspace_size", "w2l_ctc_viterbi_target",
-    "w2l_set_precision", "w2l_get_precision", "w2l_gemm", "w2l_cast_bf16", "w2l_cast_bf16_rows", "w2l_sgd_step_ex", "w2l_finite_guard",
+    "w2l_set_precision", "w2l_get_precision", "w2l_gemm", "w2l_cast_bf16", "w2l_cast_bf16_rows", "w2l_split_tf32", "w2l_sgd_step_ex", "w2l_finite_guard",
     "w2l_mask_bands", "w2l_trainer_set_precision", "w2l_trainer_set_grad_stream", "w2l_trainer_set_grad_stream_delay", "w2l_delay", "w2l_trainer_status", "w2l_trainer_save", "w2l_trainer_load", "w2l_trainer_export_streaming",
     "w2l_text_create", "w2l_text_destroy", "w2l_text_num_classes", "w2l_text_encode", "w2l_text_prediction2ltr", "w2l_text_target2ltr",
     "w2l_text_ltr2wrd", "w2l_text_align_words", "w2l_edit_distance",
@@ -99,6 +99,7 @@
     lib.w2l_gemm.argtypes = [vp, i, i, i, i, i, i, vp, i, vp, i, vp, i, i, vp, i, i, vp, i, i, i, f32, f32, u64, i]
     lib.w2l_cast_bf16.argtypes = [vp, ll, vp, vp]
     lib.w2l_cast_bf16_rows.argtypes = [vp, ll, i, i, i, vp, vp]
+    lib.w2l_split_tf32.argtypes = [vp, i, i, i, i, i, vp, vp]
     lib.w2l_sgd_step_ex.argtypes = [vp, ll, vp, vp, vp, f32, f32, f32, f32, f32, vp, i, vp]
     lib.w2l_finite_guard.argtypes = [vp, i, vp, vp, vp]
     lib.w2l_mask_bands.argtypes = [vp, i, i, i, i, vp, vp, i, vp, vp, i, vp, vp, f32]
@@ -333,7 +334,7 @@
 
 
 PRECISIONS = {"tf32": 0, "f32": 1, "fp32": 1, "bf16": 2}
-GEMM_KINDS = {"tf32": 0, "f32x3": 1, "bf16": 2}
+GEMM_KINDS = {"tf32": 0, "f32x3": 1, "bf16": 2, "f32x3_split_b": 3}
 
 
 def set_precision(p) -> None:
@@ -348,9 +349,9 @@
          aux_mode=0, aux_scale=1.0, dropout_p=0.0, seed=0, M=None, N=None, K=None, lda=None, ldb=None, allow_overlap=False):
     if M is None:
         M, K = (A.shape[1], A.shape[0]) if a_mn else A.shape
-        N = B.shape[1] if b_mn else B.shape[0]
+        N = B.shape[-2] if B.dim() == 3 else (B.shape[1] if b_mn else B.shape[0])
     lda = A.stride(0) if lda is None else lda
-    ldb = B.stride(0) if ldb is None else ldb
+    ldb = B.stride(-2) if ldb is None else ldb
     if out is None:
         out = torch.empty((M, N), dtype=torch.bfloat16 if out_bf16 else torch.float32, device=A.device)
     _check(lib.w2l_gemm(_stream(), GEMM_KINDS[kind], int(a_mn), int(b_mn), M, N, K, _ptr(A), lda, _ptr(B), ldb, _ptr(out),
@@ -364,6 +365,17 @@
     x = _req(x, torch.float32, "x")
     y = torch.empty(x.shape, dtype=torch.bfloat16, device=x.device)
     _check(lib.w2l_cast_bf16(_stream(), x.numel(), _ptr(x), _ptr(y)))
+    return y
+
+
+def split_tf32(x, transpose=False, cols_padded=None):
+    if x.dtype != torch.float32 or not x.is_cuda or x.dim() != 2 or x.stride(1) != 1:
+        raise TypeError("split_tf32: x must be a 2-D CUDA float32 tensor with contiguous rows")
+    rows, cols = x.shape
+    k = rows if transpose else cols
+    cols_padded = (k + 3) // 4 * 4 if cols_padded is None else cols_padded
+    y = torch.empty((2, cols if transpose else rows, cols_padded), dtype=torch.float32, device=x.device)
+    _check(lib.w2l_split_tf32(_stream(), int(transpose), rows, cols, x.stride(0), cols_padded, _ptr(x), _ptr(y)))
     return y
 
 
diff --git a/wav2letter_b200/csrc/gemm_wgmma.cu b/wav2letter_b200/csrc/gemm_wgmma.cu
--- a/wav2letter_b200/csrc/gemm_wgmma.cu
+++ b/wav2letter_b200/csrc/gemm_wgmma.cu
@@ -21,25 +21,28 @@
 constexpr int kGemmThreads = 384;
 constexpr int kConvThreads = 96;
 constexpr int kConsumerThreads = 256;
-enum { kTf32 = W2L_GEMM_TF32, kF32x3 = W2L_GEMM_F32X3, kBf16 = W2L_GEMM_BF16 };
+enum { kTf32 = W2L_GEMM_TF32, kF32x3 = W2L_GEMM_F32X3, kBf16 = W2L_GEMM_BF16, kF32x3SplitB = W2L_GEMM_F32X3_SPLIT_B };
 
 __host__ __device__ constexpr bool converts(int mode, bool a_mn, bool b_mn) { return mode == kF32x3 || (mode == kTf32 && (a_mn || b_mn)); }
-__host__ __device__ constexpr size_t raw_bytes(int bn) { return (size_t)kTileBytes + (size_t)bn * kRowBytes; }
+__host__ __device__ constexpr bool a_in_regs(int mode, bool a_mn, bool b_mn) { return converts(mode, a_mn, b_mn) || mode == kF32x3SplitB; }
+__host__ __device__ constexpr size_t raw_bytes(int mode, int bn) { return (size_t)kTileBytes + (size_t)bn * kRowBytes * (mode == kF32x3SplitB ? 2 : 1); }
 __host__ __device__ constexpr size_t cvt_bytes(int mode, int bn) { return (size_t)bn * kRowBytes * (mode == kF32x3 ? 2 : 1); }
 constexpr size_t kSmemTail = 1024 + 256;
 constexpr size_t kSmemBudget = 227 * 1024 - kSmemTail;
 constexpr int kConvRawStages = 4;
 constexpr int kIdSlots = 4;
 __host__ __device__ constexpr int raw_stages(int mode, bool a_mn, bool b_mn, int bn) {
-  return converts(mode, a_mn, b_mn) ? kConvRawStages : (kSmemBudget / raw_bytes(bn) > 6 ? 6 : (int)(kSmemBudget / raw_bytes(bn)));
+  return converts(mode, a_mn, b_mn) ? kConvRawStages
+                                    : (kSmemBudget / raw_bytes(mode, bn) > 6 ? 6 : (int)(kSmemBudget / raw_bytes(mode, bn)));
 }
 __host__ __device__ constexpr int cvt_stages(int mode, bool a_mn, bool b_mn, int bn) {
   return !converts(mode, a_mn, b_mn) ? 0
-         : (kSmemBudget - kConvRawStages * raw_bytes(bn)) / cvt_bytes(mode, bn) > 4 ? 4
-                                                                                     : (int)((kSmemBudget - kConvRawStages * raw_bytes(bn)) / cvt_bytes(mode, bn));
+         : (kSmemBudget - kConvRawStages * raw_bytes(mode, bn)) / cvt_bytes(mode, bn) > 4
+             ? 4
+             : (int)((kSmemBudget - kConvRawStages * raw_bytes(mode, bn)) / cvt_bytes(mode, bn));
 }
 __host__ __device__ constexpr size_t smem_for(int mode, bool a_mn, bool b_mn, int bn) {
-  return raw_stages(mode, a_mn, b_mn, bn) * raw_bytes(bn) + cvt_stages(mode, a_mn, b_mn, bn) * cvt_bytes(mode, bn) + kSmemTail;
+  return raw_stages(mode, a_mn, b_mn, bn) * raw_bytes(mode, bn) + cvt_stages(mode, a_mn, b_mn, bn) * cvt_bytes(mode, bn) + kSmemTail;
 }
 
 struct GemmParams {
@@ -164,13 +167,15 @@
                   unsigned int* sched) {
   extern __shared__ __align__(1024) unsigned char smem_raw[];
   unsigned char* smem = reinterpret_cast<unsigned char*>((reinterpret_cast<uintptr_t>(smem_raw) + 1023) & ~(uintptr_t)1023);
-  constexpr bool kIsBf16 = kMode == kBf16, kSplit = kMode == kF32x3, kConv = converts(kMode, kAMn, kBMn);
+  constexpr bool kIsBf16 = kMode == kBf16, kPreSplit = kMode == kF32x3SplitB, kSplit = kMode == kF32x3 || kPreSplit;
+  constexpr bool kConv = converts(kMode, kAMn, kBMn), kRegA = a_in_regs(kMode, kAMn, kBMn);
   constexpr int BKE = kRowBytes / (kIsBf16 ? 2 : 4);
   constexpr int kStages = raw_stages(kMode, kAMn, kBMn, BN), kCvtStages = cvt_stages(kMode, kAMn, kBMn, BN);
-  constexpr size_t kRaw = raw_bytes(BN), kCvt = cvt_bytes(kMode, BN);
+  constexpr size_t kRaw = raw_bytes(kMode, BN), kCvt = cvt_bytes(kMode, BN);
   constexpr uint32_t kOperandBytes = (uint32_t)kRaw;
   static_assert(kStages >= 2 && (!kConv || kCvtStages >= 2), "gemm: at least two stages per ring");
-  static_assert(!kConv || BN == 128, "gemm: the converted kinds take A from registers at BN = 128");
+  static_assert(!kRegA || BN == 128, "gemm: the kinds that take A from registers run at BN = 128");
+  static_assert(!kPreSplit || !kBMn, "gemm: pre-split B planes are K-major");
   static_assert(!kIsBf16 || !kBMn || BN % 64 == 0, "gemm: MN-major bf16 B is staged in boxes of 64 columns");
   unsigned char* cvt_ring = smem + kStages * kRaw;
   uint64_t* bars = reinterpret_cast<uint64_t*>(cvt_ring + kCvtStages * kCvt);
@@ -220,7 +225,13 @@
     m0 = (r / tiles_n) * BM;
     n0 = (r % tiles_n) * BN;
     kb_begin = z * kb_per;
-    num_kb = max(0, min(total_kb, kb_begin + kb_per) - kb_begin);
+    int total = total_kb;
+    if constexpr (kPreSplit) {
+      int k = p.K;
+      asm volatile("" : "+r"(k));
+      total = (k + BKE - 1) / BKE;
+    }
+    num_kb = max(0, min(total, kb_begin + kb_per) - kb_begin);
   };
 
   if (wg == 0) {
@@ -248,7 +259,10 @@
 #pragma unroll
               for (int j = 0; j < BM / 8; ++j) tma_load_2d(&map_a, &full[s], sa + j * 1024, m0 + 8 * j, k0);
             }
-            if (!kBMn) {
+            if (kPreSplit) {
+              tma_load_3d(&map_b, &full[s], sb, k0, n0, 0);
+              tma_load_3d(&map_b, &full[s], sb + BN * kRowBytes, k0, n0, 1);
+            } else if (!kBMn) {
               tma_load_2d(&map_b, &full[s], sb, k0, n0);
             } else if (kIsBf16) {
 #pragma unroll
@@ -301,7 +315,7 @@
       float acc[BN / 2];
 #pragma unroll
       for (int i = 0; i < BN / 2; ++i) acc[i] = 0.f;
-      if constexpr (kConv) {
+      if constexpr (kRegA) {
         struct AFrag {
           uint32_t hi[4][4], lo[4][4];
         };
@@ -309,8 +323,12 @@
           wg::fence_operands(f.hi);
           if constexpr (kSplit) wg::fence_operands(f.lo);
         };
+        auto release_b = [&](uint32_t i) {
+          if constexpr (kConv) mbar_arrive(&cvt_empty[i % kCvtStages]);
+          else mbar_arrive(&empty[i % kStages]);
+        };
         auto step = [&](AFrag& cur, AFrag& prev, int kb) {
-          const int s = it % kStages, c = it % kCvtStages;
+          const int s = it % kStages;
           mbar_wait(&full[s], (it / kStages) & 1);
           const uint32_t sa = smem_u32(smem + s * kRaw);
 #pragma unroll
@@ -325,9 +343,15 @@
               if constexpr (kSplit) cur.lo[kk][i] = rn_tf32(__float_as_uint(__uint_as_float(x) - __uint_as_float(cur.hi[kk][i])));
             }
           }
-          mbar_arrive(&empty[s]);
-          mbar_wait(&ready[c], (it / kCvtStages) & 1);
-          const uint32_t b_base = smem_u32(cvt_ring + c * kCvt);
+          uint32_t b_base;
+          if constexpr (kConv) {
+            const int c = it % kCvtStages;
+            mbar_arrive(&empty[s]);
+            mbar_wait(&ready[c], (it / kCvtStages) & 1);
+            b_base = smem_u32(cvt_ring + c * kCvt);
+          } else {
+            b_base = sa + kTileBytes;
+          }
           fence_frag(cur);
           wg::fence_operands(acc);
           wg::fence();
@@ -347,7 +371,7 @@
           wg::fence_operands(acc);
           if constexpr (kSplit) wg::wait<1>(); else wg::wait<0>();
           fence_frag(prev);
-          if (kb > 0) mbar_arrive(&cvt_empty[(it - 1) % kCvtStages]);
+          if (kb > 0) release_b(it - 1);
           ++it;
         };
         AFrag fa, fb;
@@ -359,7 +383,7 @@
         wg::fence_operands(acc);
         fence_frag(fa);
         fence_frag(fb);
-        if (num_kb > 0) mbar_arrive(&cvt_empty[(it - 1) % kCvtStages]);
+        if (num_kb > 0) release_b(it - 1);
       } else {
         for (int kb = 0; kb < num_kb; ++kb, ++it) {
           const int s = it % kStages;
@@ -416,24 +440,56 @@
   }
 }
 
-int make_map(CUtensorMap* map, int mode, bool conv, const void* ptr, long long rows, long long cols, long long ld, int box_cols, int box_rows,
-             bool swizzle) {
+template <bool kT>
+__global__ void __launch_bounds__(256) split_tf32_kernel(int rows, int cols, int ld, int R, int ld_out, const float* __restrict__ x,
+                                                         float* __restrict__ y) {
+  __shared__ float tile[32][33];
+  const int tx = threadIdx.x & 31, ty = threadIdx.x >> 5;
+  const int r0 = blockIdx.x * 32, c0 = blockIdx.y * 32;
+  if (kT) {
+    for (int i = ty; i < 32; i += 8) {
+      const int sr = c0 + i, sc = r0 + tx;
+      tile[i][tx] = (sr < rows && sc < cols) ? x[(size_t)sr * ld + sc] : 0.f;
+    }
+    __syncthreads();
+  }
+  const size_t plane = (size_t)R * ld_out;
+  for (int i = ty; i < 32; i += 8) {
+    const int r = r0 + i, c = c0 + tx;
+    if (r >= R || c >= ld_out) continue;
+    const float v = kT ? tile[tx][i] : (c < cols ? x[(size_t)r * ld + c] : 0.f);
+    const uint32_t h = rn_tf32(__float_as_uint(v));
+    const uint32_t l = rn_tf32(__float_as_uint(v - __uint_as_float(h)));
+    y[(size_t)r * ld_out + c] = __uint_as_float(h);
+    y[plane + (size_t)r * ld_out + c] = __uint_as_float(l);
+  }
+}
+
+int make_map(CUtensorMap* map, int mode, bool raw, const void* ptr, long long rows, long long cols, long long ld, int box_cols, int box_rows,
+             bool swizzle, int planes = 1) {
   EncodeTiledFn fn = encode_fn();
   if (!fn) return fail(W2L_ERR_CUDA, "gemm: cuTensorMapEncodeTiled entry point not found");
   const int es = mode == kBf16 ? 2 : 4;
-  cuuint64_t dims[2] = {(cuuint64_t)cols, (cuuint64_t)rows};
-  cuuint64_t strides[1] = {(cuuint64_t)ld * es};
-  cuuint32_t box[2] = {(cuuint32_t)box_cols, (cuuint32_t)box_rows};
-  cuuint32_t estr[2] = {1, 1};
-  const CUtensorMapDataType dt = mode == kBf16 ? CU_TENSOR_MAP_DATA_TYPE_BFLOAT16 : (conv ? CU_TENSOR_MAP_DATA_TYPE_FLOAT32 : CU_TENSOR_MAP_DATA_TYPE_TFLOAT32);
-  CUresult r = fn(map, dt, 2, const_cast<void*>(ptr), dims, strides, box, estr, CU_TENSOR_MAP_INTERLEAVE_NONE,
+  cuuint64_t dims[3] = {(cuuint64_t)cols, (cuuint64_t)rows, (cuuint64_t)planes};
+  cuuint64_t strides[2] = {(cuuint64_t)ld * es, (cuuint64_t)(rows * ld * es)};
+  cuuint32_t box[3] = {(cuuint32_t)box_cols, (cuuint32_t)box_rows, 1};
+  cuuint32_t estr[3] = {1, 1, 1};
+  const CUtensorMapDataType dt = mode == kBf16 ? CU_TENSOR_MAP_DATA_TYPE_BFLOAT16 : (raw ? CU_TENSOR_MAP_DATA_TYPE_FLOAT32 : CU_TENSOR_MAP_DATA_TYPE_TFLOAT32);
+  CUresult r = fn(map, dt, planes > 1 ? 3 : 2, const_cast<void*>(ptr), dims, strides, box, estr, CU_TENSOR_MAP_INTERLEAVE_NONE,
                   swizzle ? CU_TENSOR_MAP_SWIZZLE_128B : CU_TENSOR_MAP_SWIZZLE_NONE, CU_TENSOR_MAP_L2_PROMOTION_L2_256B,
                   CU_TENSOR_MAP_FLOAT_OOB_FILL_NONE);
   if (r != CUDA_SUCCESS) return fail(W2L_ERR_CUDA, "gemm: cuTensorMapEncodeTiled failed with code " + std::to_string((int)r));
   return W2L_OK;
 }
 
-const char* kernel_name(int mode) { return mode == kBf16 ? "gemm_wgmma_kernel<bf16>" : (mode == kF32x3 ? "gemm_wgmma_kernel<f32x3>" : "gemm_wgmma_kernel<tf32>"); }
+const char* kernel_name(int mode) {
+  switch (mode) {
+    case kBf16: return "gemm_wgmma_kernel<bf16>";
+    case kF32x3: return "gemm_wgmma_kernel<f32x3>";
+    case kF32x3SplitB: return "gemm_wgmma_kernel<f32x3_split_b>";
+    default: return "gemm_wgmma_kernel<tf32>";
+  }
+}
 
 thread_local int g_variant = 1;
 
@@ -480,7 +536,7 @@
 }
 template <int kMode, bool kAMn, bool kBMn>
 int launch_mode(cudaStream_t stream, int bn, const CUtensorMap& ma, const CUtensorMap& mb, const GemmParams& p) {
-  if constexpr (converts(kMode, kAMn, kBMn)) {
+  if constexpr (a_in_regs(kMode, kAMn, kBMn)) {
     return launch_bn<kMode, kAMn, kBMn, 128>(stream, ma, mb, p);
   } else if constexpr (kMode == kBf16) {
     return bn <= 128 ? launch_bn<kMode, kAMn, kBMn, 128>(stream, ma, mb, p) : launch_bn<kMode, kAMn, kBMn, 256>(stream, ma, mb, p);
@@ -495,10 +551,14 @@
 }
 template <int kMode>
 int launch(cudaStream_t stream, bool a_mn, bool b_mn, int bn, const CUtensorMap& ma, const CUtensorMap& mb, const GemmParams& p) {
-  if (!a_mn && !b_mn) return launch_mode<kMode, false, false>(stream, bn, ma, mb, p);
-  if (!a_mn && b_mn) return launch_mode<kMode, false, true>(stream, bn, ma, mb, p);
-  if (a_mn && b_mn) return launch_mode<kMode, true, true>(stream, bn, ma, mb, p);
-  return launch_mode<kMode, true, false>(stream, bn, ma, mb, p);
+  if constexpr (kMode == kF32x3SplitB) {
+    return a_mn ? launch_mode<kMode, true, false>(stream, bn, ma, mb, p) : launch_mode<kMode, false, false>(stream, bn, ma, mb, p);
+  } else {
+    if (!a_mn && !b_mn) return launch_mode<kMode, false, false>(stream, bn, ma, mb, p);
+    if (!a_mn && b_mn) return launch_mode<kMode, false, true>(stream, bn, ma, mb, p);
+    if (a_mn && b_mn) return launch_mode<kMode, true, true>(stream, bn, ma, mb, p);
+    return launch_mode<kMode, true, false>(stream, bn, ma, mb, p);
+  }
 }
 
 int splits_for(int tiles, int total_kb, bool plain) {
@@ -509,7 +569,7 @@
 thread_local int g_force_bn = 0;
 int choose_bn(int mode, bool a_mn, bool b_mn, int M, int N, int total_kb, bool plain, int* splits_out) {
   auto allowed = [&](int bn) {
-    if (converts(mode, a_mn, b_mn)) return bn == 128;
+    if (a_in_regs(mode, a_mn, b_mn)) return bn == 128;
     if (mode == kBf16) return bn == 128 || bn == 256;
     return true;
   };
@@ -543,7 +603,8 @@
               void* C, int ldc, int c_bf16, const float* bias, int act, int accumulate, const void* aux, int ld_aux, int aux_bf16,
               int aux_mode, float aux_scale, float dropout_p, unsigned long long seed, bool allow_overlap) {
   cudaStream_t stream = static_cast<cudaStream_t>(stream_);
-  if (mode != kTf32 && mode != kF32x3 && mode != kBf16) return fail(W2L_ERR_INVALID_ARGUMENT, "gemm: unknown operand kind");
+  if (mode != kTf32 && mode != kF32x3 && mode != kBf16 && mode != kF32x3SplitB) return fail(W2L_ERR_INVALID_ARGUMENT, "gemm: unknown operand kind");
+  if (mode == kF32x3SplitB && b_mn_major) return fail(W2L_ERR_INVALID_ARGUMENT, "gemm: F32X3_SPLIT_B takes K-major B planes");
   if (M <= 0 || N <= 0 || K <= 0) return fail(W2L_ERR_INVALID_ARGUMENT, "gemm: M, N, K must be positive");
   if (!A || !B || !C) return fail(W2L_ERR_INVALID_ARGUMENT, "gemm: null pointer");
   if (act < 0 || act > 1) return fail(W2L_ERR_INVALID_ARGUMENT, "gemm: act must be 0 (none) or 1 (relu)");
@@ -563,24 +624,28 @@
   const bool plain = act == 0 && aux_mode == 0 && dropout_p == 0.f && bias == nullptr && !c_bf16;
   int splits = 1;
   const int BN = choose_bn(mode, a_mn_major != 0, b_mn_major != 0, M, N, total_kb, plain, &splits);
-  const bool conv = converts(mode, a_mn_major != 0, b_mn_major != 0);
+  const bool raw = a_in_regs(mode, a_mn_major != 0, b_mn_major != 0);
   const bool bf16 = mode == kBf16;
   CUtensorMap ma, mb;
   int rc;
   if (!a_mn_major)
-    rc = make_map(&ma, mode, conv, A, M, K, lda, bke, BM, true);
+    rc = make_map(&ma, mode, raw, A, M, K, lda, bke, BM, true);
   else
-    rc = make_map(&ma, mode, conv, A, K, M, lda, bf16 ? 64 : 8, bke, bf16);
+    rc = make_map(&ma, mode, raw, A, K, M, lda, bf16 ? 64 : 8, bke, bf16);
   if (rc) return rc;
   if (!b_mn_major)
-    rc = make_map(&mb, mode, conv, B, N, K, ldb, bke, BN, true);
+    rc = make_map(&mb, mode, raw, B, N, K, ldb, bke, BN, true, mode == kF32x3SplitB ? 2 : 1);
   else
-    rc = make_map(&mb, mode, conv, B, K, N, ldb, bf16 ? 64 : BN, bke, bf16);
+    rc = make_map(&mb, mode, raw, B, K, N, ldb, bf16 ? 64 : BN, bke, bf16);
   if (rc) return rc;
   GemmParams p{M, N, K, ldc, act, C, bias, accumulate, aux_mode, ld_aux, aux, aux_scale, dropout_p, seed, splits, c_bf16, aux_bf16, nullptr};
   if (splits > 1) W2L_CUDA_CHECK(cudaMallocAsync(reinterpret_cast<void**>(&p.ws), sizeof(float) * (size_t)splits * M * N, stream));
-  rc = mode == kBf16 ? launch<kBf16>(stream, a_mn_major, b_mn_major, BN, ma, mb, p)
-                     : (mode == kF32x3 ? launch<kF32x3>(stream, a_mn_major, b_mn_major, BN, ma, mb, p) : launch<kTf32>(stream, a_mn_major, b_mn_major, BN, ma, mb, p));
+  switch (mode) {
+    case kBf16: rc = launch<kBf16>(stream, a_mn_major, b_mn_major, BN, ma, mb, p); break;
+    case kF32x3: rc = launch<kF32x3>(stream, a_mn_major, b_mn_major, BN, ma, mb, p); break;
+    case kF32x3SplitB: rc = launch<kF32x3SplitB>(stream, a_mn_major, b_mn_major, BN, ma, mb, p); break;
+    default: rc = launch<kTf32>(stream, a_mn_major, b_mn_major, BN, ma, mb, p);
+  }
   if (splits > 1) {
     if (rc == W2L_OK) {
       const long long mn = (long long)M * N;
@@ -685,3 +750,18 @@
   W2L_LAUNCH_CHECK("cast_bf16_rows_kernel");
   return W2L_OK;
 }
+extern "C" int w2l_split_tf32(void* stream_, int transpose, int rows, int cols, int ld, int cols_padded, const float* x, float* planes) {
+  if (rows <= 0 || cols <= 0) return W2L_OK;
+  if (!x || !planes || ld < cols) return fail(W2L_ERR_INVALID_ARGUMENT, "split_tf32: bad arguments");
+  const int R = transpose ? cols : rows;
+  if (cols_padded < (transpose ? rows : cols) || (cols_padded + 31) / 32 > 65535)
+    return fail(W2L_ERR_INVALID_ARGUMENT, "split_tf32: bad plane size");
+  cudaStream_t stream = static_cast<cudaStream_t>(stream_);
+  const dim3 grid((unsigned)((R + 31) / 32), (unsigned)((cols_padded + 31) / 32));
+  if (transpose)
+    split_tf32_kernel<true><<<grid, 256, 0, stream>>>(rows, cols, ld, R, cols_padded, x, planes);
+  else
+    split_tf32_kernel<false><<<grid, 256, 0, stream>>>(rows, cols, ld, R, cols_padded, x, planes);
+  W2L_LAUNCH_CHECK("split_tf32_kernel");
+  return W2L_OK;
+}
diff --git a/wav2letter_b200/csrc/tma_ptx.cuh b/wav2letter_b200/csrc/tma_ptx.cuh
--- a/wav2letter_b200/csrc/tma_ptx.cuh
+++ b/wav2letter_b200/csrc/tma_ptx.cuh
@@ -37,6 +37,13 @@
       "l"(map), "r"(smem_u32(bar)), "r"(c0), "r"(c1)
       : "memory");
 }
+__device__ __forceinline__ void tma_load_3d(const CUtensorMap* map, uint64_t* bar, void* smem_dst, int c0, int c1, int c2) {
+  asm volatile(
+      "cp.async.bulk.tensor.3d.shared::cluster.global.mbarrier::complete_tx::bytes [%0], [%1, {%3, %4, %5}], [%2];" ::"r"(
+          smem_u32(smem_dst)),
+      "l"(map), "r"(smem_u32(bar)), "r"(c0), "r"(c1), "r"(c2)
+      : "memory");
+}
 __device__ __forceinline__ uint64_t make_desc_sw128(uint32_t saddr, uint32_t lbo_bytes, uint32_t sbo_bytes) {
   uint64_t d = 0;
   d |= (uint64_t)((saddr >> 4) & 0x3FFF);
diff --git a/wav2letter_b200/host/fl_compat.cpp b/wav2letter_b200/host/fl_compat.cpp
--- a/wav2letter_b200/host/fl_compat.cpp
+++ b/wav2letter_b200/host/fl_compat.cpp
@@ -441,6 +441,21 @@
           unsigned long long seed = 0, int allowOverlap = 0) {
   return w2l_gemm(currentStream(), gemmKind(), a_mn, b_mn, M, N, K, A.a.ptr(), A.ld, B.a.ptr(), B.ld, C, ldc, 0, bias, act, accumulate, aux, ld_aux, 0,
                   aux_mode, aux_scale, dropP, seed, allowOverlap);
+}
+GemmOperand weightPlanes(int b_mn, int N, int K, const GemmOperand& W) {
+  GemmOperand planes;
+  if (gemmKind() != W2L_GEMM_F32X3) return planes;
+  planes.ld = (int)padUp(K, 4);
+  planes.a = af::array::empty(af::dim4(planes.ld, N, 2));
+  check(w2l_split_tf32(currentStream(), b_mn, b_mn ? K : N, b_mn ? N : K, W.ld, planes.ld, W.a.f32(), planes.a.f32()));
+  return planes;
+}
+int gemmWeight(int b_mn, int M, int N, int K, const GemmOperand& A, const GemmOperand& W, const GemmOperand& planes, float* C, int ldc,
+               const float* bias, int act, int accumulate, const float* aux = nullptr, int ld_aux = 0, int aux_mode = 0, float aux_scale = 1.f,
+               float dropP = 0.f, unsigned long long seed = 0) {
+  if (planes.a.isEmpty()) return gemmP(0, b_mn, M, N, K, A, W, C, ldc, bias, act, accumulate, aux, ld_aux, aux_mode, aux_scale, dropP, seed);
+  return w2l_gemm(currentStream(), W2L_GEMM_F32X3_SPLIT_B, 0, 0, M, N, K, A.a.ptr(), A.ld, planes.a.ptr(), planes.ld, C, ldc, 0, bias, act, accumulate,
+                  aux, ld_aux, 0, aux_mode, aux_scale, dropP, seed, 0);
 }
 }
 
@@ -939,12 +954,14 @@
     wop.ld = Kp;
     wop.a = padRowsF32(wv.array().f32(), nOut, nIn, nIn, Kp);
   }
-  check(gemmP(0, 0, M, nOut, Kp, xop, wop, y.f32(), nOut, hasBias_ ? bv.array().f32() : nullptr, relu ? 1 : 0, 0, nullptr, 0, 0, 1.f, dp, nextSeed()));
+  check(gemmWeight(0, M, nOut, Kp, xop, wop, weightPlanes(0, nOut, Kp, wop), y.f32(), nOut, hasBias_ ? bv.array().f32() : nullptr, relu ? 1 : 0, 0,
+                   nullptr, 0, 0, 1.f, dp, nextSeed()));
   const int nin = nIn, nout = nOut;
   const bool hasBias = hasBias_;
   std::vector<Variable> inputs{in, wv};
   if (hasBias) inputs.push_back(bv);
   return Variable(y, inputs, [=](std::vector<Variable>& ins, const Variable& gout) {
+    const GemmOperand wtPlanes = ins[0].isCalcGrad() ? weightPlanes(1, Kp, nout, wop) : GemmOperand();
     af::array dy = gout.array();
     if (!maskByConsumer && (relu || dp > 0.f)) {
       af::array m = af::array::empty(y.dims());
@@ -986,12 +1003,12 @@
       if (Kp == inCols) {
         af::array acc = ins[0].accumulableGrad();
         af::array dx = acc.isEmpty() ? af::array::empty(ins[0].dims()) : acc;
-        check(gemmP(0, 1, M, Kp, nout, dyop, wop, dx.f32(), Kp, nullptr, 0, acc.isEmpty() ? 0 : 1, inMaskMode ? ins[0].array().f32() : nullptr, Kp,
-                    inMaskMode, inMaskScale));
+        check(gemmWeight(1, M, Kp, nout, dyop, wop, wtPlanes, dx.f32(), Kp, nullptr, 0, acc.isEmpty() ? 0 : 1, inMaskMode ? ins[0].array().f32() : nullptr,
+                         Kp, inMaskMode, inMaskScale));
         if (acc.isEmpty()) ins[0].addGrad(Variable(dx, false), true);
       } else {
         af::array dxp = af::array::empty(af::dim4(Kp, M));
-        check(gemmP(0, 1, M, Kp, nout, dyop, wop, dxp.f32(), Kp, nullptr, 0, 0));
+        check(gemmWeight(1, M, Kp, nout, dyop, wop, wtPlanes, dxp.f32(), Kp, nullptr, 0, 0));
         af::array dx = af::array::empty(ins[0].dims());
         w2l::copyRows(dx.f32(), sizeof(float) * (size_t)inCols, dxp.f32(), sizeof(float) * (size_t)Kp, sizeof(float) * (size_t)inCols, (size_t)M);
         if (inMaskMode) {
```

Result: faster. 1.023 million (median of 6 runs) (+9.6%).
